# slyforce/MusicStyleTransfer

Hardware: AMD Instinct MI355X
Metric: piano-roll frames/s (VAE train step) (higher is better)
Workload: dtype bf16; 1 GPU; BASELINE configs[1]: single-track piano-roll VAE train step, T=256, pitch=128, latent=64, batch=64/GPU, bf16; encoder 256x2x8h, decoder 128x1x8h (scripts/train-vae.sh), dropout 0.2; Xavier-initialised weights; global_batch=64, seq_len=256, pitches=128, latent=64, parallelism=dp1, params=1885440

## Files before the change

include/mst_hip.h:

```cpp
#ifndef MST_HIP_H
#define MST_HIP_H

#include <stdint.h>

#ifdef __cplusplus
extern "C" {
#endif

typedef void* mst_stream_t;

enum mst_status {
  MST_OK = 0,
  MST_ERR_INVALID = -1,
  MST_ERR_LAUNCH = -2,
  MST_ERR_UNSUPPORTED = -3
};

enum mst_dtype { MST_BF16 = 0, MST_F16 = 1, MST_F32 = 2 };

enum mst_act { MST_ACT_NONE = 0, MST_ACT_RELU = 1 };

int mst_version(void);
const char* mst_last_error(void);

int mst_graph_begin(mst_stream_t stream);
int mst_graph_end(mst_stream_t stream, void** graph_exec_out);
int mst_graph_end_counted(mst_stream_t stream, void** graph_exec_out, int32_t* nodes_out, int32_t* kernel_nodes_out);
int mst_graph_launch(void* graph_exec, mst_stream_t stream);
int mst_graph_destroy(void* graph_exec);

int mst_event_create(void** ev_out);
int mst_event_record(void* ev, mst_stream_t stream);
int mst_event_sync(void* ev);
int mst_event_elapsed_ms(void* ev_start, void* ev_stop, float* ms_out);
int mst_event_destroy(void* ev);

typedef struct mst_gemm_args {
  int32_t dtype;
  int32_t c_f32;
  int64_t M, N, K;
  const void* A; int64_t lda;
  const void* B; int64_t ldb;
  void* C; int64_t ldc;
  const float* bias;
  const void* resid; int64_t ldr;
  int32_t act;
  const void* gate; int64_t ldg;
  float alpha;
  const float* rowadd; int64_t ldra; int64_t rowadd_period;
  const float* grpadd; int64_t ldga; const int32_t* grp_index;
  int64_t a_rows_per_group, a_group_stride, a_group_offset;
  int64_t c_rows_per_group, c_group_stride, c_group_offset;
  float dropout_p; uint64_t dropout_seed; uint32_t dropout_site;
  int32_t self_resid;
  const uint64_t* dropout_seed_ptr;
  int32_t a_u8;
  int32_t resid_phys;
} mst_gemm_args;

int mst_gemm_nt(const mst_gemm_args* args, mst_stream_t stream);
int mst_gemm_nt_form(const mst_gemm_args* args);

int mst_gemm_nt_pair(const mst_gemm_args* args0, const mst_gemm_args* args1, mst_stream_t stream);

typedef struct mst_bce_args {
  const uint8_t* labels;
  int64_t T;
  float label_smoothing;
  int32_t downweight;
  float* loss;
  void* probs; int64_t ldp;
  void* logits; int64_t ldl;
  float gscale;
} mst_bce_args;
int mst_gemm_sigmoid_bce(const mst_gemm_args* args, const mst_bce_args* bce, mst_stream_t stream);

typedef struct mst_ln_args {
  int32_t mode;
  const float* gamma;
  const float* beta;
  float eps;
  void* out; int64_t ld_out;
  float* mean; float* rstd;
  const void* x; int64_t ld_x;
  float* dgamma; float* dbeta;
  int32_t mask_mode;
  float* partials;
} mst_ln_args;

int mst_gemm_nt_ln(const mst_gemm_args* args, const mst_ln_args* ln, mst_stream_t stream);
int mst_gemm_sigmoid_bce_dgrad_ln(const mst_gemm_args* args, const mst_bce_args* bce, const mst_gemm_args* dgrad,
                                  const mst_ln_args* ln, mst_stream_t stream);
int64_t mst_gemm_nt_ln_parts(int64_t M);

int mst_ffn_ln_fwd(const mst_gemm_args* ff1, const mst_gemm_args* ff2, const mst_ln_args* ln, mst_stream_t stream);
int mst_ffn_ln_bwd(const mst_gemm_args* ff2_dgrad, const mst_gemm_args* ff1_dgrad, const mst_ln_args* ln, mst_stream_t stream);
typedef struct mst_ln_bwd_in {
  const void* dy; int64_t ld_dy;
  const void* x;  int64_t ld_x;
  const float* gamma; const float* mean; const float* rstd;
  void* dx; int64_t ld_dx;
  void* dx_masked; int64_t ld_dxm;
  float* dgamma; float* dbeta; float* partials;
  int32_t mask_mode;
  float dropout_p; uint64_t dropout_seed; const uint64_t* dropout_seed_ptr; uint32_t dropout_site;
} mst_ln_bwd_in;
int mst_ffn_ln_bwd_lead(const mst_ln_bwd_in* lead, const mst_gemm_args* ff2_dgrad, const mst_gemm_args* ff1_dgrad,
                        const mst_ln_args* ln, mst_stream_t stream);
int mst_proj_ffn_ln_fwd(const mst_gemm_args* proj, const mst_ln_args* ln1, const mst_gemm_args* ff1, const mst_gemm_args* ff2,
                        const mst_ln_args* ln2, mst_stream_t stream);

typedef struct mst_partial_sum {
  const float* src; int64_t n_parts; int64_t stride; int64_t len;
  float* dst; float scale;
} mst_partial_sum;
int mst_partial_sums(const mst_partial_sum* jobs, int n, mst_stream_t stream);

typedef struct mst_wgrad_args {
  int32_t dtype;
  int64_t M, N, K;
  const void* A; int64_t lda;
  const void* B; int64_t ldb;
  float* dW; int64_t ldw;
  float* db;
  float scale;
  int64_t a_rows_per_group, a_group_stride, a_group_offset;
  int64_t b_rows_per_group, b_group_stride, b_group_offset;
  int32_t a_u8;
} mst_wgrad_args;

typedef struct mst_outer_job {
  const float* L; const void* R; int32_t r_dtype; int64_t r_stride;
  int64_t B, J, I;
  float* out; float* obias;
} mst_outer_job;
int mst_outer_jobs(const mst_outer_job* jobs, int n, mst_stream_t stream);
int mst_gemm_wgrad_batch_flush(const mst_wgrad_args* list, int n, float* scratch, int64_t scratch_bytes,
                               const mst_partial_sum* sums, int n_sums, const mst_outer_job* outers, int n_outers,
                               mst_stream_t stream);
int mst_gemm_wgrad_plan(const mst_wgrad_args* list, int n, int64_t scratch_bytes, int64_t* plan);

int mst_embed_fwd(int dtype, int64_t B, int64_t T, int64_t D,
                  const int32_t* tokens, const float* table, int64_t ldt,
                  const int32_t* classes, const float* cls_table, int64_t ldc,
                  const float* pos, int64_t ldp, float alpha,
                  void* out, int64_t ld_out, int64_t S_out, int64_t s_off,
                  uint8_t* keymask, mst_stream_t stream);

int mst_embed_bwd(int dtype, int64_t B, int64_t T, int64_t D,
                  const int32_t* tokens, float* dtable, int64_t ldt,
                  const int32_t* classes, float* dcls, int64_t ldc, float alpha,
                  const void* dX, int64_t ld_dx, int64_t S_out, int64_t s_off,
                  mst_stream_t stream);

int mst_group_colsum(int dtype, int64_t B, int64_t T, int64_t D, const void* X, int64_t ldx,
                     int64_t S_out, int64_t s_off, const int32_t* idx, float* dst, int64_t ldd,
                     float alpha, mst_stream_t stream);

int mst_mask_from_lengths(int64_t B, int64_t S, const int32_t* lens, int32_t add,
                          uint8_t* keymask, mst_stream_t stream);

int mst_attn_keysoftmax_fwd(int dtype, int64_t B, int64_t S, int64_t H, int64_t dh,
                            const void* qkv, int64_t ld_qkv, int64_t k_off, int64_t q_off, int64_t v_off,
                            const uint8_t* keymask, float* lse,
                            void* out, int64_t ld_out,
                            int64_t q_limit ,
                            mst_stream_t stream);

int mst_attn_qkv_fwd(int dtype, int64_t B, int64_t S, int64_t H, int64_t dh, const void* x, int64_t ld_x, const void* w,
                     int64_t ld_w, const float* bias, void* qkv, int64_t ld_qkv, int64_t k_off, int64_t q_off, int64_t v_off,
                     const uint8_t* keymask, float* lse, void* out, int64_t ld_out, int64_t q_limit, mst_stream_t stream);
int mst_attn_keysoftmax_bwd(int dtype, int64_t B, int64_t S, int64_t H, int64_t dh,
                            const void* qkv, int64_t ld_qkv, int64_t k_off, int64_t q_off, int64_t v_off,
                            const uint8_t* keymask, const float* lse,
                            const void* dout, int64_t ld_dout,
                            void* dqkv, int64_t ld_dqkv, float* delta,
                            int64_t q_limit ,
                            mst_stream_t stream);

int mst_attn_causal_fwd(int dtype, int64_t B, int64_t S, int64_t H, int64_t dh,
                        const void* qkv, int64_t ld_qkv, int64_t k_off, int64_t q_off, int64_t v_off,
                        const uint8_t* keymask, float* lse, void* out, int64_t ld_out, mst_stream_t stream);
int mst_attn_causal_bwd(int dtype, int64_t B, int64_t S, int64_t H, int64_t dh,
                        const void* qkv, int64_t ld_qkv, int64_t k_off, int64_t q_off, int64_t v_off,
                        const uint8_t* keymask, const float* lse, const void* dout, int64_t ld_dout,
                        void* dqkv, int64_t ld_dqkv, float* delta, mst_stream_t stream);

int mst_layernorm_fwd(int dtype, int64_t M, int64_t D, const void* x, int64_t ldx,
                      const float* gamma, const float* beta, float eps,
                      void* y, int64_t ldy, float* mean, float* rstd,
                      int64_t row_id_stride ,
                      mst_stream_t stream);

int mst_layernorm_bwd(int dtype, int64_t M, int64_t D, const void* x, int64_t ldx,
                      const float* gamma, const float* mean, const float* rstd,
                      const void* dy, int64_t ldy, void* dx, int64_t ld_dx,
                      void* dx_masked, int64_t ld_dxm, float* dgamma, float* dbeta,
                      int mask_mode, float dropout_p, uint64_t dropout_seed, uint32_t dropout_site,
                      const uint64_t* dropout_seed_ptr,
                      int64_t row_id_stride ,
                      float* partials ,
                      mst_stream_t stream);
int64_t mst_layernorm_bwd_parts(int64_t M, int64_t D);

int mst_latent_fwd(int dtype, int64_t B, int64_t De, int64_t Z, int64_t Dd,
                   const void* enc_out, int64_t enc_sample_stride,
                   const float* Wl, const float* bl, const float* eps,
                   const float* Wh, const float* bh,
                   const int32_t* classes, const float* cls_d, int64_t ld_cls,
                   const float* pos_d, float alpha_d,
                   float* mu, float* sigma, float* z, float* kl,
                   void* dec_in, int64_t dec_sample_stride, mst_stream_t stream);
int mst_latent_fwd_proj(int dtype, int64_t B, int64_t De, int64_t Z, int64_t Dd,
                        const void* enc_out, int64_t enc_sample_stride,
                        const float* Wl, const float* bl, const float* eps,
                        const float* Wh, const float* bh,
                        const int32_t* classes, const float* cls_d, int64_t ld_cls,
                        const float* pos_d, float alpha_d,
                        float* mu, float* sigma, float* z, float* kl,
                        void* dec_in, int64_t dec_sample_stride,
                        const void* Wq, int64_t ld_wq, const float* bq, void* qkv0, int64_t qkv_sample_stride, int64_t nq,
                        mst_stream_t stream);
int mst_latent_rows(int dtype, int64_t N, int64_t M, int64_t Z, int64_t Dd,
                    const float* zsrc, const float* ssrc, const int32_t* a, const int32_t* b, const float* w, int mode,
                    float tau, uint64_t seed, const uint64_t* seed_ptr, uint32_t site, int64_t row0,
                    const float* Wh, const float* bh,
                    const int32_t* ca, const int32_t* cb, const float* cw, const float* cls_d, int64_t ld_cls, int64_t n_classes,
                    const float* pos_d, float alpha_d,
                    float* z_out, void* dec_in, int64_t dec_stride, mst_stream_t stream);

int mst_latent_bwd_vec(int dtype, int64_t B, int64_t De, int64_t Z, int64_t Dd, const float* Wl, const float* eps, const float* Wh,
                       const int32_t* classes, const float* mu, const float* sigma, const void* d_dec_in, int64_t dec_sample_stride,
                       float alpha_d, float kl_weight, float gscale, float enc_scale, float* dcls_d, int64_t ld_cls,
                       void* d_enc_out, int64_t denc_sample_stride, float* scratch, mst_stream_t stream);
int mst_latent_bwd_vec_proj(int dtype, int64_t B, int64_t De, int64_t Z, int64_t Dd, const float* Wl, const float* eps, const float* Wh,
                            const int32_t* classes, const float* mu, const float* sigma,
                            const void* dq0, int64_t dq_sample_stride, const void* Wt, int64_t ld_wt, int64_t nq,
                            const void* resid0, int64_t resid_sample_stride,
                            float alpha_d, float kl_weight, float gscale, float enc_scale, float* dcls_d, int64_t ld_cls,
                            void* d_enc_out, int64_t denc_sample_stride, float* scratch, mst_stream_t stream);

int mst_latent_bwd_vec_sched(int dtype, int64_t B, int64_t De, int64_t Z, int64_t Dd, const float* Wl, const float* eps, const float* Wh,
                             const int32_t* classes, const float* mu, const float* sigma, const void* d_dec_in, int64_t dec_sample_stride,
                             float alpha_d, const float* sched, const float* kl, float gscale, float enc_scale, float* dcls_d,
                             int64_t ld_cls, void* d_enc_out, int64_t denc_sample_stride, float* scratch, mst_stream_t stream);
int mst_latent_bwd_vec_proj_sched(int dtype, int64_t B, int64_t De, int64_t Z, int64_t Dd, const float* Wl, const float* eps,
                                  const float* Wh, const int32_t* classes, const float* mu, const float* sigma,
                                  const void* dq0, int64_t dq_sample_stride, const void* Wt, int64_t ld_wt, int64_t nq,
                                  const void* resid0, int64_t resid_sample_stride,
                                  float alpha_d, const float* sched, const float* kl, float gscale, float enc_scale, float* dcls_d,
                                  int64_t ld_cls, void* d_enc_out, int64_t denc_sample_stride, float* scratch, mst_stream_t stream);

int mst_reparam_kl_fwd(int64_t B, int64_t Z, const float* mu, const float* sigma, const float* eps,
                       float* z, float* kl, mst_stream_t stream);
int mst_reparam_kl_bwd(int64_t B, int64_t Z, const float* mu, const float* sigma, const float* eps,
                       const float* dz, float kl_weight, float* dmu, float* dsigma, mst_stream_t stream);

typedef struct mst_row_tail_args {
  int32_t dtype;
  int64_t B, D;
  const void* att; int64_t rs_att;
  const void* resid; int64_t rs_res;
  const void* Wp; int64_t ldwp; const float* bp;
// ... 146 lines not shown
```

musicstyletransfer_amd/csrc/gemm_nt.hip:

```cpp
#include <math.h>
#include <type_traits>
#include "common.hpp"
#include "gemm_tile.hpp"
#include "bce_math.hpp"
#include "step_begin.hpp"
#include "shadows.hpp"

namespace mst {

template <typename T, int BM, int BN, int WGM, int WGN, bool C_F32, int BK, bool ROWOPS, int PATH, bool DROP, bool AU8 = false>
__global__ __launch_bounds__(WGM * WGN * 64) void gemm_nt_kernel(mst_gemm_args a) {
  extern __shared__ __attribute__((aligned(16))) unsigned char smem[];
  f32x4 acc[(BN / WGN) / 16][(BM / WGM) / 16];
  int64_t m0, n0;
  float bias_pre[8];
  gemm_bias_preload<BM, BN>(a, bias_pre);
  gemm_mainloop<T, BM, BN, WGM, WGN, BK, ROWOPS, AU8, false, PATH == 1 || PATH == 4>(a, smem, acc, m0, n0);
  gemm_epilogue<T, BM, BN, WGM, WGN, C_F32, ROWOPS, PATH, DROP>(a, smem, acc, m0, n0, bias_pre);
}

template <typename T, int BM, int BN, int WGM, int WGN, int BK, int PATH>
__global__ __launch_bounds__(WGM * WGN * 64) void gemm_nt_pair_kernel(mst_gemm_args a0, mst_gemm_args a1, int tiles0, int tiles1, StepBegin sb,
                                                                       int n_begin) {
  extern __shared__ __attribute__((aligned(16))) unsigned char smem[];
// ... 77 lines not shown
      bet8[e] = (MODE == 1) ? l.beta[nc + e] : 0.f;
    }
  }
  float dg8[8], db8[8];
#pragma unroll
  for (int e = 0; e < 8; ++e) { dg8[e] = 0.f; db8[e] = 0.f; }

  u32x4 rv[ITERS], xv[ITERS];
  float mean_r[ITERS], rstd_r[ITERS];
  const bool tile_remap = a.c_rows_per_group <= 0 || a.c_rows_per_group % BM == 0;
  const int64_t pm0 = remap_row(m0, a.c_rows_per_group, a.c_group_stride, a.c_group_offset);
  auto phys_row = [&](int64_t m) { return tile_remap ? pm0 + (m - m0) : remap_row(m, a.c_rows_per_group, a.c_group_stride, a.c_group_offset); };
#pragma unroll
  for (int it = 0; it < ITERS; ++it) {
    const int64_t m = m0 + row0 + it * RSTEP;
    rv[it] = u32x4{0u, 0u, 0u, 0u}; xv[it] = rv[it]; mean_r[it] = 0.f; rstd_r[it] = 0.f;
    if (m < a.M) {
      const int64_t pm = phys_row(m);
      if (lds_resid) rv[it] = *reinterpret_cast<const u32x4*>(lds_resid + (row0 + it * RSTEP) * lds_resid_ld + nc);
      else if (resid) rv[it] = *reinterpret_cast<const u32x4*>(resid + m * a.ldr + nc);
      if (MODE == 2) {
        xv[it] = *reinterpret_cast<const u32x4*>(reinterpret_cast<const T*>(l.x) + pm * l.ld_x + nc);
        mean_r[it] = l.mean[pm];
        rstd_r[it] = l.rstd[pm];
      }
    }
  }
  FFN_STAMP(6);
#pragma unroll
  for (int it = 0; it < ITERS; ++it) {
    const int row = row0 + it * RSTEP;
    const int64_t m = m0 + row;
    if (m < a.M) {
      const int64_t pm = phys_row(m);
      const f32x4 v0 = *reinterpret_cast<const f32x4*>(sF + row * LDS_F + nc);
      const f32x4 v1 = *reinterpret_cast<const f32x4*>(sF + row * LDS_F + nc + 4);
      float t[8] = {v0[0], v0[1], v0[2], v0[3], v1[0], v1[1], v1[2], v1[3]};
#pragma unroll
      for (int e = 0; e < 8; ++e) t[e] = (t[e] + bias8[e]) * a.alpha;
      if (MODE == 1 && (has_drop || a.self_resid)) {
        float u0[4] = {t[0], t[1], t[2], t[3]}, u1[4] = {t[4], t[5], t[6], t[7]};
        if (has_drop) {
          const uint64_t w = (uint64_t)(pm * a.N + nc) >> 2;
          dropout_apply4(dkey, w, dthr, inv_keep, u0);
          dropout_apply4(dkey, w + 1, dthr, inv_keep, u1);
        }
#pragma unroll
        for (int e = 0; e < 4; ++e) {
          t[e] = a.self_resid ? t[e] + u0[e] : u0[e];
          t[4 + e] = a.self_resid ? t[4 + e] + u1[e] : u1[e];
        }
      }
      if (resid || lds_resid) {
        Pack8 p8; p8.u = rv[it];
#pragma unroll
        for (int e = 0; e < 8; ++e) t[e] += bits_to_f32<T>(p8.h[e]);
      }
      Pack8 hb;
#pragma unroll
      for (int e = 0; e < 8; ++e) { hb.h[e] = f32_to_bits<T>(t[e]); t[e] = bits_to_f32<T>(hb.h[e]); }
      if (MODE == 1) {
        *reinterpret_cast<u32x4*>(reinterpret_cast<T*>(a.C) + pm * a.ldc + nc) = hb.u;
        float s = 0.f;
#pragma unroll
        for (int e = 0; e < 8; ++e) s += t[e];
        const float mean = row_sum<CPR>(s) * inv_n;
        float ss = 0.f;
#pragma unroll
        for (int e = 0; e < 8; ++e) { t[e] -= mean; ss += t[e] * t[e]; }
        const float rstd = 1.f / sqrtf(row_sum<CPR>(ss) * inv_n + l.eps);
        Pack8 yb;
#pragma unroll
        for (int e = 0; e < 8; ++e) yb.h[e] = f32_to_bits<T>(t[e] * rstd * gam8[e] + bet8[e]);
        *reinterpret_cast<u32x4*>(reinterpret_cast<T*>(l.out) + pm * l.ld_out + nc) = yb.u;
        if (lds_out) *reinterpret_cast<u32x4*>(lds_out + row * lds_out_ld + nc) = yb.u;
        if (ch == 0) { l.mean[pm] = mean; l.rstd[pm] = rstd; }
      } else {
        const int64_t rid = pm;
        const float mean = mean_r[it], rstd = rstd_r[it];
        Pack8 xb; xb.u = xv[it];
        float xh[8], g[8], s1 = 0.f, s2 = 0.f;
#pragma unroll
        for (int e = 0; e < 8; ++e) {
          xh[e] = (bits_to_f32<T>(xb.h[e]) - mean) * rstd;
          g[e] = t[e] * gam8[e];
          s1 += g[e];
          s2 += g[e] * xh[e];
          dg8[e] += t[e] * xh[e];
          db8[e] += t[e];
        }
        s1 = row_sum<CPR>(s1) * inv_n;
        s2 = row_sum<CPR>(s2) * inv_n;
        uint32_t keep8 = 0xFFu;
        if (l.mask_mode != 0 && has_drop) {
          const uint64_t w = (uint64_t)(rid * BN + nc) >> 2;
          keep8 = dropout_keep4k(dkey, w, dthr) | (dropout_keep4k(dkey, w + 1, dthr) << 4);
        }
        Pack8 ob, mb;
#pragma unroll
        for (int e = 0; e < 8; ++e) {
          float o = rstd * (g[e] - s1 - xh[e] * s2);
          float om = 0.f;
          if (l.mask_mode != 0) {
            const float k = has_drop ? (((keep8 >> e) & 1u) ? inv_keep : 0.f) : 1.f;
            if (l.mask_mode == 1) om = o * k; else o = o * (1.f + k);
          }
          ob.h[e] = f32_to_bits<T>(o);
          mb.h[e] = f32_to_bits<T>(om);
        }
        *reinterpret_cast<u32x4*>(reinterpret_cast<T*>(a.C) + pm * a.ldc + nc) = ob.u;
        if (l.mask_mode == 1) *reinterpret_cast<u32x4*>(reinterpret_cast<T*>(l.out) + m * l.ld_out + nc) = mb.u;
        if (lds_out) *reinterpret_cast<u32x4*>(lds_out + row * lds_out_ld + nc) = l.mask_mode == 1 ? mb.u : ob.u;
      }
    } else if (lds_out) {
      *reinterpret_cast<u32x4*>(lds_out + row * lds_out_ld + nc) = u32x4{0u, 0u, 0u, 0u};
    }
  }
  FFN_STAMP(7);
  if (MODE == 2) {
    __syncthreads();
    float* red = sF;
#pragma unroll
    for (int e = 0; e < 8; ++e) {
      red[row0 * BN + nc + e] = dg8[e];
      red[(RSTEP + row0) * BN + nc + e] = db8[e];
    }
    __syncthreads();
    for (int c = tid; c < 2 * BN; c += NT) {
      const int which = c / BN, col = c % BN;
      float s = 0.f;
      for (int r = 0; r < RSTEP; ++r) s += red[(which * RSTEP + r) * BN + col];
      if (l.partials) l.partials[(int64_t)blockIdx.x * 2 * BN + c] = s;
      else atomicAdd((which ? l.dbeta : l.dgamma) + col, s);
    }
  }
}

template <typename T, int BM, int BN, int WGM, int WGN, int MODE>
__global__ __launch_bounds__(WGM * WGN * 64) void gemm_nt_ln_kernel(mst_gemm_args a, mst_ln_args l) {
  extern __shared__ __attribute__((aligned(16))) unsigned char smem[];
  f32x4 acc[(BN / WGN) / 16][(BM / WGM) / 16];
  int64_t m0, n0;
  constexpr size_t LOOP_B = (size_t)2 * (BM + BN) * 64 * 2, EPI_B = (size_t)BM * (BN + 4) * 4;
  float* sPar = reinterpret_cast<float*>(smem + (LOOP_B > EPI_B ? LOOP_B : EPI_B));
  for (int i = threadIdx.x; i < BN; i += WGM * WGN * 64) {
    sPar[i] = a.bias ? a.bias[i] : 0.f;
    sPar[BN + i] = l.gamma[i];
    sPar[2 * BN + i] = (MODE == 1) ? l.beta[i] : 0.f;
  }
  gemm_mainloop<T, BM, BN, WGM, WGN, 64>(a, smem, acc, m0, n0);
  gemm_epilogue_ln<T, BM, BN, WGM, WGN, MODE>(a, l, smem, acc, m0, nullptr, 0, nullptr, 0, sPar);
}

template <typename T, int BN, bool KEEP>
__device__ __forceinline__ void gemm_bce_tile(const mst_gemm_args& a, const mst_bce_args& q, unsigned char* smem, float* red, u32x4* keepA) {
  constexpr int BM = 64, WGM = 2, WGN = 4, NT = 512;
  constexpr int WTM = BM / WGM, WTN = BN / WGN, TM = WTM / 16, TN = WTN / 16;
  constexpr int LDS_F = BN + 4, CPR = BN / 8, RSTEP = NT / CPR, ITERS = BM / RSTEP;
  f32x4 acc[TN][TM];
  int64_t m0, n0;
  float bias8[8];
  gemm_bias_preload<BM, BN>(a, bias8);
  gemm_mainloop<T, BM, BN, WGM, WGN, 64>(a, smem, acc, m0, n0);
  const int64_t P = a.N;
  const int tid = threadIdx.x, lane = tid & 63, wave = tid >> 6;
  const int wm = wave / WGN, wn = wave % WGN, frow = lane & 15, fq = lane >> 4;
  float* sF = reinterpret_cast<float*>(smem);
#pragma unroll
  for (int i = 0; i < TM; ++i)
#pragma unroll
    for (int j = 0; j < TN; ++j)
      *reinterpret_cast<f32x4*>(sF + (wm * WTM + i * 16 + frow) * LDS_F + wn * WTN + j * 16 + fq * 4) = acc[j][i];
  const int64_t b = m0 / q.T;
  const int64_t per_sample = q.T * P;
  float w = 0.f;
  if (q.downweight) {
    const uint8_t* lab = q.labels + b * per_sample;
    int cnt = 0;
    for (int64_t i = (int64_t)tid * 8; i < per_sample; i += (int64_t)NT * 8)
      cnt += __popcll(*reinterpret_cast<const uint64_t*>(lab + i) & 0x0101010101010101ull);
    float c = wave_sum((float)cnt);
    if (lane == 0) red[wave] = c;
    __syncthreads();
    float np = 0.f;
#pragma unroll
    for (int i = 0; i < NT / 64; ++i) np += red[i];
    w = np / (((float)q.T * (float)P - np) + 1e-12f);
  }
  __syncthreads();
  const int ch = tid % CPR, nc = ch * 8, row0 = tid / CPR;
  const int64_t gc = n0 + nc;
  const float inv_n = 1.f / ((float)q.T * (float)P), ls = q.label_smoothing;
  float lsum = 0.f;
  const float s1 = (1.f - ls) + 0.5f * ls, s0 = 0.5f * ls;
  auto sweep = [&](auto dwc) {
    constexpr bool DW = decltype(dwc)::value;
#pragma unroll
    for (int it = 0; it < ITERS; ++it) {
      const int row = row0 + it * RSTEP;
      const int64_t m = m0 + row;
      const bool live = m < a.M;
      const f32x4 v0 = *reinterpret_cast<const f32x4*>(sF + row * LDS_F + nc);
      const f32x4 v1 = *reinterpret_cast<const f32x4*>(sF + row * LDS_F + nc + 4);
      const float t8[8] = {v0[0], v0[1], v0[2], v0[3], v1[0], v1[1], v1[2], v1[3]};
      const uint64_t lab8 = live ? *reinterpret_cast<const uint64_t*>(q.labels + m * P + gc) : 0ull;
      Pack8 pb, gb, xb;
      float x8[8];
      bool in_dom = true;
#pragma unroll
      for (int e = 0; e < 8; ++e) {
        xb.h[e] = f32_to_bits<T>((t8[e] + bias8[e]) * a.alpha);
        x8[e] = bits_to_f32<T>(xb.h[e]);
        in_dom = in_dom && bce_fast_domain(x8[e]);
      }
      const bool fast = __all(in_dom || !live);
#pragma unroll
      for (int e = 0; e < 8; ++e) {
        const float y = (float)((lab8 >> (8 * e)) & 0xFFull);
        float p, bce, dbce;
        bce_fast<DW>(x8[e], y, s1, s0, w, p, bce, dbce);
        if (!fast) {
          float p2, b2, d2;
          bce_exact<DW>(x8[e], y, ls, w, p2, b2, d2);
          if (!bce_fast_domain(x8[e])) { p = p2; bce = b2; dbce = d2; }
        }
        lsum += live ? bce : 0.f;
        pb.h[e] = f32_to_bits<T>(p);
        gb.h[e] = f32_to_bits<T>(dbce * inv_n * q.gscale);
      }
      if (!live) continue;
      if (a.C) *reinterpret_cast<u32x4*>(reinterpret_cast<T*>(a.C) + m * a.ldc + gc) = gb.u;
      if constexpr (KEEP) keepA[(ch >> 3) * (BM * 8) + row * 8 + ((ch & 7) ^ (row & 7))] = gb.u;
      if (q.probs) *reinterpret_cast<u32x4*>(reinterpret_cast<T*>(q.probs) + m * q.ldp + gc) = pb.u;
      if (q.logits) *reinterpret_cast<u32x4*>(reinterpret_cast<T*>(q.logits) + m * q.ldl + gc) = xb.u;
    }
  };
  if (q.downweight) sweep(std::true_type()); else sweep(std::false_type());
  lsum = wave_sum(lsum);
  if (lane == 0) red[wave] = lsum;
  __syncthreads();
  if (tid == 0) {
    float tot = 0.f;
#pragma unroll
    for (int i = 0; i < NT / 64; ++i) tot += red[i];
    atomicAdd(q.loss + b, tot * inv_n);
  }
}

template <typename T, int BN>
__global__ __launch_bounds__(512) void gemm_bce_kernel(mst_gemm_args a, mst_bce_args q) {
  extern __shared__ __attribute__((aligned(16))) unsigned char smem[];
  __shared__ float red[512 / 64];
  gemm_bce_tile<T, BN, false>(a, q, smem, red, nullptr);
}

template <typename T>
__global__ __launch_bounds__(512) void gemm_bce_dgrad_ln_kernel(mst_gemm_args a, mst_bce_args q, mst_gemm_args g2, mst_ln_args l) {
  constexpr int BM = 64, BN = 128, WGM = 2, WGN = 4;
  constexpr size_t OFF2 = 48 * 1024, END2 = OFF2 + (size_t)2 * (BM + BN) * 64 * 2;
  extern __shared__ __attribute__((aligned(16))) unsigned char smem[];
  __shared__ float red[512 / 64];
  float* sPar = reinterpret_cast<float*>(smem + END2);
  for (int i = threadIdx.x; i < BN; i += 512) {
    sPar[i] = g2.bias ? g2.bias[i] : 0.f;
    sPar[BN + i] = l.gamma[i];
    sPar[2 * BN + i] = 0.f;
  }
  gemm_bce_tile<T, BN, true>(a, q, smem, red, reinterpret_cast<u32x4*>(smem + OFF2));
  __syncthreads();
  f32x4 acc[(BN / WGN) / 16][(BM / WGM) / 16];
  int64_t m0, n0;
  gemm_mainloop<T, BM, BN, WGM, WGN, 64, true, false, true>(g2, smem + OFF2, acc, m0, n0);
  gemm_epilogue_ln<T, BM, BN, WGM, WGN, 2>(g2, l, smem, acc, m0, nullptr, 0, nullptr, 0, sPar);
}

template <typename T>
static int launch_gemm_bce_dgrad_ln(const mst_gemm_args& a, const mst_bce_args& q, const mst_gemm_args& g2, const mst_ln_args& l, hipStream_t s) {
  const size_t lds = (size_t)48 * 1024 + (size_t)2 * (64 + 128) * 64 * 2 + (size_t)3 * 128 * 4;
  static bool opted = false;
  if (!opted) {
    const hipError_t e = hipFuncSetAttribute(reinterpret_cast<const void*>(&gemm_bce_dgrad_ln_kernel<T>), hipFuncAttributeMaxDynamicSharedMemorySize, (int)lds);
    if (e != hipSuccess) { set_error("gemm_bce_dgrad_ln_kernel: LDS opt-in of %zu bytes: %s", lds, hipGetErrorString(e)); return MST_ERR_LAUNCH; }
    opted = true;
  }
  hipLaunchKernelGGL((gemm_bce_dgrad_ln_kernel<T>), dim3((unsigned)cdiv(a.M, 64)), dim3(512), lds, s, a, q, g2, l);
  MST_CHECK_LAUNCH("gemm_bce_dgrad_ln_kernel");
  return MST_OK;
}

template <typename T, int BN>
static int launch_gemm_bce(const mst_gemm_args& a, const mst_bce_args& q, hipStream_t s) {
  const size_t lds_loop = (size_t)2 * (64 + BN) * 64 * 2, lds_epi = (size_t)64 * (BN + 4) * 4;
  const size_t lds = lds_loop > lds_epi ? lds_loop : lds_epi;
  if (lds > 64 * 1024) {
    static bool opted = false;
    if (!opted) {
      const hipError_t e = hipFuncSetAttribute(reinterpret_cast<const void*>(&gemm_bce_kernel<T, BN>), hipFuncAttributeMaxDynamicSharedMemorySize, (int)lds);
      if (e != hipSuccess) { set_error("gemm_bce_kernel: LDS opt-in of %zu bytes: %s", lds, hipGetErrorString(e)); return MST_ERR_LAUNCH; }
      opted = true;
    }
  }
  hipLaunchKernelGGL((gemm_bce_kernel<T, BN>), dim3((unsigned)(cdiv(a.M, 64) * (a.N / BN))), dim3(512), lds, s, a, q);
  MST_CHECK_LAUNCH("gemm_bce_kernel");
  return MST_OK;
}

template <typename T, int BN, int WGM, int WGN, int MODE, bool LEAD, bool FULL, bool EXTRA = false>
__global__ __launch_bounds__(WGM * WGN * 64) void ffn_ln_kernel(mst_gemm_args g1, mst_gemm_args g2, mst_ln_args ln, mst_ln_bwd_in lead,
                                                                mst_gemm_args gx, mst_ln_args lnx) {
  constexpr bool HEAD = EXTRA;
  static_assert(!EXTRA || MODE == 1, "the extra GEMM is the forward form's head");
  constexpr int BM = 64, BK = 64, CHUNKS = BK / 8;
  constexpr int NT = WGM * WGN * 64;
  constexpr int WTM = BM / WGM, WTN = BN / WGN, TM = WTM / 16, TN = WTN / 16;
  constexpr int B_CH = BN * CHUNKS / NT;
  constexpr int LDA = BN + 8;
  constexpr int KST = BN / BK;
  static_assert(BN * CHUNKS % NT == 0 && (BM * BN / 8) % NT == 0, "tile/threads mismatch");
  typedef typename Act<T>::vec8 vec8;
  extern __shared__ __attribute__((aligned(16))) unsigned char smem[];
  u32x4* sB = reinterpret_cast<u32x4*>(smem);
  T* sH = reinterpret_cast<T*>(smem + (size_t)2 * BN * BK * 2);
  T* sX = sH + BM * LDA;
  float* sBias1 = reinterpret_cast<float*>(sX + BM * LDA);
  float* sPar = sBias1 + g1.N;
  const int tid = threadIdx.x, lane = tid & 63, wave = tid >> 6;
  const int wm = wave / WGN, wn = wave % WGN, frow = lane & 15, fq = lane >> 4;
  int64_t m0 = xcd_chunk(blockIdx.x, gridDim.x) * BM;
  if (g1.a_rows_per_group > 0) {
    const uint32_t grp = (uint32_t)m0 / (uint32_t)g1.a_rows_per_group;
    m0 += (int64_t)grp * (g1.a_group_stride - g1.a_rows_per_group) + g1.a_group_offset;
    g1.M = g2.M = gx.M = (g1.M / g1.a_rows_per_group) * g1.a_group_stride;
  }
  const int64_t F = g1.N;
  FFN_STAMP(0); FFN_RT(190);
  const int64_t Mg = FULL ? (int64_t)1 << 62 : g1.M;
  for (int i = tid * 4; i < (int)F; i += NT * 4)
    *reinterpret_cast<f32x4*>(sBias1 + i) = g1.bias ? *reinterpret_cast<const f32x4*>(g1.bias + i) : f32x4{0.f, 0.f, 0.f, 0.f};
  const uint64_t seed2 = g2.dropout_seed ^ ((g2.dropout_p > 0.f && g2.dropout_seed_ptr) ? g2.dropout_seed_ptr[0] : 0ull);
  const uint64_t seedx = EXTRA ? gx.dropout_seed ^ ((gx.dropout_p > 0.f && gx.dropout_seed_ptr) ? gx.dropout_seed_ptr[0] : 0ull) : 0ull;
  for (int i = tid; i < BN; i += NT) {
    sPar[i] = g2.bias ? g2.bias[i] : 0.f;
    sPar[BN + i] = ln.gamma[i];
    sPar[2 * BN + i] = (MODE == 1) ? ln.beta[i] : 0.f;
    if constexpr (HEAD) {
      sPar[3 * BN + i] = gx.bias ? gx.bias[i] : 0.f;
      sPar[4 * BN + i] = lnx.gamma[i];
      sPar[5 * BN + i] = lnx.beta[i];
    }
  }
  const int n_chunks = (int)(F / BN);
  const int rot = (int)((blockIdx.x / 8) % (unsigned)n_chunks);
  auto phys = [&](int c) { const int pc = c + rot; return pc >= n_chunks ? pc - n_chunks : pc; };
  const T* __restrict__ W1 = reinterpret_cast<const T*>(g1.B);
  const T* __restrict__ W2 = reinterpret_cast<const T*>(g2.B);
  const T* __restrict__ WX = reinterpret_cast<const T*>(gx.B);

  uint32_t off1[B_CH], off2[B_CH], offx[B_CH];
  int b_lds[B_CH];
#pragma unroll
  for (int i = 0; i < B_CH; ++i) {
    const int c = tid + i * NT;
    const int row = c / CHUNKS, ch = c % CHUNKS;
    off1[i] = (uint32_t)row * (uint32_t)g1.ldb + (uint32_t)ch * 8u;
    off2[i] = (uint32_t)row * (uint32_t)g2.ldb + (uint32_t)ch * 8u;
    offx[i] = EXTRA ? (uint32_t)row * (uint32_t)gx.ldb + (uint32_t)ch * 8u : 0u;
    b_lds[i] = row * CHUNKS + (ch ^ (row & 7));
  }
  constexpr int SPC = 2 * KST;
  constexpr int RING = BN >= 256 ? 4 : 2, AHEAD = RING - 1;
  static_assert(SPC % RING == 0, "ring slots must repeat per chunk");
  u32x4 ring[RING][B_CH];
  auto load_stage = [&](int c, int s, u32x4 (&rb)[B_CH]) {
    if (HEAD && c < 0) {
      const T* base = WX + s * BK;
#pragma unroll
      for (int i = 0; i < B_CH; ++i) rb[i] = *reinterpret_cast<const u32x4*>(base + offx[i]);
    } else if (s < KST) {
      const T* base = W1 + (int64_t)phys(c) * BN * g1.ldb + s * BK;
#pragma unroll
      for (int i = 0; i < B_CH; ++i) rb[i] = *reinterpret_cast<const u32x4*>(base + off1[i]);
    } else {
      const T* base = W2 + (int64_t)phys(c) * BN + (s - KST) * BK;
#pragma unroll
      for (int i = 0; i < B_CH; ++i) rb[i] = *reinterpret_cast<const u32x4*>(base + off2[i]);
    }
  };
  auto load_piece = [&](int c, int s, u32x4 (&rb)[B_CH], auto ic) {
    constexpr int i = decltype(ic)::value;
    const T* base;
    uint32_t off;
    if (HEAD && c < 0) { base = WX + s * BK; off = offx[i]; }
    else if (s < KST) { base = W1 + (int64_t)phys(c) * BN * g1.ldb + s * BK; off = off1[i]; }
    else { base = W2 + (int64_t)phys(c) * BN + (s - KST) * BK; off = off2[i]; }
    rb[i] = *reinterpret_cast<const u32x4*>(base + off);
  };
  auto store_stage = [&](int buf, const u32x4 (&rb)[B_CH]) {
#pragma unroll
    for (int i = 0; i < B_CH; ++i) sB[buf * BN * CHUNKS + b_lds[i]] = rb[i];
  };
  {
    auto pro = [&](auto jc) {
      constexpr int j = decltype(jc)::value;
      if constexpr (HEAD) {
        static_assert(!HEAD || AHEAD <= KST, "the head GEMM's stages cover the prologue");
        if (j < AHEAD) load_stage(-1, j, ring[j % RING]);
      } else {
        if (j < AHEAD && (j < SPC || n_chunks > 1)) load_stage(j / SPC, j % SPC, ring[j % RING]);
      }
    };
    pro(std::integral_constant<int, 0>()); pro(std::integral_constant<int, 1>()); pro(std::integral_constant<int, 2>());
    pro(std::integral_constant<int, 3>()); pro(std::integral_constant<int, 4>()); pro(std::integral_constant<int, 5>());
    pro(std::integral_constant<int, 6>());
    static_assert(AHEAD <= 7, "the prologue list covers seven stages");
  }
  if constexpr (LEAD) {
    constexpr int CPR = BN / 8, RSTEP = NT / CPR, ITERS = BM / RSTEP;
    const int ch = tid % CPR, nc = ch * 8, row0 = tid / CPR;
    const float inv_n = 1.f / (float)BN;
    const bool has_drop = lead.dropout_p > 0.f && lead.mask_mode == 1;
    const uint64_t dseed = lead.dropout_seed ^ ((has_drop && lead.dropout_seed_ptr) ? lead.dropout_seed_ptr[0] : 0ull);
    const uint32_t dkey = dropout_key(dseed, lead.dropout_site), dthr = dropout_thr(lead.dropout_p);
    const float inv_keep = dropout_inv_keep(lead.dropout_p);
    float gam8[8], dg8[8], db8[8];
#pragma unroll
    for (int e = 0; e < 8; ++e) { gam8[e] = lead.gamma[nc + e]; dg8[e] = 0.f; db8[e] = 0.f; }
    u32x4 dyv[ITERS], xv[ITERS];
    float mean_r[ITERS], rstd_r[ITERS];
#pragma unroll
    for (int it = 0; it < ITERS; ++it) {
      const int64_t m = m0 + row0 + it * RSTEP;
      dyv[it] = u32x4{0u, 0u, 0u, 0u}; xv[it] = dyv[it]; mean_r[it] = 0.f; rstd_r[it] = 0.f;
      if (m < Mg) {
        dyv[it] = *reinterpret_cast<const u32x4*>(reinterpret_cast<const T*>(lead.dy) + m * lead.ld_dy + nc);
        xv[it] = *reinterpret_cast<const u32x4*>(reinterpret_cast<const T*>(lead.x) + m * lead.ld_x + nc);
        mean_r[it] = lead.mean[m];
        rstd_r[it] = lead.rstd[m];
      }
    }
#pragma unroll
    for (int it = 0; it < ITERS; ++it) {
      const int row = row0 + it * RSTEP;
      const int64_t m = m0 + row;
      Pack8 db, xb;
      db.u = dyv[it]; xb.u = xv[it];
      float xh[8], g[8], s1 = 0.f, s2 = 0.f;
#pragma unroll
      for (int e = 0; e < 8; ++e) {
        const float d = bits_to_f32<T>(db.h[e]);
        xh[e] = (bits_to_f32<T>(xb.h[e]) - mean_r[it]) * rstd_r[it];
        g[e] = d * gam8[e];
        s1 += g[e];
        s2 += g[e] * xh[e];
        dg8[e] += d * xh[e];
        db8[e] += d;
      }
      s1 = row_sum<CPR>(s1) * inv_n;
      s2 = row_sum<CPR>(s2) * inv_n;
      uint32_t keep8 = 0xFFu;
      if (has_drop) {
        const uint64_t w = (uint64_t)(m * BN + nc) >> 2;
        keep8 = dropout_keep4k(dkey, w, dthr) | (dropout_keep4k(dkey, w + 1, dthr) << 4);
      }
      Pack8 ob, mb;
#pragma unroll
      for (int e = 0; e < 8; ++e) {
        const float o = rstd_r[it] * (g[e] - s1 - xh[e] * s2);
        const float k = has_drop ? (((keep8 >> e) & 1u) ? inv_keep : 0.f) : 1.f;
        ob.h[e] = f32_to_bits<T>(o);
        mb.h[e] = f32_to_bits<T>(o * k);
      }
      if (m < Mg) {
        *reinterpret_cast<u32x4*>(reinterpret_cast<T*>(lead.dx) + m * lead.ld_dx + nc) = ob.u;
        if (lead.mask_mode == 1) *reinterpret_cast<u32x4*>(reinterpret_cast<T*>(lead.dx_masked) + m * lead.ld_dxm + nc) = mb.u;
      }
      *reinterpret_cast<u32x4*>(sX + row * LDA + nc) = (m < Mg) ? (lead.mask_mode == 1 ? mb.u : ob.u) : u32x4{0u, 0u, 0u, 0u};
    }
    float* red = reinterpret_cast<float*>(smem);
    static_assert((size_t)2 * RSTEP * BN * 4 <= (size_t)2 * BN * BK * 2, "reduction scratch must fit the weight stages");
#pragma unroll
    for (int e = 0; e < 8; ++e) {
      red[row0 * BN + nc + e] = dg8[e];
      red[(RSTEP + row0) * BN + nc + e] = db8[e];
    }
    __syncthreads();
    for (int c = tid; c < 2 * BN; c += NT) {
      const int which = c / BN, col = c % BN;
      float sm = 0.f;
      for (int r = 0; r < RSTEP; ++r) sm += red[(which * RSTEP + r) * BN + col];
      if (lead.partials) lead.partials[(int64_t)blockIdx.x * 2 * BN + c] = sm;
      else atomicAdd((which ? lead.dbeta : lead.dgamma) + col, sm);
    }
    __syncthreads();
  } else
  {
    const T* X = reinterpret_cast<const T*>(HEAD ? gx.A : g1.A);
    const int64_t ldx = HEAD ? gx.lda : g1.lda;
    constexpr int CPR = BN / 8;
#pragma unroll
    for (int i = 0; i < BM * CPR / NT; ++i) {
      const int c = tid + i * NT, row = c / CPR, ch = c % CPR;
      u32x4 v = {0u, 0u, 0u, 0u};
      if (m0 + row < Mg) v = *reinterpret_cast<const u32x4*>(X + (m0 + row) * ldx + ch * 8);
      *reinterpret_cast<u32x4*>(sX + row * LDA + ch * 8) = v;
    }
  }
  auto mma_stage = [&](f32x4 (&acc)[TN][TM], const T* sA, int buf, const u32x4 (&rb)[B_CH], auto&& hook) {
    const u32x4* cB = sB + buf * BN * CHUNKS;
#pragma unroll
    for (int ks = 0; ks < BK / 32; ++ks) {
      vec8 xf[TM], wf[TN];
      const int kc = ks * 4 + fq;
#pragma unroll
      for (int i = 0; i < TM; ++i)
        xf[i] = __builtin_bit_cast(vec8, *reinterpret_cast<const u32x4*>(sA + (wm * WTM + i * 16 + frow) * LDA + kc * 8));
#pragma unroll
      for (int j = 0; j < TN; ++j) {
        const int row = wn * WTN + j * 16 + frow;
        wf[j] = __builtin_bit_cast(vec8, cB[row * CHUNKS + (kc ^ (row & 7))]);
      }
      auto row = [&](auto jc) {
        constexpr int j = decltype(jc)::value;
        if constexpr (j < TN) {
#pragma unroll
          for (int i = 0; i < TM; ++i) acc[j][i] = Act<T>::mfma16(wf[j], xf[i], acc[j][i]);
          if (ks == 0) hook(std::integral_constant<int, j>()); else hook(std::integral_constant<int, TN + j>());
        }
      };
      static_assert(TN <= 4, "row list");
      row(std::integral_constant<int, 0>()); row(std::integral_constant<int, 1>());
      row(std::integral_constant<int, 2>()); row(std::integral_constant<int, 3>());
    }
  };
  auto no_hook = [](auto) {};

  f32x4 acc1[TN][TM], acc2[TN][TM];
#pragma unroll
  for (int j = 0; j < TN; ++j)
#pragma unroll
    for (int i = 0; i < TM; ++i) acc2[j][i] = f32x4{0.f, 0.f, 0.f, 0.f};
  const float p1 = g1.dropout_p;
  const bool drop1 = MODE == 1 && p1 > 0.f;
  const uint64_t seed1 = g1.dropout_seed ^ ((drop1 && g1.dropout_seed_ptr) ? g1.dropout_seed_ptr[0] : 0ull);
  const uint32_t dkey1 = dropout_key(seed1, g1.dropout_site), dthr1 = dropout_thr(p1);
  const float inv_keep1 = dropout_inv_keep(p1);
  const bool idx32 = (uint64_t)g1.M * (uint64_t)F < (1ull << 32);
  const bool relu1 = MODE == 1 && g1.act == MST_ACT_RELU;
  const bool step_form1 = MODE == 1 && relu1 && drop1 && idx32 && g1.alpha == 1.f;
  uint32_t rowmul[TM];
#pragma unroll
  for (int i = 0; i < TM; ++i) rowmul[i] = (uint32_t)(m0 + wm * WTM + i * 16 + frow) * (uint32_t)(F >> 1) * DROPOUT_MUL;
  T* Aout = reinterpret_cast<T*>(g1.C);

  auto extra_gemm = [&](int cx) {
#pragma unroll
    for (int j = 0; j < TN; ++j)
#pragma unroll
      for (int i = 0; i < TM; ++i) acc1[j][i] = f32x4{0.f, 0.f, 0.f, 0.f};
    store_stage(0, ring[0]);
    __syncthreads();
    auto xstage = [&](auto sc) {
      constexpr int s = decltype(sc)::value;
      if constexpr (s < KST) {
        constexpr int t = s + AHEAD;
        if constexpr (t < KST) load_stage(cx, t, ring[t % RING]);
        else if constexpr (HEAD) load_stage(0, t - KST, ring[t % RING]);
        mma_stage(acc1, sX + s * BK, s & 1, ring[s % RING], no_hook);
        if constexpr (s + 1 < KST) store_stage((s + 1) & 1, ring[(s + 1) % RING]);
        __syncthreads();
      }
    };
    static_assert(!EXTRA || (KST <= 4 && KST % RING == 0), "the extra GEMM stage list / ring slots");
    xstage(std::integral_constant<int, 0>()); xstage(std::integral_constant<int, 1>());
    xstage(std::integral_constant<int, 2>()); xstage(std::integral_constant<int, 3>());
  };
  if constexpr (HEAD) {
    extra_gemm(-1);
    gemm_epilogue_ln<T, BM, BN, WGM, WGN, 1>(gx, lnx, smem, acc1, m0, nullptr, 0, sX, LDA, sPar + 3 * BN, &seedx);
    __syncthreads();
  }
  store_stage(0, ring[0]);
  __syncthreads();
  FFN_STAMP(1);
  for (int c = 0; c < n_chunks; ++c) {
    const int pc = phys(c);
#pragma unroll
    for (int j = 0; j < TN; ++j)
#pragma unroll
      for (int i = 0; i < TM; ++i) acc1[j][i] = f32x4{0.f, 0.f, 0.f, 0.f};
    constexpr int OUT_CH = BM * (BN / 8) / NT;
    u32x4 gv[OUT_CH];
    if constexpr (MODE == 2) {
      const T* G = reinterpret_cast<const T*>(g1.gate);
#pragma unroll
      for (int i = 0; i < OUT_CH; ++i) {
        const int cc = tid + i * NT, row = cc / (BN / 8), ch = cc % (BN / 8);
        gv[i] = u32x4{0u, 0u, 0u, 0u};
        if (m0 + row < Mg) gv[i] = *reinterpret_cast<const u32x4*>(G + (m0 + row) * g1.ldg + (int64_t)pc * BN + ch * 8);
      }
    }
    auto stage = [&](auto sc) {
      constexpr int s = decltype(sc)::value;
      if constexpr (s < SPC) {
        constexpr bool IL = BN >= 256 && B_CH <= 2 * TN;
        constexpr int t = s + AHEAD;
        const int tc = t < SPC ? c : (c + 1 < n_chunks ? c + 1 : c);
        const bool more = s + 1 < SPC || c + 1 < n_chunks;
        auto piece = [&](auto kc) {
          constexpr int k = decltype(kc)::value;
          if constexpr (IL && k < B_CH) {
            __builtin_amdgcn_sched_barrier(0);
            load_piece(tc, t % SPC, ring[t % RING], kc);
            if (more) sB[((s + 1) & 1) * BN * CHUNKS + b_lds[k]] = ring[(s + 1) % RING][k];
            __builtin_amdgcn_sched_barrier(0);
          }
        };
        if constexpr (!IL) load_stage(tc, t % SPC, ring[t % RING]);
        FFN_STAMP(8 + (c * SPC + s) * 4);
        if constexpr (s < KST) mma_stage(acc1, sX + s * BK, s & 1, ring[s % RING], piece);
        else mma_stage(acc2, sH + (s - KST) * BK, s & 1, ring[s % RING], piece);
        FFN_STAMP(8 + (c * SPC + s) * 4 + 1);
        if constexpr (s == KST - 1) {
          auto chunk_epilogue = [&](auto step_form) {
            constexpr bool STEP = decltype(step_form)::value;
            const uint32_t cmul = ((uint32_t)pc * (BN / 2) + (uint32_t)((wn * WTN + fq * 4) / 2)) * DROPOUT_MUL;
#pragma unroll
            for (int j = 0; j < TN; ++j) {
              const int n = wn * WTN + j * 16 + fq * 4;
              const int64_t col = (int64_t)pc * BN + n;
              const f32x4 b4 = *reinterpret_cast<const f32x4*>(sBias1 + col);
#pragma unroll
              for (int i = 0; i < TM; ++i) {
                const int row = wm * WTM + i * 16 + frow;
                float tv[4];
                if constexpr (STEP) {
#pragma unroll
                  for (int e = 0; e < 4; ++e) tv[e] = fmaxf(acc1[j][i][e] + b4[e], 0.f);
                  dropout_apply4_pre(dkey1, rowmul[i] + cmul + (uint32_t)(j * 8) * DROPOUT_MUL, dthr1, inv_keep1, tv);
                } else {
#pragma unroll
                  for (int e = 0; e < 4; ++e) {
                    tv[e] = (acc1[j][i][e] + b4[e]) * g1.alpha;
                    if (relu1) tv[e] = fmaxf(tv[e], 0.f);
                  }
                  if (drop1) dropout_apply4(dkey1, (uint64_t)((m0 + row) * F + col) >> 2, dthr1, inv_keep1, tv);
                }
                uint16_t hb[4];
#pragma unroll
                for (int e = 0; e < 4; ++e) hb[e] = f32_to_bits<T>(tv[e]);
                *reinterpret_cast<u32x2*>(sH + row * LDA + n) =
                    u32x2{(uint32_t)hb[0] | ((uint32_t)hb[1] << 16), (uint32_t)hb[2] | ((uint32_t)hb[3] << 16)};
              }
            }
          };
          if (step_form1) chunk_epilogue(std::true_type()); else chunk_epilogue(std::false_type());
        }
        if (!IL && more) store_stage((s + 1) & 1, ring[(s + 1) % RING]);
        FFN_STAMP(8 + (c * SPC + s) * 4 + 2);
        __syncthreads();
        FFN_STAMP(8 + (c * SPC + s) * 4 + 3);
        if constexpr (s == KST - 1) {
          constexpr int CPR = BN / 8;
#pragma unroll
          for (int i = 0; i < BM * CPR / NT; ++i) {
            const int cc = tid + i * NT, row = cc / CPR, ch = cc % CPR;
            u32x4 v = *reinterpret_cast<const u32x4*>(sH + row * LDA + ch * 8);
            if constexpr (MODE == 2) {
              Pack8 pv, pg;
              pv.u = v; pg.u = gv[i];
#pragma unroll
              for (int e = 0; e < 8; ++e)
                if (!(bits_to_f32<T>(pg.h[e]) > 0.f)) pv.h[e] = 0;
              v = pv.u;
              *reinterpret_cast<u32x4*>(sH + row * LDA + ch * 8) = v;
            }
            if (m0 + row < Mg) *reinterpret_cast<u32x4*>(Aout + (m0 + row) * g1.ldc + (int64_t)pc * BN + ch * 8) = v;
          }
          if constexpr (MODE == 2) __syncthreads();
        }
      }
    };
    static_assert(SPC <= 8, "the stage list below covers eight stages per chunk");
    stage(std::integral_constant<int, 0>()); stage(std::integral_constant<int, 1>());
    stage(std::integral_constant<int, 2>()); stage(std::integral_constant<int, 3>());
    stage(std::integral_constant<int, 4>()); stage(std::integral_constant<int, 5>());
    stage(std::integral_constant<int, 6>()); stage(std::integral_constant<int, 7>());
  }
  const bool resid_is_x = g2.resid == g1.A && g2.ldr == g1.lda;
  FFN_STAMP(2);
  gemm_epilogue_ln<T, BM, BN, WGM, WGN, MODE>(g2, ln, smem, acc2, m0, resid_is_x ? sX : nullptr, LDA, nullptr, 0, sPar, &seed2);
  FFN_STAMP(3); FFN_RT(191);
}

template <typename T, int BN>
static int launch_ffn_ln(const mst_gemm_args& g1, const mst_gemm_args& g2, const mst_ln_args& ln, const mst_ln_bwd_in* lead, hipStream_t s,
                         const mst_gemm_args* gx = nullptr, const mst_ln_args* lnx = nullptr) {
  constexpr int BM = 64;
  const int ex = gx ? 1 : 0;
  const size_t lds_loop = (size_t)2 * BN * 64 * 2 + (size_t)2 * BM * (BN + 8) * 2 + (size_t)g1.N * 4 + (size_t)6 * BN * 4;
  const size_t lds_epi = (size_t)BM * (BN + 4) * 4;
  const size_t lds = lds_loop > lds_epi ? lds_loop : lds_epi;
  const int full = g1.M % BM == 0 ? 1 : 0;
  const int mi = ex ? 6 + full : (lead ? 2 : (ln.mode == 2 ? 1 : 0)) * 2 + full;
  typedef void (*kern_t)(mst_gemm_args, mst_gemm_args, mst_ln_args, mst_ln_bwd_in, mst_gemm_args, mst_ln_args);
  const kern_t fns[8] = {&ffn_ln_kernel<T, BN, 2, 4, 1, false, false>, &ffn_ln_kernel<T, BN, 2, 4, 1, false, true>,
                         &ffn_ln_kernel<T, BN, 2, 4, 2, false, false>, &ffn_ln_kernel<T, BN, 2, 4, 2, false, true>,
                         &ffn_ln_kernel<T, BN, 2, 4, 2, true, false>, &ffn_ln_kernel<T, BN, 2, 4, 2, true, true>,
                         &ffn_ln_kernel<T, BN, 2, 4, 1, false, false, true>, &ffn_ln_kernel<T, BN, 2, 4, 1, false, true, true>};
  static size_t opted[8] = {64 * 1024, 64 * 1024, 64 * 1024, 64 * 1024, 64 * 1024, 64 * 1024, 64 * 1024, 64 * 1024};
  if (lds > opted[mi]) {
    const hipError_t e = hipFuncSetAttribute(reinterpret_cast<const void*>(fns[mi]), hipFuncAttributeMaxDynamicSharedMemorySize, (int)lds);
    if (e != hipSuccess) { set_error("ffn_ln_kernel: LDS opt-in of %zu bytes: %s", lds, hipGetErrorString(e)); return MST_ERR_LAUNCH; }
    opted[mi] = lds;
  }
  const mst_ln_bwd_in none = {};
  const mst_gemm_args no_gemm = {};
  const mst_ln_args no_ln = {};
  hipLaunchKernelGGL(fns[mi], dim3((unsigned)cdiv(g1.M, BM)), dim3(512), lds, s, g1, g2, ln, lead ? *lead : none,
                     gx ? *gx : no_gemm, lnx ? *lnx : no_ln);
  MST_CHECK_LAUNCH("ffn_ln_kernel");
  return MST_OK;
}

template <typename T, int BM, int BN, int WGM, int WGN>
static int launch_gemm_ln(const mst_gemm_args& a, const mst_ln_args& l, hipStream_t s) {
  const size_t lds_loop = (size_t)2 * (BM + BN) * 64 * 2, lds_epi = (size_t)BM * (BN + 4) * 4;
  const size_t lds = (lds_loop > lds_epi ? lds_loop : lds_epi) + (size_t)3 * BN * 4;
  dim3 grid((unsigned)cdiv(a.M, BM)), block(WGM * WGN * 64);
  const int mi = l.mode == 2 ? 1 : 0;
  const void* fn = mi ? reinterpret_cast<const void*>(&gemm_nt_ln_kernel<T, BM, BN, WGM, WGN, 2>)
                      : reinterpret_cast<const void*>(&gemm_nt_ln_kernel<T, BM, BN, WGM, WGN, 1>);
  if (lds > 64 * 1024) {
    static bool opted[2] = {false, false};
    if (!opted[mi]) {
      const hipError_t e = hipFuncSetAttribute(fn, hipFuncAttributeMaxDynamicSharedMemorySize, (int)lds);
      if (e != hipSuccess) { set_error("gemm_nt_ln_kernel: LDS opt-in of %zu bytes: %s", lds, hipGetErrorString(e)); return MST_ERR_LAUNCH; }
      opted[mi] = true;
    }
  }
  if (mi) hipLaunchKernelGGL((gemm_nt_ln_kernel<T, BM, BN, WGM, WGN, 2>), grid, block, lds, s, a, l);
  else hipLaunchKernelGGL((gemm_nt_ln_kernel<T, BM, BN, WGM, WGN, 1>), grid, block, lds, s, a, l);
  MST_CHECK_LAUNCH("gemm_nt_ln_kernel");
  return MST_OK;
}

static bool gemm_3cu_form(const mst_gemm_args& a) {
  constexpr int BM = 128, BN = 128, BK = 32;
  const bool rowops = a.rowadd || a.grpadd || a.a_rows_per_group > 0 || a.c_rows_per_group > 0;
  return !a.c_f32 && !a.a_u8 && !rowops && a.dropout_p == 0.f && !a.self_resid && a.M % BM == 0 && a.N % BN == 0 && a.K % BK == 0 &&
         a.ldc % 8 == 0 && (uint64_t)a.M * (uint64_t)a.N < (1ull << 32) &&
         (!a.resid || (a.ldr % 8 == 0 && (uintptr_t)a.resid % 16 == 0)) && (!a.gate || (a.ldg % 8 == 0 && (uintptr_t)a.gate % 16 == 0));
}
template <typename T>
static int launch_gemm_3cu(const mst_gemm_args& a, hipStream_t s) {
  constexpr int BM = 128, BN = 128, BK = 32;
  const size_t lds_loop = (size_t)2 * (BM + BN) * BK * 2, lds_epi = (size_t)(BM / 2) * (BN + 4) * 4;
  const size_t lds = lds_loop > lds_epi ? lds_loop : lds_epi;
  hipLaunchKernelGGL((gemm_nt_kernel<T, BM, BN, 2, 2, false, BK, false, 4, false>), dim3((unsigned)((a.M / BM) * (a.N / BN))), dim3(256), lds, s, a);
  MST_CHECK_LAUNCH("gemm_nt_kernel");
  return MST_OK;
}

template <int BM, int BN>
static bool gemm_fast_form(const mst_gemm_args& a) {
  const bool rowops = a.rowadd || a.grpadd || a.a_rows_per_group > 0 || a.c_rows_per_group > 0;
  const int64_t phys_rows = a.c_rows_per_group > 0 ? (a.M / a.c_rows_per_group + 1) * a.c_group_stride + a.c_group_offset : a.M;
  return !a.c_f32 && a.M % BM == 0 && a.N % BN == 0 && a.ldc % 8 == 0 &&
         (a.c_rows_per_group <= 0 || a.c_rows_per_group % BM == 0) &&
         (uint64_t)phys_rows * (uint64_t)a.N < (1ull << 32) &&
         (!a.resid || (a.ldr % 8 == 0 && (uintptr_t)a.resid % 16 == 0)) &&
         (!a.gate || (a.ldg % 8 == 0 && (uintptr_t)a.gate % 16 == 0)) &&
         (!rowops || (a.rowadd_period % BM == 0 && (!a.rowadd || (a.ldra % 4 == 0 && (uintptr_t)a.rowadd % 16 == 0)) &&
                      (!a.grpadd || (a.ldga % 4 == 0 && (uintptr_t)a.grpadd % 16 == 0))));
}

template <int BM, int BN, int BK>
static int gemm_variant(const mst_gemm_args& a) {
  const bool rowops = a.rowadd || a.grpadd || a.a_rows_per_group > 0 || a.c_rows_per_group > 0;
  const bool fast = gemm_fast_form<BM, BN>(a) && a.K % BK == 0;
  const bool drop = a.dropout_p > 0.f || a.self_resid;
  return a.a_u8 ? (fast ? 8 : 9) : (a.c_f32 ? 3 : (fast ? (drop ? 1 : 0) : 2)) + (rowops ? 4 : 0);
}

static int gemm_nt_form(const mst_gemm_args& a) {
  const int64_t big_tiles = cdiv(a.M, 128) * cdiv(a.N, 128);
  const int64_t last_round = big_tiles % 512;
  const bool stub_round = big_tiles > 512 && last_round > 0 && last_round < 128;
  const bool ragged128 = a.M % 128 != 0 && a.M % 64 == 0 && a.N % 128 == 0 && !a.c_f32;
  if (big_tiles > 512 && big_tiles <= 768 && a.N >= 128 && !ragged128 && gemm_3cu_form(a)) return 3 * 16;
  if (big_tiles >= 384 && a.N >= 128 && !stub_round && !ragged128) return 2 * 16 + gemm_variant<128, 128, 64>(a);
  if (a.M <= 64 && a.K >= 512 && a.K % 256 == 0) return 1 * 16 + gemm_variant<64, 64, 256>(a);
  return gemm_variant<64, 64, 64>(a);
}

template <typename T, int BM, int BN, int WGM, int WGN, int BK = 64>
static int launch_gemm(const mst_gemm_args& a, int variant, hipStream_t s) {
  const int64_t tiles = cdiv(a.M, BM) * cdiv(a.N, BN);
  const size_t lds_loop = (size_t)2 * (BM + BN) * BK * 2, lds_epi = (size_t)BM * (BN + 4) * 4;
  const size_t lds = lds_loop > lds_epi ? lds_loop : lds_epi;
  dim3 grid((unsigned)tiles), block(WGM * WGN * 64);
  typedef void (*kern_t)(mst_gemm_args);
  const kern_t fns[10] = {&gemm_nt_kernel<T, BM, BN, WGM, WGN, false, BK, false, 1, false>, &gemm_nt_kernel<T, BM, BN, WGM, WGN, false, BK, false, 1, true>,
                         &gemm_nt_kernel<T, BM, BN, WGM, WGN, false, BK, false, 2, true>, &gemm_nt_kernel<T, BM, BN, WGM, WGN, true, BK, false, 2, true>,
                         &gemm_nt_kernel<T, BM, BN, WGM, WGN, false, BK, true, 1, false>, &gemm_nt_kernel<T, BM, BN, WGM, WGN, false, BK, true, 1, true>,
                         &gemm_nt_kernel<T, BM, BN, WGM, WGN, false, BK, true, 2, true>, &gemm_nt_kernel<T, BM, BN, WGM, WGN, true, BK, true, 2, true>,
                         &gemm_nt_kernel<T, BM, BN, WGM, WGN, false, BK, true, 1, false, true>, &gemm_nt_kernel<T, BM, BN, WGM, WGN, false, BK, true, 2, false, true>};
  if (lds > 64 * 1024) {
    static bool opted[10] = {false, false, false, false, false, false, false, false, false, false};
    if (!opted[variant]) {
      const hipError_t e = hipFuncSetAttribute(reinterpret_cast<const void*>(fns[variant]), hipFuncAttributeMaxDynamicSharedMemorySize, (int)lds);
      if (e != hipSuccess) { set_error("gemm_nt_kernel: LDS opt-in of %zu bytes: %s", lds, hipGetErrorString(e)); return MST_ERR_LAUNCH; }
      opted[variant] = true;
    }
  }
  hipLaunchKernelGGL(fns[variant], grid, block, lds, s, a);
  MST_CHECK_LAUNCH("gemm_nt_kernel");
  return MST_OK;
}

}

using namespace mst;

static int check_gemm_common(const mst_gemm_args& a) {
  MST_CHECK_ARG(a.M > 0 && a.N > 0 && a.K > 0, "mst_gemm_nt: M,N,K must be positive (got %lld,%lld,%lld)",
                (long long)a.M, (long long)a.N, (long long)a.K);
  MST_CHECK_ARG(a.K % 8 == 0 && a.lda % 8 == 0 && a.ldb % 8 == 0,
                "mst_gemm_nt: K, lda, ldb must be multiples of 8 (got %lld,%lld,%lld)", (long long)a.K,
                (long long)a.lda, (long long)a.ldb);
  MST_CHECK_ARG(a.A && a.B && a.C, "mst_gemm_nt: null operand");
  MST_CHECK_ARG(a.dropout_p >= 0.f && a.dropout_p < 1.f, "mst_gemm_nt: dropout_p must be in [0,1)");
  MST_CHECK_ARG(((uintptr_t)a.A % 16 == 0) && ((uintptr_t)a.B % 16 == 0) && ((uintptr_t)a.C % 16 == 0),
                "mst_gemm_nt: operands must be 16-byte aligned");
  return MST_OK;
}

extern "C" int64_t mst_gemm_nt_ln_parts(int64_t M) { return M > 0 ? cdiv(M, 64) : 0; }

static int ffn_ln_impl(const char* who, const mst_gemm_args* first, const mst_gemm_args* second, const mst_ln_args* ln, int mode,
                       mst_stream_t stream, const mst_ln_bwd_in* lead = nullptr, const mst_gemm_args* extra = nullptr,
                       const mst_ln_args* extra_ln = nullptr) {
  MST_CHECK_ARG(first != nullptr && second != nullptr && ln != nullptr, "%s: null args", who);
  const mst_gemm_args& a = *first;
  const mst_gemm_args& b = *second;
  const mst_ln_args& l = *ln;
  int rc = check_gemm_common(a);
  if (rc) return rc;
  rc = check_gemm_common(b);
  if (rc) return rc;
  MST_CHECK_ARG(a.dtype == b.dtype && a.M == b.M, "%s: the two GEMMs must share dtype and M", who);
  MST_CHECK_ARG((b.N == 256 || b.N == 128) && a.K == b.N, "%s: the model width (first K = second N) must be 128 or 256 (got %lld, %lld)", who,
                (long long)a.K, (long long)b.N);
  MST_CHECK_ARG(a.N == b.K && a.N % b.N == 0, "%s: the hidden width (first N = second K) must be a multiple of the model width", who);
  MST_CHECK_ARG(b.A == a.C && b.lda == a.ldc, "%s: the second GEMM's A operand must be the first one's output (it is consumed on chip)", who);
  MST_CHECK_ARG(!a.c_f32 && !b.c_f32 && !b.gate && !a.rowadd && !b.rowadd && !a.grpadd && !b.grpadd && !a.resid && !a.self_resid &&
                b.act == MST_ACT_NONE && a.c_rows_per_group <= 0 && b.a_rows_per_group <= 0 && b.c_rows_per_group <= 0,
                "%s: fp32 outputs, row-indexed adds, row remaps, a gate or activation on the second GEMM and a residual on the first are not supported", who);
  MST_CHECK_ARG(a.a_rows_per_group <= 0 || (a.a_rows_per_group % 64 == 0 && a.M % a.a_rows_per_group == 0 && a.a_group_offset >= 0 &&
                                            a.a_group_stride >= a.a_rows_per_group + a.a_group_offset && a.M < (1ll << 31)),
                "%s: row groups must be whole 64-row tiles (rows per group %lld, stride %lld, offset %lld, M %lld)", who,
                (long long)a.a_rows_per_group, (long long)a.a_group_stride, (long long)a.a_group_offset, (long long)a.M);
  MST_CHECK_ARG(a.lda % 8 == 0 && a.ldc % 8 == 0 && a.ldc >= a.N && b.ldc % 8 == 0 && b.ldc >= b.N, "%s: leading dimensions must be multiples of 8", who);
  MST_CHECK_ARG((uint64_t)a.N * (uint64_t)a.ldb < (1ull << 32) && (uint64_t)b.N * (uint64_t)b.ldb < (1ull << 32), "%s: weight matrices too large", who);
  MST_CHECK_ARG(!b.resid || (b.ldr % 8 == 0 && b.ldr >= b.N && (uintptr_t)b.resid % 16 == 0), "%s: bad residual layout", who);
  MST_CHECK_ARG(!a.bias || (uintptr_t)a.bias % 16 == 0, "%s: the first GEMM's bias must be 16-byte aligned", who);
  MST_CHECK_ARG(a.dropout_p == 0.f || a.N % 4 == 0, "%s: dropout needs widths that are multiples of 4", who);
  MST_CHECK_ARG(l.mode == mode && l.gamma && l.mean && l.rstd, "%s: LayerNorm arguments of the wrong form", who);
  if (mode == 1) {
    MST_CHECK_ARG(!a.gate, "%s: a gate belongs to the backward form", who);
    MST_CHECK_ARG(l.beta && l.out && l.ld_out % 8 == 0 && l.ld_out >= b.N && (uintptr_t)l.out % 16 == 0,
                  "%s: the LayerNorm arguments are those of mst_gemm_nt_ln's forward form", who);
  } else {
    MST_CHECK_ARG(a.gate && a.ldg % 8 == 0 && a.ldg >= a.N && (uintptr_t)a.gate % 16 == 0, "%s: the first GEMM needs the forward activation as its gate", who);
    MST_CHECK_ARG(a.act == MST_ACT_NONE && a.dropout_p == 0.f && !b.self_resid, "%s: activation / dropout / self_resid belong to the forward form", who);
    MST_CHECK_ARG(l.x && l.ld_x % 8 == 0 && (uintptr_t)l.x % 16 == 0 && (l.partials || (l.dgamma && l.dbeta)) && (uintptr_t)l.partials % 16 == 0,
                  "%s: backward needs x and dgamma + dbeta (or partials)", who);
    MST_CHECK_ARG(l.mask_mode >= 0 && l.mask_mode <= 2 &&
                  (l.mask_mode != 1 || (l.out && l.ld_out % 8 == 0 && l.ld_out >= b.N && (uintptr_t)l.out % 16 == 0)),
                  "%s: mask_mode must be 0, 1 (with out) or 2", who);
  }
  if (lead) {
    const mst_ln_bwd_in& q = *lead;
    MST_CHECK_ARG(mode == 2, "%s: a leading LayerNorm belongs to the backward form", who);
    MST_CHECK_ARG(q.dy && q.x && q.gamma && q.mean && q.rstd && q.dx && (q.partials || (q.dgamma && q.dbeta)), "%s: leading LayerNorm: null pointer", who);
    MST_CHECK_ARG(q.ld_dy % 8 == 0 && q.ld_x % 8 == 0 && q.ld_dx % 8 == 0 && q.ld_dy >= b.N && q.ld_x >= b.N && q.ld_dx >= b.N &&
                  ((uintptr_t)q.dy | (uintptr_t)q.x | (uintptr_t)q.dx | (uintptr_t)q.partials) % 16 == 0, "%s: leading LayerNorm: bad layout", who);
    MST_CHECK_ARG(q.mask_mode == 0 || (q.mask_mode == 1 && q.dx_masked && q.ld_dxm % 8 == 0 && q.ld_dxm >= b.N && (uintptr_t)q.dx_masked % 16 == 0),
                  "%s: leading LayerNorm: mask_mode must be 0 or 1 (with dx_masked)", who);
    MST_CHECK_ARG(q.dropout_p >= 0.f && q.dropout_p < 1.f, "%s: leading LayerNorm: dropout_p must be in [0,1)", who);
    const void* tile = q.mask_mode == 1 ? q.dx_masked : q.dx;
    const int64_t tile_ld = q.mask_mode == 1 ? q.ld_dxm : q.ld_dx;
    MST_CHECK_ARG(a.A == tile && a.lda == tile_ld, "%s: the first GEMM's A operand must be the leading LayerNorm's (masked) output", who);
  }
  if (extra) {
    const mst_gemm_args& x = *extra;
    rc = check_gemm_common(x);
    if (rc) return rc;
    MST_CHECK_ARG(x.dtype == a.dtype && x.M == a.M && x.N == b.N && x.K == b.N, "%s: the extra GEMM is width x width on the same rows", who);
    MST_CHECK_ARG(!x.c_f32 && !x.gate && !x.rowadd && !x.grpadd && x.act == MST_ACT_NONE && x.a_rows_per_group <= 0 && x.c_rows_per_group <= 0 &&
                  x.ldc % 8 == 0 && x.ldc >= x.N && (uint64_t)x.N * (uint64_t)x.ldb < (1ull << 32),
                  "%s: the extra GEMM takes no gate, activation, row-indexed add or row remap", who);
    MST_CHECK_ARG(mode == 1 && extra_ln != nullptr, "%s: the projection (with its LayerNorm) rides in front of the forward form", who);
    const mst_ln_args& q = *extra_ln;
    MST_CHECK_ARG(q.mode == 1 && q.gamma && q.beta && q.mean && q.rstd && q.out == a.A && q.ld_out == a.lda,
                  "%s: the leading LayerNorm's output must be the first GEMM's A operand", who);
    MST_CHECK_ARG(!x.resid || (x.ldr % 8 == 0 && x.ldr >= x.N && (uintptr_t)x.resid % 16 == 0), "%s: bad residual layout", who);
  }
  hipStream_t s = (hipStream_t)stream;
  return dispatch_act(a.dtype, [&](auto tag) -> int {
    typedef decltype(tag) T;
    if (b.N == 256) return launch_ffn_ln<T, 256>(a, b, l, lead, s, extra, extra_ln);
    return launch_ffn_ln<T, 128>(a, b, l, lead, s, extra, extra_ln);
  });
}

extern "C" int mst_proj_ffn_ln_fwd(const mst_gemm_args* proj, const mst_ln_args* ln1, const mst_gemm_args* ff1, const mst_gemm_args* ff2,
                                   const mst_ln_args* ln2, mst_stream_t stream) {
  MST_CHECK_ARG(proj != nullptr && ln1 != nullptr, "mst_proj_ffn_ln_fwd: null args");
  return ffn_ln_impl("mst_proj_ffn_ln_fwd", ff1, ff2, ln2, 1, stream, nullptr, proj, ln1);
}

extern "C" int mst_ffn_ln_bwd_lead(const mst_ln_bwd_in* lead, const mst_gemm_args* ff2_dgrad, const mst_gemm_args* ff1_dgrad,
                                   const mst_ln_args* ln, mst_stream_t stream) {
  MST_CHECK_ARG(lead != nullptr, "mst_ffn_ln_bwd_lead: null args");
  return ffn_ln_impl("mst_ffn_ln_bwd_lead", ff2_dgrad, ff1_dgrad, ln, 2, stream, lead);
}

extern "C" int mst_ffn_ln_fwd(const mst_gemm_args* ff1, const mst_gemm_args* ff2, const mst_ln_args* ln, mst_stream_t stream) {
  return ffn_ln_impl("mst_ffn_ln_fwd", ff1, ff2, ln, 1, stream);
}
extern "C" int mst_ffn_ln_bwd(const mst_gemm_args* ff2_dgrad, const mst_gemm_args* ff1_dgrad, const mst_ln_args* ln, mst_stream_t stream) {
  return ffn_ln_impl("mst_ffn_ln_bwd", ff2_dgrad, ff1_dgrad, ln, 2, stream);
}

static int check_gemm_ln(const mst_gemm_args& a, const mst_ln_args& l) {
  int rc = check_gemm_common(a);
  if (rc) return rc;
  MST_CHECK_ARG(a.N == 256 || a.N == 128, "mst_gemm_nt_ln: the row width N must be 128 or 256 (got %lld): use mst_gemm_nt + "
                "mst_layernorm_* for other widths", (long long)a.N);
  MST_CHECK_ARG(l.mode == 1 || l.mode == 2, "mst_gemm_nt_ln: mode must be 1 (forward) or 2 (backward)");
  MST_CHECK_ARG(!a.c_f32 && !a.gate && !a.rowadd && !a.grpadd && a.act == MST_ACT_NONE,
                "mst_gemm_nt_ln: fp32 output, gate, rowadd, grpadd and activations are not supported in the fused form");
  MST_CHECK_ARG(a.ldc % 8 == 0 && a.ldc >= a.N, "mst_gemm_nt_ln: ldc must be a multiple of 8 and >= N");
  MST_CHECK_ARG(!a.resid || (a.ldr % 8 == 0 && a.ldr >= a.N && (uintptr_t)a.resid % 16 == 0), "mst_gemm_nt_ln: bad residual layout");
  MST_CHECK_ARG(l.gamma && l.mean && l.rstd, "mst_gemm_nt_ln: gamma / mean / rstd are required");
  if (l.mode == 1) {
    MST_CHECK_ARG(l.beta && l.out && l.ld_out % 8 == 0 && l.ld_out >= a.N && (uintptr_t)l.out % 16 == 0, "mst_gemm_nt_ln: forward needs beta and out");
  } else {
    MST_CHECK_ARG(l.x && l.ld_x % 8 == 0 && (uintptr_t)l.x % 16 == 0 && (l.partials || (l.dgamma && l.dbeta)),
                  "mst_gemm_nt_ln: backward needs x and dgamma + dbeta (or partials)");
    MST_CHECK_ARG((uintptr_t)l.partials % 16 == 0, "mst_gemm_nt_ln: partials must be 16-byte aligned");
    MST_CHECK_ARG(l.mask_mode >= 0 && l.mask_mode <= 2, "mst_gemm_nt_ln: mask_mode must be 0, 1 or 2");
    MST_CHECK_ARG(l.mask_mode != 1 || (l.out && l.ld_out % 8 == 0 && l.ld_out >= a.N && (uintptr_t)l.out % 16 == 0),
                  "mst_gemm_nt_ln: mask_mode 1 needs out");
    MST_CHECK_ARG(!a.self_resid, "mst_gemm_nt_ln: self_resid belongs to the forward form");
  }
  return MST_OK;
}

extern "C" int mst_gemm_nt_ln(const mst_gemm_args* args, const mst_ln_args* ln, mst_stream_t stream) {
  MST_CHECK_ARG(args != nullptr && ln != nullptr, "mst_gemm_nt_ln: null args");
  const mst_gemm_args& a = *args;
  const mst_ln_args& l = *ln;
  int rc = check_gemm_ln(a, l);
  if (rc) return rc;
  hipStream_t s = (hipStream_t)stream;
  return dispatch_act(a.dtype, [&](auto tag) -> int {
    typedef decltype(tag) T;
    if (a.N == 256) return launch_gemm_ln<T, 64, 256, 2, 4>(a, l, s);
    return launch_gemm_ln<T, 64, 128, 2, 4>(a, l, s);
  });
}

static int check_gemm_bce(const mst_gemm_args& a, const mst_bce_args& q) {
  MST_CHECK_ARG(a.M > 0 && a.K > 0 && a.K % 8 == 0 && a.lda % 8 == 0 && a.ldb % 8 == 0 && a.A && a.B,
                "mst_gemm_sigmoid_bce: bad GEMM operands");
  MST_CHECK_ARG(((uintptr_t)a.A % 16 == 0) && ((uintptr_t)a.B % 16 == 0), "mst_gemm_sigmoid_bce: operands must be 16-byte aligned");
  MST_CHECK_ARG(a.N == 128 || (a.N > 0 && a.N % 256 == 0), "mst_gemm_sigmoid_bce: the row of pitches must be 128 or a multiple of 256 wide (got %lld): use "
                "mst_gemm_nt + mst_sigmoid_bce for other widths", (long long)a.N);
  MST_CHECK_ARG(a.N <= 256 || !q.downweight, "mst_gemm_sigmoid_bce: the label down-weighting counts a sample's positives in every workgroup — rows wider than "
                "one tile (256) take mst_gemm_nt + mst_sigmoid_bce");
  MST_CHECK_ARG(q.T > 0 && q.T % 64 == 0 && a.M % q.T == 0, "mst_gemm_sigmoid_bce: T must be a multiple of 64 and divide M (a tile holds one sample's rows)");
  MST_CHECK_ARG(!a.c_f32 && !a.resid && !a.gate && !a.rowadd && !a.grpadd && a.act == MST_ACT_NONE && a.dropout_p == 0.f && !a.self_resid &&
                a.c_rows_per_group <= 0 && !a.a_u8, "mst_gemm_sigmoid_bce: only bias, alpha and an A row remap are supported");
  MST_CHECK_ARG(q.labels && q.loss && (uintptr_t)q.labels % 8 == 0, "mst_gemm_sigmoid_bce: labels / loss missing or labels not 8-byte aligned");
  MST_CHECK_ARG(!a.C || (a.ldc % 8 == 0 && a.ldc >= a.N && (uintptr_t)a.C % 16 == 0), "mst_gemm_sigmoid_bce: bad dlogits layout");
  MST_CHECK_ARG(!q.probs || (q.ldp % 8 == 0 && q.ldp >= a.N && (uintptr_t)q.probs % 16 == 0), "mst_gemm_sigmoid_bce: bad probs layout");
  MST_CHECK_ARG(!q.logits || (q.ldl % 8 == 0 && q.ldl >= a.N && (uintptr_t)q.logits % 16 == 0), "mst_gemm_sigmoid_bce: bad logits layout");
  return MST_OK;
}

extern "C" int mst_gemm_sigmoid_bce(const mst_gemm_args* args, const mst_bce_args* bce, mst_stream_t stream) {
  MST_CHECK_ARG(args != nullptr && bce != nullptr, "mst_gemm_sigmoid_bce: null args");
  const mst_gemm_args& a = *args;
  const mst_bce_args& q = *bce;
  int rc = check_gemm_bce(a, q);
  if (rc) return rc;
  hipStream_t s = (hipStream_t)stream;
  return dispatch_act(a.dtype, [&](auto tag) -> int {
    typedef decltype(tag) T;
    if (a.N % 256 == 0) return launch_gemm_bce<T, 256>(a, q, s);
    return launch_gemm_bce<T, 128>(a, q, s);
  });
}

extern "C" int mst_gemm_sigmoid_bce_dgrad_ln(const mst_gemm_args* args, const mst_bce_args* bce, const mst_gemm_args* dgrad,
                                             const mst_ln_args* ln, mst_stream_t stream) {
  MST_CHECK_ARG(args != nullptr && bce != nullptr && dgrad != nullptr && ln != nullptr, "mst_gemm_sigmoid_bce_dgrad_ln: null args");
  const mst_gemm_args &a = *args, &g2 = *dgrad;
  const mst_bce_args& q = *bce;
  const mst_ln_args& l = *ln;
  int rc = check_gemm_bce(a, q);
  if (rc == MST_OK) rc = check_gemm_ln(g2, l);
  if (rc) return rc;
  const bool one = a.N == 128 && g2.N == 128 && g2.K == 128 && g2.M == a.M && a.M % 64 == 0 && l.mode == 2 && a.C && g2.A == a.C &&
                   g2.lda == a.ldc && g2.dtype == a.dtype && g2.a_rows_per_group <= 0 && !g2.a_u8;
  if (!one) {
    rc = mst_gemm_sigmoid_bce(args, bce, stream);
    return rc != MST_OK ? rc : mst_gemm_nt_ln(dgrad, ln, stream);
  }
  hipStream_t s = (hipStream_t)stream;
  return dispatch_act(a.dtype, [&](auto tag) -> int {
    typedef decltype(tag) T;
    return launch_gemm_bce_dgrad_ln<T>(a, q, g2, l, s);
  });
}

static int check_gemm_nt(const mst_gemm_args* args) {
  MST_CHECK_ARG(args != nullptr, "mst_gemm_nt: null args");
  const mst_gemm_args& a = *args;
  MST_CHECK_ARG(a.M > 0 && a.N > 0 && a.K > 0, "mst_gemm_nt: M,N,K must be positive (got %lld,%lld,%lld)",
                (long long)a.M, (long long)a.N, (long long)a.K);
  MST_CHECK_ARG(a.K % 8 == 0 && a.lda % 8 == 0 && a.ldb % 8 == 0,
                "mst_gemm_nt: K, lda, ldb must be multiples of 8 (got %lld,%lld,%lld)", (long long)a.K,
                (long long)a.lda, (long long)a.ldb);
  MST_CHECK_ARG(a.ldc % 4 == 0 && a.ldc >= a.N, "mst_gemm_nt: ldc must be a multiple of 4 and >= N");
  MST_CHECK_ARG(a.A && a.B && a.C, "mst_gemm_nt: null operand");
  MST_CHECK_ARG(!a.resid || (a.ldr % 4 == 0 && a.ldr >= a.N), "mst_gemm_nt: ldr must be a multiple of 4 and >= N");
  MST_CHECK_ARG(!a.gate || (a.ldg % 4 == 0 && a.ldg >= a.N), "mst_gemm_nt: ldg must be a multiple of 4 and >= N");
  MST_CHECK_ARG((!a.rowadd && !a.grpadd) || a.rowadd_period > 0, "mst_gemm_nt: rowadd_period must be > 0");
  MST_CHECK_ARG(!a.grpadd || a.grp_index, "mst_gemm_nt: grpadd needs grp_index");
  MST_CHECK_ARG(a.dropout_p >= 0.f && a.dropout_p < 1.f, "mst_gemm_nt: dropout_p must be in [0,1)");
  MST_CHECK_ARG(a.dropout_p == 0.f || a.N % 4 == 0, "mst_gemm_nt: dropout needs N to be a multiple of 4");
  MST_CHECK_ARG(((uintptr_t)a.A % 16 == 0) && ((uintptr_t)a.B % 16 == 0) && ((uintptr_t)a.C % 16 == 0),
                "mst_gemm_nt: operands must be 16-byte aligned");
  MST_CHECK_ARG(!a.a_u8 || (!a.c_f32 && a.dropout_p == 0.f && !a.self_resid),
                "mst_gemm_nt: a uint8 A operand comes with a 16-bit C and without dropout / self_resid");
  if (a.dtype != MST_BF16 && a.dtype != MST_F16) return dispatch_act(a.dtype, [](auto) { return 0; });
  return MST_OK;
}

extern "C" int mst_gemm_nt_form(const mst_gemm_args* args) {
  const int rc = check_gemm_nt(args);
  return rc != MST_OK ? rc : gemm_nt_form(*args);
}

extern "C" int mst_gemm_nt(const mst_gemm_args* args, mst_stream_t stream) {
  const int rc = check_gemm_nt(args);
  if (rc != MST_OK) return rc;
  const mst_gemm_args& a = *args;
  const int form = gemm_nt_form(a), variant = form & 15;
  hipStream_t s = (hipStream_t)stream;
  return dispatch_act(a.dtype, [&](auto tag) -> int {
    typedef decltype(tag) T;
    switch (form >> 4) {
      case 3: return launch_gemm_3cu<T>(a, s);
      case 2: return launch_gemm<T, 128, 128, 2, 2>(a, variant, s);
      case 1: return launch_gemm<T, 64, 64, 2, 2, 256>(a, variant, s);
      default: return launch_gemm<T, 64, 64, 2, 2>(a, variant, s);
    }
  });
}

extern "C" int mst_gemm_nt_pair(const mst_gemm_args* args0, const mst_gemm_args* args1, mst_stream_t stream) {
  return mst_gemm_nt_pair_begin(args0, args1, nullptr, stream);
}

extern "C" int mst_gemm_nt_pair_begin(const mst_gemm_args* args0, const mst_gemm_args* args1, const mst_step_begin_args* begin,
                                      mst_stream_t stream) {
  MST_CHECK_ARG(args0 != nullptr && args1 != nullptr, "mst_gemm_nt_pair: null args");
  const mst_gemm_args &a0 = *args0, &a1 = *args1;
  auto plain = [](const mst_gemm_args& a) {
    return a.a_u8 && !a.c_f32 && a.M > 0 && a.N > 0 && a.K > 0 && a.K % 8 == 0 && a.lda % 8 == 0 && a.ldb % 8 == 0 && a.ldc >= a.N &&
           a.A && a.B && a.C && (uintptr_t)a.A % 16 == 0 && (uintptr_t)a.B % 16 == 0 && (uintptr_t)a.C % 16 == 0 && !a.resid && !a.gate &&
           a.act == 0 && a.dropout_p == 0.f && !a.self_resid && ((!a.rowadd && !a.grpadd) || a.rowadd_period > 0) &&
           (!a.grpadd || a.grp_index) && gemm_fast_form<64, 64>(a) && a.K % 64 == 0 && cdiv(a.M, 64) * cdiv(a.N, 64) < (1 << 20);
  };
  if (a0.dtype != a1.dtype || !plain(a0) || !plain(a1) || (begin && begin->sh_w && begin->sh_dtype != a0.dtype)) {
    int rc = begin ? mst_step_begin(begin, stream) : MST_OK;
    if (rc == MST_OK) rc = mst_gemm_nt(args0, stream);
    return rc != MST_OK ? rc : mst_gemm_nt(args1, stream);
  }
  StepBegin sb = {};
  int n_begin = 0;
  if (begin) {
    int64_t grid = 0;
    const int rc = pack_step_begin(*begin, sb, &grid);
    if (rc) return rc;
    n_begin = (int)((grid + 7) / 8 * 8);
  }
  hipStream_t s = (hipStream_t)stream;
  return dispatch_act(a0.dtype, [&](auto tag) -> int {
    typedef decltype(tag) T;
    const int64_t sh_tiles = sb.sh_w ? sb.sh_tiles : 0;
    if (a0.K >= 1024 && a1.K >= 1024 && gemm_fast_form<128, 128>(a0) && gemm_fast_form<128, 128>(a1)) {
      const int t0 = (int)((a0.M / 128) * (a0.N / 128)), t1 = (int)((a1.M / 128) * (a1.N / 128));
      const size_t lds_b = (size_t)2 * (128 + 128) * 64 * 2;
      static bool opted = false;
      if (!opted) {
        const hipError_t e = hipFuncSetAttribute(reinterpret_cast<const void*>(&gemm_nt_pair_kernel<T, 128, 128, 2, 2, 64, 4>),
                                                 hipFuncAttributeMaxDynamicSharedMemorySize, (int)lds_b);
        if (e != hipSuccess) { set_error("gemm_nt_pair_kernel: LDS opt-in of %zu bytes: %s", lds_b, hipGetErrorString(e)); return MST_ERR_LAUNCH; }
        opted = true;
      }
      hipLaunchKernelGGL((gemm_nt_pair_kernel<T, 128, 128, 2, 2, 64, 4>), dim3((unsigned)(n_begin + t0 + t1 + sh_tiles)), dim3(256), lds_b, s, a0, a1,
                         t0, t1, sb, n_begin);
      MST_CHECK_LAUNCH("gemm_nt_pair_kernel");
      return MST_OK;
    }
    const int tiles0 = (int)((a0.M / 64) * (a0.N / 64)), tiles1 = (int)((a1.M / 64) * (a1.N / 64));
    const size_t lds = (size_t)2 * (64 + 64) * 64 * 2;
    hipLaunchKernelGGL((gemm_nt_pair_kernel<T, 64, 64, 2, 2, 64, 1>), dim3((unsigned)(n_begin + tiles0 + tiles1 + sh_tiles)), dim3(256), lds, s, a0,
                       a1, tiles0, tiles1, sb, n_begin);
    MST_CHECK_LAUNCH("gemm_nt_pair_kernel");
    return MST_OK;
  });
}

#ifdef MST_FFN_STAMPS
extern "C" int mst_debug_ffn_stamps(uint64_t* host_out) {
  return hipMemcpyFromSymbol(host_out, HIP_SYMBOL(mst::g_ffn_stamps), sizeof(uint64_t) * (8 + 48 * 4)) == hipSuccess ? 0 : -1;
}
#endif
```

musicstyletransfer_amd/csrc/runtime.hip:

```cpp
#include <stdarg.h>
#include <string.h>
#include "common.hpp"

namespace mst {
static thread_local char g_err[512] = "";
void set_error(const char* fmt, ...) {
  va_list ap;
  va_start(ap, fmt);
  vsnprintf(g_err, sizeof(g_err), fmt, ap);
  va_end(ap);
}
}

using namespace mst;

extern "C" int mst_version(void) { return 105; }
extern "C" const char* mst_last_error(void) { return g_err; }

#define HIP_TRY(expr)                                             \
  do {                                                            \
    hipError_t e__ = (expr);                                      \
    if (e__ != hipSuccess) {                                      \
      set_error("%s: %s", #expr, hipGetErrorString(e__));         \
      return MST_ERR_LAUNCH;                                      \
    }                                                             \
  } while (0)

extern "C" int mst_graph_begin(mst_stream_t stream) {
  HIP_TRY(hipStreamBeginCapture((hipStream_t)stream, hipStreamCaptureModeThreadLocal));
  return MST_OK;
}
static hipError_t count_nodes(hipGraph_t g, int32_t* nodes_out, int32_t* kernel_nodes_out) {
  size_t n = 0;
  hipError_t e = hipGraphGetNodes(g, nullptr, &n);
  if (e != hipSuccess) return e;
  int32_t kernels = 0;
  if (n > 0 && kernel_nodes_out) {
    hipGraphNode_t* nodes = new hipGraphNode_t[n];
    e = hipGraphGetNodes(g, nodes, &n);
    for (size_t i = 0; e == hipSuccess && i < n; ++i) {
      hipGraphNodeType t;
      e = hipGraphNodeGetType(nodes[i], &t);
      kernels += (e == hipSuccess && t == hipGraphNodeTypeKernel);
    }
    delete[] nodes;
    if (e != hipSuccess) return e;
  }
  if (nodes_out) *nodes_out = (int32_t)n;
  if (kernel_nodes_out) *kernel_nodes_out = kernels;
  return hipSuccess;
}

extern "C" int mst_graph_end(mst_stream_t stream, void** graph_exec_out) {
  return mst_graph_end_counted(stream, graph_exec_out, nullptr, nullptr);
}
extern "C" int mst_graph_end_counted(mst_stream_t stream, void** graph_exec_out, int32_t* nodes_out, int32_t* kernel_nodes_out) {
  MST_CHECK_ARG(graph_exec_out != nullptr, "mst_graph_end: null output");
  hipGraph_t g = nullptr;
  HIP_TRY(hipStreamEndCapture((hipStream_t)stream, &g));
  hipError_t ec = (nodes_out || kernel_nodes_out) ? count_nodes(g, nodes_out, kernel_nodes_out) : hipSuccess;
  if (ec != hipSuccess) {
    (void)hipGraphDestroy(g);
    set_error("hipGraphGetNodes: %s", hipGetErrorString(ec));
    return MST_ERR_LAUNCH;
  }
  hipGraphExec_t ge = nullptr;
  hipError_t e = hipGraphInstantiate(&ge, g, nullptr, nullptr, 0);
  (void)hipGraphDestroy(g);
  if (e != hipSuccess) {
    set_error("hipGraphInstantiate: %s", hipGetErrorString(e));
    return MST_ERR_LAUNCH;
  }
  *graph_exec_out = (void*)ge;
  return MST_OK;
}
extern "C" int mst_graph_launch(void* graph_exec, mst_stream_t stream) {
  HIP_TRY(hipGraphLaunch((hipGraphExec_t)graph_exec, (hipStream_t)stream));
  return MST_OK;
}
extern "C" int mst_graph_destroy(void* graph_exec) {
  if (graph_exec) HIP_TRY(hipGraphExecDestroy((hipGraphExec_t)graph_exec));
  return MST_OK;
}

extern "C" int mst_event_create(void** ev_out) {
  MST_CHECK_ARG(ev_out != nullptr, "mst_event_create: null output");
  hipEvent_t ev;
  HIP_TRY(hipEventCreate(&ev));
  *ev_out = (void*)ev;
  return MST_OK;
}
extern "C" int mst_event_record(void* ev, mst_stream_t stream) {
  HIP_TRY(hipEventRecord((hipEvent_t)ev, (hipStream_t)stream));
  return MST_OK;
}
extern "C" int mst_event_sync(void* ev) {
  HIP_TRY(hipEventSynchronize((hipEvent_t)ev));
  return MST_OK;
}
extern "C" int mst_event_elapsed_ms(void* a, void* b, float* ms_out) {
  HIP_TRY(hipEventElapsedTime(ms_out, (hipEvent_t)a, (hipEvent_t)b));
  return MST_OK;
}
extern "C" int mst_event_destroy(void* ev) {
  if (ev) HIP_TRY(hipEventDestroy((hipEvent_t)ev));
  return MST_OK;
}

__global__ void selftest_kernel(int32_t* flags) {
  __shared__ __bf16 tile[32 * 32];
  const int l = threadIdx.x;
  auto Aval = [](int i, int k) { return (float)(((i * 3 + k * 5) % 7) - 3); };
  auto Bval = [](int k, int j) { return (float)(((k * 2 + j * 7) % 5) - 2); };

  {
    bf16x8 a, b;
    for (int j = 0; j < 8; ++j) {
      a[j] = (__bf16)Aval(l & 15, 8 * (l >> 4) + j);
      b[j] = (__bf16)Bval(8 * (l >> 4) + j, l & 15);
    }
    f32x4 d = {0, 0, 0, 0};
    d = __builtin_amdgcn_mfma_f32_16x16x32_bf16(a, b, d, 0, 0, 0);
    int ok = 1;
    for (int r = 0; r < 4; ++r) {
      int row = 4 * (l >> 4) + r, col = l & 15;
      float ref = 0;
      for (int k = 0; k < 32; ++k) ref += Aval(row, k) * Bval(k, col);
      ok &= (d[r] == ref);
    }
    ok = __all(ok);
    if (l == 0) flags[0] = ok;
  }
  f32x16 X;
  {
    bf16x8 a, b;
    for (int j = 0; j < 8; ++j) {
      a[j] = (__bf16)Aval(l & 31, 8 * (l >> 5) + j);
      b[j] = (__bf16)Bval(8 * (l >> 5) + j, l & 31);
    }
    f32x16 d;
    for (int r = 0; r < 16; ++r) d[r] = 0;
    d = __builtin_amdgcn_mfma_f32_32x32x16_bf16(a, b, d, 0, 0, 0);
    int ok = 1;
    for (int r = 0; r < 16; ++r) {
      int row = (r & 3) + 8 * (r >> 2) + 4 * (l >> 5), col = l & 31;
      float ref = 0;
      for (int k = 0; k < 16; ++k) ref += Aval(row, k) * Bval(k, col);
      ok &= (d[r] == ref);
    }
    ok = __all(ok);
    if (l == 0) flags[1] = ok;
    X = d;
  }
  auto Tval = [](int r, int c) { return (float)((r * 37 + c * 11) % 251); };
  for (int i = l; i < 32 * 32; i += 64) tile[i] = (__bf16)Tval(i / 32, i % 32);
  __syncthreads();
  {
    int g_i = l & 15, q = g_i >> 2, p = g_i & 3;
    int r0 = 8 + 4 * (l >> 5), c0 = 16 * ((l >> 4) & 1);
    const __bf16* addr = &tile[(r0 + q) * 32 + c0 + 4 * p];
    i16x4 v = __builtin_amdgcn_ds_read_tr16_b64_v4i16(
        (__attribute__((address_space(3))) i16x4*)(uintptr_t)(addr));
    int ok = 1;
    for (int e = 0; e < 4; ++e) {
      uint16_t bits = (uint16_t)v[e];
      float got = bits_to_f32<__bf16>(bits);
      ok &= (got == Tval(r0 + e, c0 + g_i));
    }
    ok = __all(ok);
// ... 38 lines not shown
```

musicstyletransfer_amd/engine.py:

```python
import math
import os
import warnings
from collections import OrderedDict, namedtuple

import numpy as np
import torch

from . import ops as o
from ._lib import CE_MAX_WORKGROUPS
from .ops import roundup


class VAEConfig:

    def __init__(self, kind, in_dim, out_dim, num_classes, latent_dim, e_model, e_layers, e_heads, d_model, d_layers,
                 d_heads, e_dropout=0.0, d_dropout=0.0, d_causal=False):
        assert kind in ("token", "pianoroll")
        assert e_model % e_heads == 0 and d_model % d_heads == 0
        self.kind = kind
        self.in_dim, self.out_dim = in_dim, out_dim
        self.num_classes, self.latent_dim = num_classes, latent_dim
        self.e_model, self.e_layers, self.e_heads = e_model, e_layers, e_heads
        self.d_model, self.d_layers, self.d_heads = d_model, d_layers, d_heads
        self.e_dropout, self.d_dropout = float(e_dropout), float(d_dropout)
# ... 194 lines not shown
                    raise RuntimeError(f"a one-launch position-0 tail failed on at least one rank (status words summed over the ranks: "
                                       f"{flags}, {skipped} skipped step(s)); the replicas are no longer identical — restart from the "
                                       "last checkpoint with MST_ROW_TAIL=0")
                cur = self.step_status[:2].tolist()
                self.handle_step_status(cur[0] or flags, cur[1] or skipped)
                handled = True
        if not self._poll_pending:
            self._poll_dev.copy_(self.step_status[:2])
            if reduce is not None:
                reduce(self._poll_dev)
            self._poll_host.copy_(self._poll_dev, non_blocking=True)
            self._poll_event.record()
            self._poll_pending = True
        return handled

    def read_metrics(self, reset=True):
        buf = self._metric_buf.cpu()
        acc = buf[:3].tolist()
        flags, skipped, nonfinite = buf[4:7].view(torch.int32).tolist()
        if nonfinite:
            self.nonfinite_steps += int(nonfinite)
            o.zero(self._metric_buf[6:7])
            warnings.warn(f"{int(nonfinite)} training step(s) skipped: a per-sample loss was not finite (an fp16 activation overflow or "
                          "sigma = 0 under log(sigma^2)); parameters, moments and the step count were left as they were", RuntimeWarning)
        if flags or skipped:
            self.handle_step_status(flags, skipped)
        out = {"kl_sum": acc[0], "total_sum": acc[1], "count": acc[2], "skipped_steps": skipped, "nonfinite_steps": int(nonfinite)}
        beta_t, _, f_lr, sched_t = buf[8:12].tolist()
        if sched_t > 0:
            out.update(kl_weight=beta_t, lr_scale=f_lr)
        if self.tok_parts is not None:
            t = self.tok_parts.cpu().double().sum(0).tolist()
            out.update(nll_sum=t[0], acc_hits=t[1], topk_hits=t[2], n_tokens=t[3])
        if reset:
            o.zero(self.metric_acc)
            if self.tok_parts is not None:
                o.zero(self.tok_parts)
        return out

    def wgrad_scratch(self, n_floats=16 * 1024 * 1024 + 256 * 256):
        for t in self._wgrad_scratch:
            if t.numel() >= n_floats:
                return t
        t = torch.empty(n_floats, dtype=torch.float32, device=self.device)
        self._wgrad_scratch.append(t)
        return t

    def _view(self, flat, name):
        shape = self.shapes[name]
        off = self.offsets[name]
        return flat[off: off + int(np.prod(shape))].view(*shape)

    def p(self, name):
        return self._view(self.w, name)

    def grad(self, name):
        return self._view(self.g, name)

    def h(self, name):
        return self._view(self.w16, name)

    def fused(self, flat, prefix, what):
        D = self.shapes[f"{prefix}.att.W_k.weight"][0]
        off = self.offsets[f"{prefix}.att.W_k.{what}"]
        return flat[off: off + 3 * D * D].view(3 * D, D) if what == "weight" else flat[off: off + 3 * D]

    def t(self, name):
        so, r, c = self.t_specs[name]
        off = self.t_off[name]
        return self.wt16[off: off + c * roundup(r, 8)].view(c, roundup(r, 8))

    def _layer_params(self, side, i):
        pre = f"{side}.layer{i}"

        def dense(name):
            w, b = f"{pre}.{name}.weight", f"{pre}.{name}.bias"
            return Dense(self.h(w), self.p(b), self.t(w), self.grad(w), self.grad(b))

        def norm(name):
            g, b = f"{pre}.{name}.gamma", f"{pre}.{name}.beta"
            return Norm(self.p(g), self.p(b), self.grad(g), self.grad(b), f"{pre}.{name}")

        kqv = Dense(self.fused(self.w16, pre, "weight"), self.fused(self.w, pre, "bias"), self.t(f"{pre}.att.W_kqv"),
                    self.fused(self.g, pre, "weight"), self.fused(self.g, pre, "bias"))
        dec = side == "decoder"
        return LayerParams(kqv, dense("att.W_proj"), dense("ff1"), dense("ff2"), norm("ln1"), norm("ln3" if dec else "ln2"),
                           self_resid=dec, mask_mode=2 if dec else 1)

    def layer(self, side, i):
        return self._layers[side, i]

    def load_numpy(self, params_np):
        host = np.zeros(self.n, np.float32)
        for name, shape in self.shapes.items():
            a = np.asarray(params_np[name], np.float32)
            assert tuple(a.shape) == tuple(shape), f"{name}: expected {shape}, got {a.shape}"
            host[self.offsets[name]: self.offsets[name] + a.size] = a.reshape(-1)
        self.w.copy_(torch.from_numpy(host))
        self.refresh_shadows()

    def to_numpy(self, which="w"):
        host = getattr(self, which).detach().cpu().numpy()
        return OrderedDict((n, host[self.offsets[n]: self.offsets[n] + int(np.prod(s))].reshape(s).copy())
                           for n, s in self.shapes.items())

    def shadowed_names(self):
        names = set()
        for key in self.t_specs:
            if key.endswith(".att.W_kqv"):
                p = key[: -len("W_kqv")]
                names.update({p + "W_k.weight", p + "W_q.weight", p + "W_v.weight"})
            else:
                names.add(key)
        return names

    def as_consumed_numpy(self):
        w = self.to_numpy("w")
        w16 = self.w16.detach().float().cpu().numpy()
        for n in self.shadowed_names():
            s = self.shapes[n]
            w[n] = w16[self.offsets[n]: self.offsets[n] + int(np.prod(s))].reshape(s).copy()
        return w

    def refresh_shadows(self):
        o.cast_to_act(self.w, self.w16)
        o.transpose_shadows(self.w, self.wt16, self.t_desc, self.t_prefix, len(self.t_specs), self.t_tiles)


class _Layer:
    pass


Dense = namedtuple("Dense", "w b t dw db")
Norm = namedtuple("Norm", "gamma beta dgamma dbeta site")
LayerParams = namedtuple("LayerParams", "kqv proj ff1 ff2 ln1 ln2 self_resid mask_mode")

Rows = namedtuple("Rows", "view c_remap ln")
ALL_ROWS = Rows(lambda buf: buf, (0, 0, 0), {})


def position0_rows(B, S):
    return Rows(lambda buf: buf.view(B, S, -1)[:, 0, :], (1, S, 0), dict(M=B, row_id_stride=S))


class Dropout(namedtuple("Dropout", "p seed_ptr site0")):

    def at(self, k):
        return dict(dropout_p=self.p, dropout_site=self.site0 + k, dropout_seed_ptr=self.seed_ptr) if self.p > 0 else {}


NO_DROPOUT = Dropout(0.0, None, 0)


def row_block_fwd(P, L, x_in, rows, drop, form, row_groups=None, tail=None):
    D, v = P.proj.w.shape[0], rows.view
    if form == "tail":
        o.row_tail_fwd(v(L.att), v(x_in), P.proj.w, P.proj.b, P.ln1.gamma, P.ln1.beta, P.ff1.w, P.ff1.b, P.ff2.w, P.ff2.b, P.ln2.gamma,
                       P.ln2.beta, v(L.h1), v(L.x1), v(L.a), v(L.h2), v(L.x2), L.mean1, L.rstd1, L.mean2, L.rstd2, dropout_p=drop.p,
                       dropout_seed_ptr=drop.seed_ptr, site0=drop.site0, **tail)
        return L.x2
    proj = dict(N=D, K=D, bias=P.proj.b, resid=v(x_in), **drop.at(0))
    ff1 = dict(K=D, bias=P.ff1.b, act=o.ACT_RELU, **drop.at(1))
    ff2 = dict(K=4 * D, bias=P.ff2.b, **drop.at(2))
    ff2.update(dict(self_resid=True) if P.self_resid else dict(resid=v(L.x1)))
    if form == "fused":
        head = dict(att=L.att, W=P.proj.w, h1=L.h1, gamma=P.ln1.gamma, beta=P.ln1.beta, mean=L.mean1, rstd=L.rstd1, **proj)
        o.ffn_ln_fwd(L.x1, P.ff1.w, L.a, P.ff2.w, L.h2, P.ln2.gamma, P.ln2.beta, L.x2, L.mean2, L.rstd2, ff1=ff1, ff2=ff2, proj=head,
                     row_groups=row_groups)
        return L.x2
    o.gemm_nt(v(L.att), P.proj.w, L.h1, c_remap=rows.c_remap, **proj)
    o.layernorm_fwd(v(L.h1), P.ln1.gamma, P.ln1.beta, v(L.x1), L.mean1, L.rstd1, D=D, **rows.ln)
    o.gemm_nt(v(L.x1), P.ff1.w, L.a, c_remap=rows.c_remap, **ff1)
    o.gemm_nt(v(L.a), P.ff2.w, L.h2, c_remap=rows.c_remap, **ff2)
    o.layernorm_fwd(v(L.h2), P.ln2.gamma, P.ln2.beta, v(L.x2), L.mean2, L.rstd2, D=D, **rows.ln)
    return L.x2


def _lead_mask(P, t, drop):
    if P.mask_mode == 2:
        return dict(mask_mode=2, **drop.at(2))
    return dict(mask_mode=1, dx_masked=t.dhm, **drop.at(2)) if drop.p > 0 else {}


def no_partials(norm, parts):
    return None


def row_block_bwd(P, L, t, dy, rows, drop, form, partials, dy_done=False, row_groups=None, tail=None):
    D, v = P.proj.w.shape[0], rows.view
    if form == "tail":
        o.row_tail_bwd(v(dy), v(L.h2), v(L.h1), v(L.a), L.mean1, L.rstd1, L.mean2, L.rstd2, P.ln1.gamma, P.ln2.gamma, P.ff2.t, P.ff1.t,
                       P.proj.t, t.dh, t.dhm, t.dx1, t.dh1m, t.dpre, v(t.dh1), v(t.datt), P.ln1.dgamma, P.ln1.dbeta, P.ln2.dgamma,
                       P.ln2.dbeta, dropout_p=drop.p, dropout_seed_ptr=drop.seed_ptr, site0=drop.site0, **tail)
        return t.dhm, t.dh1m
    M = L.h1.shape[0]
    lead = None
    if not dy_done and form == "fused" and P.mask_mode == 1:
        lead = dict(dy=dy, x=L.h2, gamma=P.ln2.gamma, mean=L.mean2, rstd=L.rstd2, dx=t.dh, dgamma=P.ln2.dgamma, dbeta=P.ln2.dbeta,
                    partials=partials(P.ln2, o.gemm_nt_ln_parts(M)), **_lead_mask(P, t, drop))
    elif not dy_done:
        mask = _lead_mask(P, t, drop)
        if P.mask_mode == 2:
            mask["dropout_site"] = drop.site0 + 2
        o.layernorm_bwd(v(L.h2), P.ln2.gamma, L.mean2, L.rstd2, v(dy), t.dh, P.ln2.dgamma, P.ln2.dbeta, D=D,
                        partials=partials(P.ln2, o.layernorm_bwd_parts(M, D)), **rows.ln, **mask)
    dff = t.dhm if (drop.p > 0 and not P.self_resid) else t.dh
    resid_ff = None if P.self_resid else t.dh
    inv_keep = 1.0 / (1.0 - drop.p) if drop.p > 0 else 1.0
    ln1 = dict(dx_masked=t.dh1m, mask_mode=1, **drop.at(0)) if drop.p > 0 else {}
    if form == "fused":
        n = M if row_groups is None else M // row_groups[1] * row_groups[0]
        o.ffn_ln_bwd(dff, P.ff2.t, t.dpre, L.a, P.ff1.t, t.dh1, L.h1, P.ln1.gamma, L.mean1, L.rstd1, P.ln1.dgamma, P.ln1.dbeta,
                     alpha=inv_keep, resid=resid_ff, partials=partials(P.ln1, o.gemm_nt_ln_parts(n)), lead=lead, row_groups=row_groups,
                     **ln1)
    else:
        o.gemm_nt(dff, P.ff2.t, t.dpre, N=4 * D, K=D, gate=v(L.a), alpha=inv_keep)
        if form == "ln_fused":
            o.gemm_nt_ln_bwd(t.dpre, P.ff1.t, t.dh1, L.h1, P.ln1.gamma, L.mean1, L.rstd1, P.ln1.dgamma, P.ln1.dbeta, N=D, K=4 * D,
                             resid=resid_ff, partials=partials(P.ln1, o.gemm_nt_ln_parts(M)), **ln1)
        else:
            o.gemm_nt(t.dpre, P.ff1.t, t.dx1, N=D, K=4 * D, resid=resid_ff)
            o.layernorm_bwd(v(L.h1), P.ln1.gamma, L.mean1, L.rstd1, t.dx1, v(t.dh1), P.ln1.dgamma, P.ln1.dbeta, D=D,
                            partials=partials(P.ln1, o.layernorm_bwd_parts(M, D)), **rows.ln, **ln1)
    dproj = t.dh1m if drop.p > 0 else v(t.dh1)
    o.gemm_nt(dproj, P.proj.t, t.datt, N=D, K=D, c_remap=rows.c_remap)
    return dff, dproj


def layer_wgrads(P, L, t, x_in, dff, dproj, rows):
    D, v = P.proj.w.shape[0], rows.view
    return [o.wgrad_problem(dff, v(L.a), P.ff2.dw, P.ff2.db, N=D, K=4 * D),
            o.wgrad_problem(t.dpre, v(L.x1), P.ff1.dw, P.ff1.db, N=4 * D, K=D),
            o.wgrad_problem(dproj, v(L.att), P.proj.dw, P.proj.db, N=D, K=D),
            o.wgrad_problem(t.dqkv, x_in, P.kqv.dw, P.kqv.db, N=3 * D, K=D)]


def row_tail_selfcheck(store, B=64, S=2):
    store.tail_checked = True
    cfg, dev, adt = store.cfg, store.device, store.act_dtype
    D, F = cfg.e_model, 4 * cfg.e_model
    if not (o.can_row_tail(B, D) and store.tail_fused and cfg.e_layers >= 1):
        return True
    f32 = dict(dtype=torch.float32, device=dev)
    P = store.layer("encoder", cfg.e_layers - 1)
    scratch = lambda n: n._replace(dgamma=torch.zeros(D, **f32), dbeta=torch.zeros(D, **f32))
    P = P._replace(ln1=scratch(P.ln1), ln2=scratch(P.ln2))

    def rnd(n, width, site):
        a = torch.zeros(n, width, **f32)
        o.randn(a, seed=0x7A11, site=site)
        t = torch.zeros(n, width, dtype=adt, device=dev)
        o.cast_to_act(a, t)
        return t

    z = lambda n, w: torch.zeros(n, w, dtype=adt, device=dev)
    att, xin = rnd(B * S, D, 1), rnd(B * S, D, 2)
    status = torch.zeros(2, dtype=torch.int32, device=dev)
    sync = torch.zeros(8, dtype=torch.int32, device=dev)
    rows = position0_rows(B, S)

    def fbufs():
        L = _Layer()
        L.att, L.h1, L.x1, L.a, L.h2, L.x2 = att, z(B * S, D), z(B * S, D), z(B * S, F), z(B * S, D), z(B * S, D)
        L.mean1, L.rstd1, L.mean2, L.rstd2 = (torch.zeros(B * S, **f32) for _ in range(4))
        return L

    u, f = fbufs(), fbufs()
    tail = dict(stat_stride=S, phys_stride=S, status=status[0:1])
    row_block_fwd(P, u, xin, rows, NO_DROPOUT, "launches")
    row_block_fwd(P, f, xin, rows, NO_DROPOUT, "tail", tail=dict(tail, sync=sync[0:3]))
    dy = rnd(B * S, D, 3)

    def bbufs():
        t = _Layer()
        t.dh, t.dhm, t.dx1, t.dh1m, t.dpre, t.dh1, t.datt = z(B, D), z(B, D), z(B, D), z(B, D), z(B, F), z(B * S, D), z(B * S, D)
        return t

    ub, fb = bbufs(), bbufs()
    row_block_bwd(P, u, ub, dy, rows, NO_DROPOUT, "launches", no_partials)
    row_block_bwd(P, u, fb, dy, rows, NO_DROPOUT, "tail", no_partials, tail=dict(tail, sync=sync[4:7]))
    torch.cuda.current_stream().synchronize()
    want_f, want_b = o.row_tail_barriers(D)
    sy, stv = sync.cpu().tolist(), status.cpu().tolist()
    why = []
    if stv[0]:
        why.append(f"status flags {stv[0]:#x}")
    if sy[0] != want_f or sy[4] != want_b:
        why.append(f"barrier counters {sy[0]} / {sy[4]} instead of {want_f} / {want_b}")
    ulp = 2.0 ** -7 if adt == torch.bfloat16 else 2.0 ** -10
    host = lambda t: t.float().cpu().numpy()
    for k in ("h1", "x1", "a", "h2", "x2"):
        a, b = host(rows.view(getattr(f, k))), host(rows.view(getattr(u, k)))
        if not np.all(np.abs(a - b) <= 4 * ulp * np.maximum(np.abs(b), 1.0)):
            why.append(f"forward {k}: max difference {np.abs(a - b).max():.3g}")
    for k in ("dh", "dpre", "dx1", "dh1", "datt"):
        a, b = host(getattr(fb, k)), host(getattr(ub, k))
        if not np.abs(a - b).max() <= 4 * ulp * max(float(np.abs(b).max()), 1e-6) + 1e-6:
            why.append(f"backward {k}: max difference {np.abs(a - b).max():.3g} (scale {np.abs(b).max():.3g})")
    if why:
        store.tail_fused = False
        warnings.warn("the one-launch position-0 tail failed its start-up check on this device (" + "; ".join(why) +
                      "): using the five-launch form", RuntimeWarning)
    return not why


Forms = namedtuple("Forms", "tails riders shadows fuse_bce bce_dgrad skip_row0 cls_fold ffn_e ffn_d ln_bwd_e ln_bwd_d sched")


def check_schedule(kl_warmup_steps=0, kl_cycle_steps=0, kl_free_bits=0.0, lr_warmup_steps=0):
    for name, val in (("kl_warmup_steps", kl_warmup_steps), ("kl_cycle_steps", kl_cycle_steps), ("lr_warmup_steps", lr_warmup_steps)):
        if int(val) != val or val < 0:
            raise ValueError(f"{name} must be a non-negative integer, not {val!r}")
    if not kl_free_bits >= 0:
        raise ValueError(f"kl_free_bits must be >= 0 nats per sample, not {kl_free_bits!r}")
    if kl_cycle_steps > 0 and kl_warmup_steps == 0:
        raise ValueError("kl_cycle_steps restarts the KL warm-up: it needs kl_warmup_steps > 0")
    if kl_cycle_steps > 0 and kl_warmup_steps > kl_cycle_steps:
        raise ValueError(f"kl_warmup_steps ({kl_warmup_steps}) must not exceed kl_cycle_steps ({kl_cycle_steps})")


def schedule_values(t, kl_weight=1.0, kl_warmup_steps=0, kl_cycle_steps=0, lr_warmup_steps=0):
    f_lr = min(1.0, t / lr_warmup_steps) if lr_warmup_steps > 0 else 1.0
    u = (t - 1) % kl_cycle_steps + 1 if kl_cycle_steps > 0 else t
    ramp = min(1.0, u / kl_warmup_steps) if kl_warmup_steps > 0 else 1.0
    return float(np.float32(float(np.float32(kl_weight)) * ramp)), f_lr


class StepPlan:

    def __init__(self, store, B, T, lr=3e-4, clip_gradient=1.0, kl_weight=1.0, label_smoothing=0.0,
                 negative_label_downscaling=False, global_batch=None, gscale=None, want_probs=False, seed=0,
                 internal_eps=False, optimizer_params=None, sample_offset=0, site_base=0,
                 kl_warmup_steps=0, kl_cycle_steps=0, kl_free_bits=0.0, lr_warmup_steps=0):
        cfg = store.cfg
        self.store, self.cfg, self.B, self.T = store, cfg, B, T
        self.dev, self.adt = store.device, store.act_dtype
        self.lr, self.clip, self.kl_weight = lr, clip_gradient, kl_weight
        check_schedule(kl_warmup_steps, kl_cycle_steps, kl_free_bits, lr_warmup_steps)
        self.schedule = dict(kl_warmup_steps=int(kl_warmup_steps), kl_cycle_steps=int(kl_cycle_steps), kl_free_bits=float(kl_free_bits),
                             lr_warmup_steps=int(lr_warmup_steps))
        self.scheduled = any(self.schedule.values())
        self.ls, self.nld = label_smoothing, negative_label_downscaling
        self.global_batch = global_batch or B
        self.sample_offset, self.site_base = int(sample_offset), int(site_base)
        if (self.sample_offset * cfg.latent_dim) % 2:
            raise ValueError("sample_offset * latent_dim must be even (eps is drawn in Box-Muller pairs)")
        self.gscale = gscale if gscale is not None else (1024.0 if self.adt == torch.float16 else 1.0)
        self.gscale_enc = 1.0
        self.want_probs, self.internal_eps = want_probs, internal_eps
        self.opt = dict(beta1=0.9, beta2=0.999, eps=1e-8, wd=0.0)
        if optimizer_params:
            for k_src, k_dst in (("beta1", "beta1"), ("beta2", "beta2"), ("epsilon", "eps"), ("wd", "wd")):
                if k_src in optimizer_params:
                    self.opt[k_dst] = float(optimizer_params[k_src])
        dev, adt = self.dev, self.adt
        De, Dd, Z = cfg.e_model, cfg.d_model, cfg.latent_dim
        Se, Sd = T, T + 1
        self.Me, self.Md = B * Se, B * Sd
        f32 = dict(dtype=torch.float32, device=dev)

        def act(rows, width):
            return torch.zeros(rows, roundup(width, 8), dtype=adt, device=dev)

        self.ride = (cfg.kind != "token" and cfg.d_layers >= 1 and cfg.e_layers >= 1 and Dd in (128, 256) and
                     o.can_ride(B * T, 3 * Dd, Dd, T) and o.can_ride(B * T, Dd, 3 * Dd, T))
        self.shadows_on_tail = True
        self.forms = self._resolve_forms()
        if cfg.kind == "token":
            seg = [("tokens", B * T * 4), ("labels", B * T * 4)]
        else:
            self.ld_roll = roundup(cfg.in_dim + (cfg.num_classes if self.forms.cls_fold else 0), 8)
            seg = [("roll", B * T * self.ld_roll), ("labels", B * T * cfg.out_dim)]
        seg += [("seq_lens", B * 4), ("classes", B * 4)]
        self.in_layout, off = {}, 0
        for name, nbytes in seg:
            self.in_layout[name] = (off, nbytes)
            off = roundup(off + nbytes, 16)
        self.own_inbuf = torch.zeros(off, dtype=torch.uint8, device=dev)
        self.bind_inputs(self.own_inbuf)
        self.eps = torch.zeros(B, Z, **f32)
        self.rng_state = store.rng_state(seed)
        self._outers = []

        self.pos_e = torch.from_numpy(positional_table(De, Se)).to(dev)
        self.pos_d = torch.from_numpy(positional_table(Dd, Sd)).to(dev)
        self.keymask_e = torch.zeros(B, Se, dtype=torch.uint8, device=dev)
        self.keymask_d = torch.zeros(B, Sd, dtype=torch.uint8, device=dev)

        def layers(n, M, D, H, S):
            out = []
            for _ in range(n):
                L = _Layer()
                L.qkv, L.att, L.h1, L.x1 = act(M, 3 * D), act(M, D), act(M, D), act(M, D)
                L.a, L.h2, L.x2 = act(M, 4 * D), act(M, D), act(M, D)
                L.lse = torch.zeros(2, B, H, S, **f32)
                L.mean1, L.rstd1 = torch.zeros(M, **f32), torch.zeros(M, **f32)
                L.mean2, L.rstd2 = torch.zeros(M, **f32), torch.zeros(M, **f32)
                out.append(L)
            return out

        self.x0_e = act(self.Me, De)
        self.enc = layers(cfg.e_layers, self.Me, De, cfg.e_heads, Se)
        self.x0_d = act(self.Md, Dd)
        self.dec = layers(cfg.d_layers, self.Md, Dd, cfg.d_heads, Sd)
        self.mu, self.sigma, self.z = torch.zeros(B, Z, **f32), torch.zeros(B, Z, **f32), torch.zeros(B, Z, **f32)
        self.kl, self.total = torch.zeros(B, **f32), torch.zeros(B, **f32)
        nb4 = (B + 3) // 4 * 4
        self._recon_buf = torch.zeros(nb4 + 8 + 24 + 64, **f32)
        self.recon = self._recon_buf[:B]
        self.sync_words = self._recon_buf[nb4: nb4 + 8].view(torch.int32)
        self.ride_queues = self._recon_buf[nb4 + 32:].view(torch.int32)
        self.metric_acc = store.metric_acc
        self.track_token_metrics = False
        self.logits = None if self.forms.fuse_bce else act(B * T, cfg.out_dim)
        self.dlogits = act(B * T, cfg.out_dim)
        if cfg.kind == "token":
            self.probs = torch.zeros(B * T, cfg.out_dim, **f32) if want_probs else None
        else:
            self.probs = act(B * T, cfg.out_dim) if want_probs else None
        self.npos = torch.zeros(B, dtype=torch.int32, device=dev)

        def bwd_bufs(M, D, H, S):
            t = _Layer()
            t.dx_a, t.dx_b = act(M, D), act(M, D)
            t.dh, t.dhm = act(M, D), act(M, D)
            t.dh1, t.dh1m = act(M, D), act(M, D)
            t.dpre, t.dx1 = act(M, 4 * D), act(M, D)
            t.datt, t.dqkv = act(M, D), act(M, 3 * D)
            t.delta = torch.zeros(B, H, S, **f32)
            return t

        self.be_l = [bwd_bufs(self.Me, De, cfg.e_heads, Se) for _ in range(cfg.e_layers)]
        self.bd_l = [bwd_bufs(self.Md, Dd, cfg.d_heads, Sd) for _ in range(cfg.d_layers)]
        self._wgrads = []
        self.wgrad_scratch = store.wgrad_scratch()
        self._ln_part, self._psums = {}, []
        for side, n_l, M, D in (("encoder", cfg.e_layers, self.Me, De), ("decoder", cfg.d_layers, self.Md, Dd)):
            rows = max(o.layernorm_bwd_parts(M, D), o.gemm_nt_ln_parts(M))
            for i in range(n_l):
                for ln in ("ln1", "ln2" if side == "encoder" else "ln3"):
                    self._ln_part[f"{side}.layer{i}.{ln}"] = torch.zeros(rows, 2 * D, **f32)
        self.lat_scratch = torch.zeros(B * (Dd + 2 * Z), **f32)
        self.d_dec_out = act(self.Md, Dd)
        self.d_enc_out = act(self.Me, De)
        c = _Layer()
        c.dh, c.dhm, c.dx1, c.dh1m = act(B, De), act(B, De), act(B, De), act(B, De)
        c.dpre = act(B, 4 * De)
        self.sp_dh1 = c.dh1 = act(self.Me, De)
        self.sp_datt = c.datt = act(self.Me, De)
        c.dqkv, c.delta = self.be_l[-1].dqkv, self.be_l[-1].delta
        self.top = c
        self.graph = None
        self.graph_late = None
        self.graph_opt = None
        self._tick_adam = False
        self._infer = False
        self._tail_used = dict(fwd=False, bwd=False)
        if o.can_row_tail(B, De) and store.tail_fused and not store.tail_checked:
            row_tail_selfcheck(store)

    @property
    def e_p(self):
        return 0.0 if self._infer else self.cfg.e_dropout

    @property
    def d_p(self):
        return 0.0 if self._infer else self.cfg.d_dropout

    def _resolve_forms(self):
        cfg, st, B, T = self.cfg, self.store, self.B, self.T
        De, Dd = cfg.e_model, cfg.d_model
        roll = cfg.kind == "pianoroll"
        tails = bool(o.can_row_tail(B, De) and st.tail_fused)
        riders = bool(self.ride and tails)
        shadows = "own" if not st.shadows_deferred else ("tail" if self.shadows_on_tail and riders else "begin")
        fuse_bce = roll and o.can_fuse_bce(cfg.out_dim, T, self.nld) and o.bce_fusion_pays(cfg.out_dim)
        ffn_d, ln_bwd_d = o.ffn_fusion_pays(Dd, 4 * Dd), o.ln_bwd_fusion_pays(Dd)
        return Forms(
            tails=tails, riders=riders, shadows=shadows, fuse_bce=fuse_bce,
            bce_dgrad=fuse_bce and ln_bwd_d,
            skip_row0=cfg.d_layers > 0 and T % 64 == 0 and ffn_d,
            cls_fold=(roll and cfg.in_dim % 8 == 0 and roundup(cfg.in_dim + cfg.num_classes, 256) == roundup(cfg.in_dim, 256) and
                      st.offsets["encoder.class2hid.weight"] == st.offsets["encoder.embedding.weight"] + cfg.in_dim * De),
            ffn_e=o.ffn_fusion_pays(De, 4 * De), ffn_d=ffn_d, ln_bwd_e=o.ln_bwd_fusion_pays(De), ln_bwd_d=ln_bwd_d,
            sched=self.scheduled)

    def _guard(self):
        fwd, bwd = o.row_tail_barriers(self.cfg.e_model)
        exp = []
        if self._tail_used["fwd"]:
            exp.append((self.sync_words[0:1], fwd))
        if self._tail_used["bwd"]:
            exp.append((self.sync_words[4:5], bwd))
        g = dict(status=self.store.step_status, expect=exp)
        if self.global_batch == self.B:
            g["finite"] = (self.recon, self.kl)
        return g

    def bind_inputs(self, buf):
        cfg, B, T = self.cfg, self.B, self.T
        need = max(a + n for a, n in self.in_layout.values())
        if not (buf.dtype == torch.uint8 and buf.is_contiguous() and buf.is_cuda and buf.data_ptr() % 16 == 0 and buf.numel() >= need):
            raise ValueError("bind_inputs: need a contiguous, 16-byte aligned device uint8 blob of pack_batch()'s size")
        self.inbuf = buf

        def inview(name, dtype, *shape):
            a, n = self.in_layout[name]
            return buf[a: a + n].view(dtype).view(*shape)

        if cfg.kind == "token":
            self.tokens = inview("tokens", torch.int32, B, T)
            self.labels = inview("labels", torch.int32, B, T)
        else:
            self.roll_cls = inview("roll", torch.uint8, B * T, self.ld_roll)
            self.roll = self.roll_cls[:, : roundup(cfg.in_dim, 8)]
            self.labels = inview("labels", torch.uint8, B * T, cfg.out_dim)
        self.seq_lens = inview("seq_lens", torch.int32, B)
        self.classes = inview("classes", torch.int32, B)

    def load_batch(self, x, seq_lens, classes, labels, eps=None):
        def dev(a, dtype):
            t = torch.as_tensor(np.asarray(a)) if not torch.is_tensor(a) else a
            return t.to(device=self.dev, dtype=dtype, non_blocking=True)

        cfg, B, T = self.cfg, self.B, self.T
        if cfg.kind == "token":
            self.tokens.copy_(dev(x, torch.int32).view(B, T))
            self.labels.copy_(dev(labels, torch.int32).view(B, T))
        else:
            self.roll[:, : cfg.in_dim].copy_(dev(x, torch.uint8).view(B * T, cfg.in_dim))
            self.labels.copy_(dev(labels, torch.uint8).view(B * T, cfg.out_dim))
        self.seq_lens.copy_(dev(seq_lens, torch.int32))
        self.classes.copy_(dev(classes, torch.int32))
        if self.forms.cls_fold:
            w = self.ld_roll - cfg.in_dim
            onehot = (self.classes.view(B, 1).to(torch.int64) == torch.arange(w, device=self.dev).view(1, w)).to(torch.uint8)
            self.roll_cls.view(B, T, -1)[:, :, cfg.in_dim:].copy_(onehot.view(B, 1, w).expand(B, T, w))
        if eps is not None:
            self.eps.copy_(dev(eps, torch.float32))

    def pack_into(self, blob, x, seq_lens, classes, labels):
        cfg, B, T = self.cfg, self.B, self.T
        assert blob.dtype == torch.uint8 and not blob.is_cuda and blob.numel() >= self.inbuf.numel()
        raw = blob.numpy()

        def seg(name, dtype, *shape):
            a, n = self.in_layout[name]
            return raw[a: a + n].view(dtype).reshape(*shape)

        def as_np(a):
            return a.cpu().numpy() if torch.is_tensor(a) else np.asarray(a)

        if cfg.kind == "token":
            np.copyto(seg("tokens", np.int32, B, T), as_np(x).reshape(B, T), casting="unsafe")
            np.copyto(seg("labels", np.int32, B, T), as_np(labels).reshape(B, T), casting="unsafe")
        else:
            ldp = self.ld_roll
            roll = seg("roll", np.uint8, B * T, ldp)
            np.copyto(roll[:, : cfg.in_dim], as_np(x).reshape(B * T, cfg.in_dim), casting="unsafe")
            if self.forms.cls_fold:
                w = ldp - cfg.in_dim
                roll.reshape(B, T, ldp)[:, :, cfg.in_dim:] = (as_np(classes).reshape(B, 1, 1).astype(np.int64) ==
                                                              np.arange(w).reshape(1, 1, w)).astype(np.uint8)
            elif ldp != cfg.in_dim:
                roll[:, cfg.in_dim:] = 0
            np.copyto(seg("labels", np.uint8, B * T, cfg.out_dim), as_np(labels).reshape(B * T, cfg.out_dim), casting="unsafe")
        np.copyto(seg("seq_lens", np.int32, B), as_np(seq_lens).reshape(B), casting="unsafe")
        np.copyto(seg("classes", np.int32, B), as_np(classes).reshape(B), casting="unsafe")
        return blob

    def pack_batch(self, x, seq_lens, classes, labels):
        return self.pack_into(torch.zeros(self.inbuf.numel(), dtype=torch.uint8), x, seq_lens, classes, labels)

    def load_packed(self, blob):
        self.inbuf.copy_(blob, non_blocking=True)

    def _drop(self, p, site):
        return dict(dropout_p=p, dropout_site=site, dropout_seed_ptr=self.rng_state) if p > 0 else {}

    def _dropout(self, p, site0):
        return Dropout(p, self.rng_state if p > 0 else None, site0)

    def _site_e(self, i):
        return self.site_base + 3 * i

    def _site_d(self, i):
        return self.site_base + 3 * (self.cfg.e_layers + i)

    def _late_shadows(self):
        st = self.store
        return dict(w=st.w, wt16=st.wt16, desc=st.t_desc_late, prefix=st.t_prefix_late, n_mat=st.t_n_late, tiles=st.t_tiles_late)

    def _top_encoder_layer_fwd(self, i, L, x_in):
        cfg, st, B, S, F = self.cfg, self.store, self.B, self.T, self.forms
        D, H = cfg.e_model, cfg.e_heads
        P = st.layer("encoder", i)
        o.attn_qkv_fwd(x_in, P.kqv.w, P.kqv.b, L.qkv, self.keymask_e, L.lse, L.att, B, S, H, D // H, 0, D, 2 * D, q_limit=1)
        self._tail_used["fwd"] = F.tails
        tail = None
        if F.tails:
            tail = dict(sync=self.sync_words[0:3], stat_stride=S, phys_stride=S, status=st.step_status[0:1], queue=self.ride_queues[0:1])
            if F.riders:
                Pd, Dd, Sd = st.layer("decoder", 0), cfg.d_model, S + 1
                tail["rider"] = dict(A=self.x0_d, B=Pd.kqv.w, C_out=self.dec[0].qkv, M=B * S, N=3 * Dd, K=Dd, bias=Pd.kqv.b,
                                     a_remap=(S, Sd, 1), c_remap=(S, Sd, 1))
                if F.shadows == "tail":
                    tail["shadows"] = self._late_shadows()
        return row_block_fwd(P, L, x_in, position0_rows(B, S), self._dropout(self.e_p, self._site_e(i)),
                             "tail" if F.tails else "launches", tail=tail)

    def _layer_fwd(self, side, i, L, x_in, keymask, D, H, S, p, site0):
        F = self.forms
        dh = D // H
        if side == "encoder" and i == self.cfg.e_layers - 1:
            return self._top_encoder_layer_fwd(i, L, x_in)
        P = self.store.layer(side, i)
        causal = side == "decoder" and self.cfg.d_causal
        if side == "decoder" and i == 0 and F.riders:
            (o.attn_causal_fwd if causal else o.attn_fwd)(L.qkv, keymask, L.lse, L.att, self.B, S, H, dh, 0, D, 2 * D)
        elif causal:
            o.gemm_nt(x_in, P.kqv.w, L.qkv, N=3 * D, K=D, bias=P.kqv.b)
            o.attn_causal_fwd(L.qkv, keymask, L.lse, L.att, self.B, S, H, dh, 0, D, 2 * D)
        else:
            o.attn_qkv_fwd(x_in, P.kqv.w, P.kqv.b, L.qkv, keymask, L.lse, L.att, self.B, S, H, dh, 0, D, 2 * D)
        fused = F.ffn_e if side == "encoder" else F.ffn_d
        return row_block_fwd(P, L, x_in, ALL_ROWS, self._dropout(p, site0), "fused" if fused else "launches",
                             row_groups=self._row0_groups(side, i))

    def _row0_groups(self, side, i):
        if side == "decoder" and i == self.cfg.d_layers - 1 and self.forms.skip_row0:
            return (self.T, self.T + 1, 1)
        return None

    def forward(self, inference=False, upto=None):
        if upto not in (None, "latent") or (upto and not inference):
            raise ValueError("forward(upto=...) takes 'latent', in inference mode only")
        cfg, st, B, T = self.cfg, self.store, self.B, self.T
        self._infer = bool(inference)
        F = self.forms = self._resolve_forms()
        self._tail_used = dict(fwd=False, bwd=False)
        De, Dd = cfg.e_model, cfg.d_model
        Se, Sd = T, T + 1
        sq_e, sq_d = math.sqrt(float(De)), math.sqrt(float(Dd))
        self._wgrads, self._psums, self._outers = [], [], []
        need_rng = self.e_p > 0 or self.d_p > 0 or self.internal_eps
        rng = st.rng_state_inference() if self._infer else self.rng_state
        tick = self._tick_adam and not self._infer
        begin = dict(rng_state=rng if need_rng else None,
                     adam_state=st.step_state if tick else None, lr=self.lr, beta1=self.opt["beta1"],
                     beta2=self.opt["beta2"], eps_out=self.eps if self.internal_eps else None,
                     eps_index0=self.sample_offset * cfg.latent_dim, lens=self.seq_lens,
                     mask_e=self.keymask_e if cfg.kind != "token" else None, add_e=0, mask_d=self.keymask_d, add_d=1,
                     zero_a=self._recon_buf, zero_b=st.g if tick else None)
        if F.shadows == "begin":
            begin["shadows"] = self._late_shadows()
        if F.sched and tick:
            begin["schedule"] = dict(block=st.sched, kl_weight=self.kl_weight, **self.schedule)
        ride = cfg.kind != "token"
        if not ride:
            o.step_begin(**begin)
        if cfg.kind == "token":
            o.embed_fwd(self.tokens, st.p("encoder.embedding.weight"), self.pos_e, self.x0_e.view(B, Se, -1), 0, sq_e,
                        classes=self.classes, cls_table=st.p("encoder.class2hid.weight"), keymask=self.keymask_e)
        else:
            o.gemm_nt_pair(dict(A=self.roll, B=st.t("encoder.embedding.weight"), C_out=self.x0_e, N=De, alpha=sq_e,
                                grpadd=st.p("encoder.class2hid.weight"), grp_index=self.classes, rowadd=self.pos_e, rowadd_period=T),
                           dict(A=self.roll, B=st.t("decoder.embedding.weight"), C_out=self.x0_d, M=B * T, N=Dd, alpha=sq_d,
                                rowadd=self.pos_d[1:], rowadd_period=T, c_remap=(T, Sd, 1)),
                           begin=begin if ride else None)
        x = self.x0_e
        for i, L in enumerate(self.enc):
            x = self._layer_fwd("encoder", i, L, x, self.keymask_e, De, cfg.e_heads, Se, self.e_p, self._site_e(i))
        self.enc_out = x
        lat = (x.view(B, Se, -1), st.p("encoder.latent_proj.weight"), st.p("encoder.latent_proj.bias"), self.eps,
               st.p("decoder.latent2hid.weight"), st.p("decoder.latent2hid.bias"), self.classes,
               st.p("decoder.class2hid.weight"), self.pos_d, sq_d, self.mu, self.sigma, self.z, self.kl,
               self.x0_d.view(B, Sd, -1))
        proj0 = None
        if F.riders:
            Pd = st.layer("decoder", 0)
            proj0 = (Pd.kqv.w, Pd.kqv.b, self.dec[0].qkv.view(B, Sd, -1))
        o.latent_fwd(*lat, proj=proj0)
        if upto == "latent":
            return
        if cfg.kind == "token":
            o.embed_fwd(self.tokens, st.p("decoder.embedding.weight"), self.pos_d, self.x0_d.view(B, Sd, -1), 1, sq_d)
        x = self.x0_d
        site_d = self._site_d(0)
        for i, L in enumerate(self.dec):
            x = self._layer_fwd("decoder", i, L, x, self.keymask_d, Dd, cfg.d_heads, Sd, self.d_p, site_d + 3 * i)
        self.dec_out = x
        if not F.fuse_bce:
            o.gemm_nt(x, st.h("decoder.output_layer.weight"), self.logits, M=B * T, K=Dd, bias=st.p("decoder.output_layer.bias"),
                      a_remap=(T, Sd, 1))

    def losses(self, with_grad=True, combine=True):
        cfg, B, T, F = self.cfg, self.B, self.T, self.forms
        dl = self.dlogits if with_grad else None
        if cfg.kind == "token":
            o.softmax_ce(self.logits, self.labels, self.recon, B, T, cfg.out_dim, probs=self.probs, dlogits=dl,
                         gscale=self.gscale, pre_zeroed=True,
                         tok_parts=self.store.tok_parts if self.track_token_metrics else None)
        elif F.fuse_bce:
            dgrad = None
            if with_grad and F.bce_dgrad:
                last, Dd, Sd = cfg.d_layers - 1, cfg.d_model, T + 1
                dgrad = dict(A=self.dlogits, B=self.store.t("decoder.output_layer.weight"), dX_out=self.bd_l[last].dh, M=B * T, N=Dd,
                             K=self.dlogits.shape[1], c_remap=(T, Sd, 1),
                             **self._out_ln_bwd("decoder", last, self.dec[last], cfg.d_dropout, self._site_d(0) + 3 * last,
                                                self.bd_l[last], B * T))
            o.gemm_sigmoid_bce(self.dec_out, self.store.h("decoder.output_layer.weight"), self.labels, self.recon, T, dgrad=dgrad,
                               dlogits=dl, probs=self.probs, label_smoothing=self.ls, downweight=self.nld, gscale=self.gscale, M=B * T,
                               K=cfg.d_model, bias=self.store.p("decoder.output_layer.bias"), a_remap=(T, T + 1, 1))
        else:
            o.sigmoid_bce(self.logits, self.labels, self.recon, B, T, cfg.out_dim, label_smoothing=self.ls,
                          downweight=self.nld, npos=self.npos, probs=self.probs, dlogits=dl, gscale=self.gscale,
                          pre_zeroed=True)
        if combine:
            o.loss_combine(self.recon, self.kl, self.kl_weight, self.total, self.metric_acc, guard=self._guard())

    LN_PARTIALS_MIN = 32

    def _ln_partials(self, norm, parts):
        if parts < self.LN_PARTIALS_MIN:
            return None
        buf, dg, db = self._ln_part[norm.site], norm.dgamma, norm.dbeta
        D = dg.numel()
        if db.data_ptr() == dg.data_ptr() + 4 * D:
            self._psums.append(o.partial_sum_job(buf, parts, dg, length=2 * D))
        else:
            self._psums += [o.partial_sum_job(buf, parts, dg, length=D), o.partial_sum_job(buf, parts, db, col_off=D, length=D)]
        return buf

    def _flush_grads(self):
        o.gemm_wgrad_batch(self._wgrads, scratch=self.wgrad_scratch, sums=self._psums, outers=self._outers)
        self.last_wgrad_launch = (self._wgrads, self._psums)
        self._wgrads, self._psums, self._outers = [], [], []

    def _out_ln_bwd(self, side, i, L, p, site0, t, M):
        P = self.store.layer(side, i)
        return dict(x=L.h2, gamma=P.ln2.gamma, mean=L.mean2, rstd=L.rstd2, dgamma=P.ln2.dgamma, dbeta=P.ln2.dbeta,
                    partials=self._ln_partials(P.ln2, o.gemm_nt_ln_parts(M)), **_lead_mask(P, t, self._dropout(p, site0)))

    def _layer_bwd(self, side, i, L, x_in, dy, dx_in, keymask, D, H, S, p, site0, t, dy_done=False, next_ln=None, ride=False):
        F, P = self.forms, self.store.layer(side, i)
        ffn, ln = (F.ffn_e, F.ln_bwd_e) if side == "encoder" else (F.ffn_d, F.ln_bwd_d)
        dff, dproj = row_block_bwd(P, L, t, dy, ALL_ROWS, self._dropout(p, site0), "fused" if ffn else ("ln_fused" if ln else "launches"),
                                   self._ln_partials, dy_done=dy_done, row_groups=self._row0_groups(side, i))
        if side == "decoder" and self.cfg.d_causal:
            o.attn_causal_bwd(L.qkv, keymask, L.lse, t.datt, t.dqkv, t.delta, self.B, S, H, D // H, 0, D, 2 * D)
        else:
            o.attn_bwd(L.qkv, keymask, L.lse, t.datt, t.dqkv, t.delta, self.B, S, H, D // H, 0, D, 2 * D)
        handed = None
        if next_ln is not None:
            kw, t_below = next_ln
            o.gemm_nt_ln_bwd(t.dqkv, P.kqv.t, t_below.dh, N=D, K=3 * D, resid=t.dh1, **kw)
        elif ride:
            T_ = self.T
            handed = (dict(A=t.dqkv, B=P.kqv.t, C_out=dx_in, M=self.B * T_, N=D, K=3 * D, resid=t.dh1, resid_phys=True,
                           a_remap=(T_, T_ + 1, 1), c_remap=(T_, T_ + 1, 1)),
                      (t.dqkv.view(self.B, S, -1), P.kqv.t, t.dh1.view(self.B, S, -1)))
        else:
            o.gemm_nt(t.dqkv, P.kqv.t, dx_in, N=D, K=3 * D, resid=t.dh1)
        self._wgrads += layer_wgrads(P, L, t, x_in, dff, dproj, ALL_ROWS)
        return handed

    def _top_encoder_layer_bwd(self, i, L, x_in, dx_in, next_ln=None, rider=None):
        cfg, st, B, S, F = self.cfg, self.store, self.B, self.T, self.forms
        D, H = cfg.e_model, cfg.e_heads
        P, c, rows = st.layer("encoder", i), self.top, position0_rows(B, S)
        self._tail_used["bwd"] = F.tails
        tail = None
        if F.tails:
            tail = dict(sync=self.sync_words[4:7], stat_stride=S, phys_stride=S, status=st.step_status[0:1], rider=rider,
                        queue=self.ride_queues[32:33])
        dff, dproj = row_block_bwd(P, L, c, self.d_enc_out, rows, self._dropout(cfg.e_dropout, self._site_e(i)),
                                   "tail" if F.tails else "launches", no_partials, tail=tail)
        o.attn_bwd(L.qkv, self.keymask_e, L.lse, c.datt, c.dqkv, c.delta, B, S, H, D // H, 0, D, 2 * D, q_limit=1)
        if next_ln is not None:
            kw, t_below = next_ln
            o.gemm_nt_ln_bwd(c.dqkv, P.kqv.t, t_below.dh, N=D, K=3 * D, resid=c.dh1, **kw)
        else:
            o.gemm_nt(c.dqkv, P.kqv.t, dx_in, N=D, K=3 * D, resid=c.dh1)
        self._wgrads += layer_wgrads(P, L, c, x_in, dff, dproj, rows)

    def backward(self):
        self.backward_early(flush=False)
        self.backward_late()

    def grad_cut(self):
        cfg, st = self.cfg, self.store
        if cfg.e_layers < 2:
            return 0
        return st.offsets[f"encoder.layer{cfg.e_layers - 1}.att.W_k.weight"]

    def _below(self, side, i, fuse):
        if not (fuse and i > 0):
            return None
        if side == "encoder":
            layers, bufs, p, site0, M = self.enc, self.be_l, self.cfg.e_dropout, self._site_e(i - 1), self.Me
        else:
            layers, bufs, p, site0, M = self.dec, self.bd_l, self.cfg.d_dropout, self._site_d(i - 1), self.Md
        return self._out_ln_bwd(side, i - 1, layers[i - 1], p, site0, bufs[i - 1], M), bufs[i - 1]

    def backward_early(self, flush):
        cfg, st, B, T, F = self.cfg, self.store, self.B, self.T, self.forms
        De, Dd = cfg.e_model, cfg.d_model
        Se, Sd = T, T + 1
        sq_d = math.sqrt(float(Dd))
        ldv = self.dlogits.shape[1]
        site_d = self._site_d(0)
        last = cfg.d_layers - 1
        if F.bce_dgrad:
            pass
        elif F.ln_bwd_d:
            o.gemm_nt_ln_bwd(self.dlogits, st.t("decoder.output_layer.weight"), self.bd_l[last].dh, M=B * T, N=Dd, K=ldv,
                             c_remap=(T, Sd, 1),
                             **self._out_ln_bwd("decoder", last, self.dec[last], cfg.d_dropout, site_d + 3 * last, self.bd_l[last], B * T))
        else:
            o.gemm_nt(self.dlogits, st.t("decoder.output_layer.weight"), self.d_dec_out, M=B * T, N=Dd, K=ldv, c_remap=(T, Sd, 1))
        self._wgrads.append(o.wgrad_problem(self.dlogits, self.dec_out, st.grad("decoder.output_layer.weight"),
                                            st.grad("decoder.output_layer.bias"), M=B * T, N=cfg.out_dim, K=Dd, b_remap=(T, Sd, 1)))
        dy, pingpong, handed = self.d_dec_out, (self.bd_l[0].dx_a, self.bd_l[0].dx_b), None
        for n, i in enumerate(reversed(range(cfg.d_layers))):
            x_in = self.dec[i - 1].x2 if i > 0 else self.x0_d
            handed = self._layer_bwd("decoder", i, self.dec[i], x_in, dy, pingpong[n % 2], self.keymask_d, Dd, cfg.d_heads, Sd,
                                     cfg.d_dropout, site_d + 3 * i, self.bd_l[i], dy_done=F.ln_bwd_d,
                                     next_ln=self._below("decoder", i, F.ln_bwd_d), ride=F.riders and i == 0)
            dy = pingpong[n % 2]
        d_x0_d = dy
        rider, dx0 = handed or (None, None)
        if cfg.kind == "token":
            o.embed_bwd(self.tokens, st.grad("decoder.embedding.weight"), d_x0_d.view(B, Sd, -1), 1, sq_d)
        else:
            self._wgrads.append(o.wgrad_problem(self.roll, d_x0_d, st.grad("decoder.embedding.weight"), M=B * T, N=cfg.out_dim,
                                                K=Dd, scale=sq_d, b_remap=(T, Sd, 1)))
        d_enc = self.d_enc_out
        o.latent_bwd_vec(st.p("encoder.latent_proj.weight"), self.eps, st.p("decoder.latent2hid.weight"), self.classes, self.mu,
                         self.sigma, d_x0_d.view(B, Sd, -1), sq_d, self.kl_weight, self.gscale_enc,
                         st.grad("decoder.class2hid.weight"), d_enc.view(B, Se, -1), self.lat_scratch,
                         enc_scale=self.gscale_enc / self.gscale, proj=dx0, sched=(st.sched, self.kl) if F.sched else None)
        self._outers += o.latent_outer_jobs(self.lat_scratch, self.enc_out.view(B, Se, -1), self.z,
                                            st.grad("encoder.latent_proj.weight"), st.grad("encoder.latent_proj.bias"),
                                            st.grad("decoder.latent2hid.weight"), st.grad("decoder.latent2hid.bias"))
        top = cfg.e_layers - 1
        x_in = self.enc[top - 1].x2 if top > 0 else self.x0_e
        self._top_encoder_layer_bwd(top, self.enc[top], x_in, self.be_l[0].dx_a, next_ln=self._below("encoder", top, F.ln_bwd_e),
                                    rider=rider)
        if flush and cfg.e_layers >= 2:
            self._flush_grads()

    def backward_late(self):
        cfg, st, B, T, F = self.cfg, self.store, self.B, self.T, self.forms
        De, Se = cfg.e_model, T
        sq_e = math.sqrt(float(De))
        dy, pingpong = self.be_l[0].dx_a, (self.be_l[0].dx_b, self.be_l[0].dx_a)
        for n, i in enumerate(reversed(range(cfg.e_layers - 1))):
            x_in = self.enc[i - 1].x2 if i > 0 else self.x0_e
            self._layer_bwd("encoder", i, self.enc[i], x_in, dy, pingpong[n % 2], self.keymask_e, De, cfg.e_heads, Se, cfg.e_dropout,
                            self._site_e(i), self.be_l[i], dy_done=F.ln_bwd_e, next_ln=self._below("encoder", i, F.ln_bwd_e))
            dy = pingpong[n % 2]
        d_x0_e = dy
        if cfg.kind == "token":
            o.embed_bwd(self.tokens, st.grad("encoder.embedding.weight"), d_x0_e.view(B, Se, -1), 0, sq_e,
                        classes=self.classes, dcls=st.grad("encoder.class2hid.weight"))
        else:
            self._wgrads.append(o.wgrad_problem(self.roll_cls, d_x0_e, st.grad("encoder.embedding.weight"), M=B * T,
                                                N=cfg.in_dim + (cfg.num_classes if F.cls_fold else 0), K=De, scale=sq_e))
            if not F.cls_fold:
                o.group_colsum(d_x0_e.view(B, Se, -1), T, De, 0, self.classes, st.grad("encoder.class2hid.weight"), sq_e)
        self._flush_grads()

    def optimizer(self):
        st = self.store
        deferred = self.forms.shadows != "own"
        sched = st.sched if self.forms.sched else None
        clip = self.clip if self.clip is not None else -1.0
        guard = self._guard()
        mt = dict(recon=self.recon, kl=self.kl, kl_weight=self.kl_weight, total=self.total, metric=self.metric_acc, **guard)
        emb = (lambda base: dict(base=base, specs=st.emb_specs, wt16=st.wt16)) if deferred else (lambda base: None)
        if self.gscale == self.gscale_enc:
            o.adam_flat(st.w, st.g, st.m, st.v, st.w16, st.step_state, lr=self.lr,
                        rescale=1.0 / (self.global_batch * self.gscale), clip=clip, advance_step=False, metrics=mt, emb=emb(0),
                        sched=sched, **self.opt)
        else:
            cut = st.offsets["decoder.latent2hid.weight"]
            rng = [(0, cut, self.gscale_enc, False), (cut, st.n, self.gscale, False)]
            for a, b, gs, adv in rng:
                o.adam_flat(st.w[a:b], st.g[a:b], st.m[a:b], st.v[a:b], st.w16[a:b], st.step_state, lr=self.lr,
                            rescale=1.0 / (self.global_batch * gs), clip=clip, advance_step=adv,
                            metrics=mt if a == 0 else (guard or None), emb=emb(a), sched=sched if a == 0 else None, **self.opt)
        if not deferred:
            o.transpose_shadows(st.w, st.wt16, st.t_desc, st.t_prefix, len(st.t_specs), st.t_tiles)

    def fwd_bwd_kernels(self, is_train=True):
        self._tick_adam = is_train
        self.forward()
        self.losses(with_grad=is_train, combine=not is_train)
        if is_train:
            self.backward()

    def step_kernels(self, is_train=True, reduce_fn=None):
        self.fwd_bwd_kernels(is_train)
        if is_train:
            if reduce_fn is not None:
                reduce_fn(self.store.g)
            self.optimizer()

    def capture(self, is_train=True, split_optimizer=False, overlap=False):
        self.is_train, self.split = is_train, split_optimizer
        self.graph_late = None
        if is_train and split_optimizer and overlap and self.grad_cut() > 0:
            def early():
                self._tick_adam = True
                self.forward()
                self.losses(with_grad=True, combine=False)
                self.backward_early(flush=True)
            self.graph = o.Graph().capture(early)
            self.graph_late = o.Graph().capture(self.backward_late)
            self.graph_opt = o.Graph().capture(self.optimizer)
        elif split_optimizer or not is_train:
            self.graph = o.Graph().capture(lambda: self.fwd_bwd_kernels(is_train))
            self.graph_opt = o.Graph().capture(self.optimizer) if is_train else None
        else:
            self.graph = o.Graph().capture(lambda: self.step_kernels(True))
            self.graph_opt = None
        return self

    def graph_nodes(self):
        gs = [g for g in (self.graph, self.graph_late, self.graph_opt) if g is not None]
        return sum(g.nodes for g in gs), sum(g.kernel_nodes for g in gs)

    def run(self, reduce_fn=None, reducer=None, stamps=None):
        if self.graph is None:
            raise RuntimeError("call capture() first")
        self.graph.launch()
        if self.graph_late is not None:
            g, cut = self.store.g, self.grad_cut()
            pending = [reducer.start(g[cut:])] if reducer is not None else []
            self.graph_late.launch()
            if stamps is not None:
                stamps[0].record()
            if reducer is not None:
                pending.append(reducer.start(g[:cut]))
                reducer.finish(pending)
            elif reduce_fn is not None:
                reduce_fn(g)
            if stamps is not None:
                stamps[1].record()
            self.graph_opt.launch()
            return
        if self.graph_opt is not None:
            if stamps is not None:
                stamps[0].record()
            if reducer is not None:
                reducer.finish([reducer.start(self.store.g)])
            elif reduce_fn is not None:
                reduce_fn(self.store.g)
            if stamps is not None:
                stamps[1].record()
            self.graph_opt.launch()

    def metrics(self, reset=True):
        m = self.store.read_metrics(reset)
        n = max(m["count"], 1.0)
        return {"kl_loss": m["kl_sum"] / n, "total_loss": m["total_sum"] / n, "count": m["count"], "nonfinite_steps": m["nonfinite_steps"],
                "kl_weight": m.get("kl_weight", self.kl_weight) if self.scheduled else self.kl_weight,
                "lr_scale": m.get("lr_scale", 1.0) if self.scheduled else 1.0}
```

musicstyletransfer_amd/ops.py:

```python
import ctypes as C
import math

import torch

from . import _lib
from ._lib import LnArgs, LnBwdIn, PartialSum, OuterJob, StepBeginArgs, StepMetrics, ACT_NONE, ACT_RELU, MST_BF16, MST_F16, GemmArgs, WgradArgs, call

_DT = {torch.bfloat16: MST_BF16, torch.float16: MST_F16}


def dt(x):
    try:
        return _DT[x if isinstance(x, torch.dtype) else x.dtype]
    except KeyError:
        raise TypeError(f"activation dtype must be bfloat16 or float16, got {x}") from None


def ptr(t):
    if t is None:
        return None
    assert t.is_cuda, "mst ops need device tensors (there is no CPU fallback)"
    if t.device.index != torch.cuda.current_device():
        raise RuntimeError(f"tensor on cuda:{t.device.index} but the current device is cuda:{torch.cuda.current_device()}: "
                           "call torch.cuda.set_device() for this rank's GPU first")
# ... 31 lines not shown
    g.act = act
    g.gate, g.ldg = ptr(gate), (ld(gate) if gate is not None else 0)
    g.alpha = alpha
    g.rowadd, g.ldra = ptr(rowadd), (ld(rowadd) if rowadd is not None else 0)
    g.rowadd_period = rowadd_period
    g.grpadd, g.ldga = ptr(grpadd), (ld(grpadd) if grpadd is not None else 0)
    g.grp_index = ptr(grp_index)
    g.a_rows_per_group, g.a_group_stride, g.a_group_offset = a_remap
    g.c_rows_per_group, g.c_group_stride, g.c_group_offset = c_remap
    g.dropout_p, g.dropout_seed, g.dropout_site = dropout_p, dropout_seed, dropout_site
    g.self_resid = 1 if self_resid else 0
    g.resid_phys = 1 if resid_phys else 0
    g.dropout_seed_ptr = ptr(dropout_seed_ptr)
    return g


def gemm_nt(A, B, C_out, **kw):
    call("mst_gemm_nt", C.byref(_gemm_args(A, B, C_out, **kw)), stream())


def gemm_nt_form(A, B, C_out, **kw):
    rc = _lib.load().mst_gemm_nt_form(C.byref(_gemm_args(A, B, C_out, **kw)))
    if rc < 0:
        _lib.check(rc, "mst_gemm_nt_form")
    return rc


def gemm_nt_pair(first, second, begin=None):
    if begin is None:
        call("mst_gemm_nt_pair", C.byref(_gemm_args(**first)), C.byref(_gemm_args(**second)), stream())
    else:
        call("mst_gemm_nt_pair_begin", C.byref(_gemm_args(**first)), C.byref(_gemm_args(**second)), C.byref(_step_begin_args(**begin)),
             stream())


def can_ride(M, N, K, T=0):
    return M % 128 == 0 and N % 128 == 0 and K % 64 == 0 and (T == 0 or T % 128 == 0)


def can_row_tail(B, D):
    return D in (128, 256) and 0 < B <= 64


def row_tail_barriers(D):
    return 3 * (D // 16), 2 * (D // 16)


def row_tail_fwd(att, resid, Wp, bp, g1, be1, W1, b1, W2, b2, g2, be2, h1, x1, a, h2, x2, mean1, rstd1, mean2, rstd2, sync, stat_stride,
                 phys_stride, eps=1e-5, dropout_p=0.0, dropout_seed_ptr=None, site0=0, status=None, rider=None, queue=None, shadows=None):
    assert sync.numel() >= 3 and (rider is None or queue is not None) and (shadows is None or rider is not None)
    q = _lib.RowTailArgs()
    q.dtype, q.B, q.D = dt(att), att.shape[0], Wp.shape[0]
    q.att, q.rs_att, q.resid, q.rs_res = ptr(att), att.stride(0), ptr(resid), resid.stride(0)
    q.Wp, q.ldwp, q.bp, q.g1, q.be1 = ptr(Wp), ld(Wp), ptr(bp), ptr(g1), ptr(be1)
    q.W1, q.ldw1, q.b1, q.W2, q.ldw2, q.b2, q.g2, q.be2 = ptr(W1), ld(W1), ptr(b1), ptr(W2), ld(W2), ptr(b2), ptr(g2), ptr(be2)
    assert h1.stride(0) == x1.stride(0) == h2.stride(0) == x2.stride(0)
    q.h1, q.x1, q.h2, q.x2, q.rs_d, q.a, q.rs_a = ptr(h1), ptr(x1), ptr(h2), ptr(x2), h1.stride(0), ptr(a), a.stride(0)
    q.mean1, q.rstd1, q.mean2, q.rstd2, q.stat_stride = ptr(mean1), ptr(rstd1), ptr(mean2), ptr(rstd2), stat_stride
    q.eps, q.dropout_p, q.dropout_seed, q.dropout_seed_ptr, q.site0 = eps, dropout_p, 0, ptr(dropout_seed_ptr), site0
    q.phys_stride, q.sync, q.status = phys_stride, ptr(sync), ptr(status)
    if shadows is not None:
        call("mst_row_tail_fwd_ride_shadows", C.byref(q), C.byref(_gemm_args(**rider)), ptr(queue), dt(shadows["wt16"]), ptr(shadows["w"]),
             ptr(shadows["wt16"]), ptr(shadows["desc"]), ptr(shadows["prefix"]), shadows["n_mat"], shadows["tiles"], stream())
    elif rider is not None:
        call("mst_row_tail_fwd_ride", C.byref(q), C.byref(_gemm_args(**rider)), ptr(queue), stream())
    else:
        call("mst_row_tail_fwd", C.byref(q), stream())


def row_tail_bwd(dy, h2, h1, a, mean1, rstd1, mean2, rstd2, g1, g2, W2t, W1t, Wpt, dh, dhm, dx1, dh1m, dpre, dh1, datt, dg1, db1, dg2, db2,
                 sync, stat_stride, phys_stride, dropout_p=0.0, dropout_seed_ptr=None, site0=0, status=None, rider=None, queue=None):
    assert sync.numel() >= 3 and (rider is None or queue is not None)
    q = _lib.RowTailBwdArgs()
    q.dtype, q.B, q.D = dt(dy), dy.shape[0], Wpt.shape[0]
    q.dy, q.rs_dy = ptr(dy), dy.stride(0)
    assert h2.stride(0) == h1.stride(0)
    q.h2, q.h1, q.rs_d, q.a, q.rs_a = ptr(h2), ptr(h1), h2.stride(0), ptr(a), a.stride(0)
    q.mean1, q.rstd1, q.mean2, q.rstd2, q.stat_stride = ptr(mean1), ptr(rstd1), ptr(mean2), ptr(rstd2), stat_stride
    q.g1, q.g2 = ptr(g1), ptr(g2)
    q.W2t, q.ldw2t, q.W1t, q.ldw1t, q.Wpt, q.ldwpt = ptr(W2t), ld(W2t), ptr(W1t), ld(W1t), ptr(Wpt), ld(Wpt)
    assert dh.stride(0) == dhm.stride(0) == dx1.stride(0) == dh1m.stride(0)
    q.dh, q.dhm, q.dx1, q.dh1m, q.rs_c = ptr(dh), ptr(dhm), ptr(dx1), ptr(dh1m), dh.stride(0)
    q.dpre, q.rs_dpre, q.dh1, q.rs_dh1, q.datt, q.rs_datt = ptr(dpre), dpre.stride(0), ptr(dh1), dh1.stride(0), ptr(datt), datt.stride(0)
    q.dg1, q.db1, q.dg2, q.db2 = ptr(dg1), ptr(db1), ptr(dg2), ptr(db2)
    q.dropout_p, q.dropout_seed, q.dropout_seed_ptr, q.site0 = dropout_p, 0, ptr(dropout_seed_ptr), site0
    q.phys_stride, q.sync, q.status = phys_stride, ptr(sync), ptr(status)
    if rider is not None:
        call("mst_row_tail_bwd_ride", C.byref(q), C.byref(_gemm_args(**rider)), ptr(queue), stream())
    else:
        call("mst_row_tail_bwd", C.byref(q), stream())


def can_fuse_bce(P, T, downweight=False):
    return (P == 128 or (P % 256 == 0 and (P == 256 or not downweight))) and T % 64 == 0


def bce_fusion_pays(P):
    return P <= 256


def _gemm_bce_args(A, B, labels, loss, T, dlogits=None, probs=None, logits=None, label_smoothing=0.0, downweight=False, gscale=1.0, **kw):
    g = _gemm_args(A, B, dlogits if dlogits is not None else A, N=B.shape[0], **kw)
    if dlogits is None:
        g.C, g.ldc = None, 0
    q = _lib.BceArgs()
    q.labels, q.T, q.label_smoothing, q.downweight, q.loss = ptr(labels), T, label_smoothing, 1 if downweight else 0, ptr(loss)
    q.probs, q.ldp = ptr(probs), (ld(probs) if probs is not None else 0)
    q.logits, q.ldl = ptr(logits), (ld(logits) if logits is not None else 0)
    q.gscale = gscale
    return g, q


def gemm_sigmoid_bce(A, B, labels, loss, T, dgrad=None, **kw):
    g, q = _gemm_bce_args(A, B, labels, loss, T, **kw)
    if dgrad is None:
        call("mst_gemm_sigmoid_bce", C.byref(g), C.byref(q), stream())
    else:
        g2, l = _gemm_ln_bwd_args(**dgrad)
        call("mst_gemm_sigmoid_bce_dgrad_ln", C.byref(g), C.byref(q), C.byref(g2), C.byref(l), stream())


def can_fuse_ln(D):
    return D in (128, 256)


def ln_bwd_fusion_pays(D):
    return D == 128


def gemm_nt_ln_fwd(A, B, H_out, gamma, beta, Y_out, mean, rstd, eps=1e-5, **kw):
    g = _gemm_args(A, B, H_out, **kw)
    l = LnArgs()
    l.mode, l.gamma, l.beta, l.eps = 1, ptr(gamma), ptr(beta), eps
    l.out, l.ld_out = ptr(Y_out), ld(Y_out)
    l.mean, l.rstd = ptr(mean), ptr(rstd)
    call("mst_gemm_nt_ln", C.byref(g), C.byref(l), stream())


def can_fuse_ffn(D, F):
    return D in (128, 256) and F % D == 0


def ffn_fusion_pays(D, F):
    return can_fuse_ffn(D, F)


def _row_groups(n_rows, row_groups):
    rpg, stride, off = row_groups
    assert n_rows % stride == 0 and rpg % 64 == 0 and off + rpg <= stride
    return (n_rows // stride) * rpg, (rpg, stride, off)


def ffn_ln_fwd(x, W1, a_out, W2, h_out, gamma, beta, y_out, mean, rstd, eps=1e-5, ff1=None, ff2=None, proj=None, row_groups=None):
    ff1, ff2 = dict(ff1 or {}), dict(ff2 or {})
    if row_groups is not None:
        M, remap = _row_groups(x.shape[0], row_groups)
        ff1.update(M=M, a_remap=remap)
        ff2.update(M=M)
        if proj is not None:
            proj = dict(proj, M=M)
    g1 = _gemm_args(x, W1, a_out, **ff1)
    g2 = _gemm_args(a_out, W2, h_out, **ff2)
    l = LnArgs()
    l.mode, l.gamma, l.beta, l.eps = 1, ptr(gamma), ptr(beta), eps
    l.out, l.ld_out = ptr(y_out), ld(y_out)
    l.mean, l.rstd = ptr(mean), ptr(rstd)
    if proj is None:
        call("mst_ffn_ln_fwd", C.byref(g1), C.byref(g2), C.byref(l), stream())
        return
    kw = {k: v for k, v in proj.items() if k not in ("att", "W", "h1", "gamma", "beta", "mean", "rstd")}
    g0 = _gemm_args(proj["att"], proj["W"], proj["h1"], **kw)
    l0 = LnArgs()
    l0.mode, l0.gamma, l0.beta, l0.eps = 1, ptr(proj["gamma"]), ptr(proj["beta"]), eps
    l0.out, l0.ld_out = ptr(x), ld(x)
    l0.mean, l0.rstd = ptr(proj["mean"]), ptr(proj["rstd"])
    call("mst_proj_ffn_ln_fwd", C.byref(g0), C.byref(l0), C.byref(g1), C.byref(g2), C.byref(l), stream())


def ffn_ln_bwd(dff, W2t, dpre_out, gate, W1t, dx_out, x, gamma, mean, rstd, dgamma, dbeta, alpha=1.0, dx_masked=None, mask_mode=0,
               partials=None, lead=None, row_groups=None, **kw):
    rg = {}
    if row_groups is not None:
        M, remap = _row_groups(dff.shape[0], row_groups)
        rg, kw = dict(M=M, a_remap=remap), dict(kw, M=M)
    g1 = _gemm_args(dff, W2t, dpre_out, gate=gate, alpha=alpha, **rg)
    g2 = _gemm_args(dpre_out, W1t, dx_out, **kw)
    l = LnArgs()
    l.mode, l.gamma = 2, ptr(gamma)
    l.mean, l.rstd = ptr(mean), ptr(rstd)
    l.x, l.ld_x = ptr(x), ld(x)
    l.dgamma, l.dbeta = ptr(dgamma), ptr(dbeta)
    l.out, l.ld_out = ptr(dx_masked), (ld(dx_masked) if dx_masked is not None else 0)
    l.mask_mode = mask_mode
    l.partials = ptr(partials)
    if partials is not None:
        assert partials.shape[0] >= gemm_nt_ln_parts(g1.M) and partials.shape[1] == 2 * g2.N and partials.is_contiguous()
    if lead is None:
        call("mst_ffn_ln_bwd", C.byref(g1), C.byref(g2), C.byref(l), stream())
        return
    q = LnBwdIn()
    q.dy, q.ld_dy = ptr(lead["dy"]), ld(lead["dy"])
    q.x, q.ld_x = ptr(lead["x"]), ld(lead["x"])
    q.gamma, q.mean, q.rstd = ptr(lead["gamma"]), ptr(lead["mean"]), ptr(lead["rstd"])
    q.dx, q.ld_dx = ptr(lead["dx"]), ld(lead["dx"])
    dxm = lead.get("dx_masked")
    q.dx_masked, q.ld_dxm = ptr(dxm), (ld(dxm) if dxm is not None else 0)
    q.dgamma, q.dbeta, q.partials = ptr(lead.get("dgamma")), ptr(lead.get("dbeta")), ptr(lead.get("partials"))
    q.mask_mode = 1 if dxm is not None else 0
    q.dropout_p, q.dropout_seed = lead.get("dropout_p", 0.0), lead.get("dropout_seed", 0)
    q.dropout_seed_ptr, q.dropout_site = ptr(lead.get("dropout_seed_ptr")), lead.get("dropout_site", 0)
    if lead.get("partials") is not None:
        assert lead["partials"].shape[0] >= gemm_nt_ln_parts(g1.M) and lead["partials"].shape[1] == 2 * g2.N
    call("mst_ffn_ln_bwd_lead", C.byref(q), C.byref(g1), C.byref(g2), C.byref(l), stream())


def gemm_nt_ln_bwd(A, B, dX_out, x, gamma, mean, rstd, dgamma, dbeta, dx_masked=None, mask_mode=0, partials=None, **kw):
    g, l = _gemm_ln_bwd_args(A, B, dX_out, x, gamma, mean, rstd, dgamma, dbeta, dx_masked, mask_mode, partials, **kw)
    call("mst_gemm_nt_ln", C.byref(g), C.byref(l), stream())


def _gemm_ln_bwd_args(A, B, dX_out, x, gamma, mean, rstd, dgamma, dbeta, dx_masked=None, mask_mode=0, partials=None, **kw):
    g = _gemm_args(A, B, dX_out, **kw)
    l = LnArgs()
    l.mode, l.gamma = 2, ptr(gamma)
    l.mean, l.rstd = ptr(mean), ptr(rstd)
    l.x, l.ld_x = ptr(x), ld(x)
    l.dgamma, l.dbeta = ptr(dgamma), ptr(dbeta)
    l.out, l.ld_out = ptr(dx_masked), (ld(dx_masked) if dx_masked is not None else 0)
    l.mask_mode = mask_mode
    l.partials = ptr(partials)
    if partials is not None:
        assert partials.shape[0] >= gemm_nt_ln_parts(g.M) and partials.shape[1] == 2 * g.N and partials.is_contiguous()
    return g, l


def gemm_nt_ln_parts(M):
    return int(_lib.load().mst_gemm_nt_ln_parts(M))


def layernorm_bwd_parts(M, D):
    return int(_lib.load().mst_layernorm_bwd_parts(M, D))


PARTIAL_SUM_MAX_JOBS = 20


def partial_sum_job(src, n_parts, dst, scale=1.0, col_off=0, length=None):
    j = PartialSum()
    length = dst.numel() if length is None else length
    assert src.dtype == dst.dtype and src.element_size() == 4 and src.shape[0] >= n_parts
    j.src = src.data_ptr() + 4 * col_off
    j.n_parts, j.stride, j.len = n_parts, src.stride(0), length
    j.dst, j.scale = ptr(dst), scale
    return j


def partial_sums(jobs):
    for i in range(0, len(jobs), PARTIAL_SUM_MAX_JOBS):
        chunk = jobs[i:i + PARTIAL_SUM_MAX_JOBS]
        call("mst_partial_sums", (PartialSum * len(chunk))(*chunk), len(chunk), stream())


def wgrad_problem(A, B, dW, db=None, M=None, N=None, K=None, scale=1.0, a_remap=(0, 0, 0), b_remap=(0, 0, 0)):
    w = WgradArgs()
    w.a_u8 = 1 if A.dtype == torch.uint8 else 0
    w.dtype = dt(B if w.a_u8 else A)
    w.M = A.shape[0] if M is None else M
    w.N = dW.shape[0] if N is None else N
    w.K = dW.shape[1] if K is None else K
    w.A, w.lda = ptr(A), ld(A)
    w.B, w.ldb = ptr(B), ld(B)
    w.dW, w.ldw = ptr(dW), ld(dW)
    w.db = ptr(db)
    w.scale = scale
    w.a_rows_per_group, w.a_group_stride, w.a_group_offset = a_remap
    w.b_rows_per_group, w.b_group_stride, w.b_group_offset = b_remap
    return w


WGRAD_MAX_PROBLEMS = 16
OUTER_MAX_JOBS = 2


def outer_job(L, R, out, obias=None):
    q = OuterJob()
    assert L.dtype == torch.float32 and L.is_contiguous() and out.dtype == torch.float32 and out.is_contiguous() and R.stride(1) == 1
    q.L, q.R, q.r_stride = ptr(L), ptr(R), R.stride(0)
    q.r_dtype = 2 if R.dtype == torch.float32 else dt(R)
    q.B, q.J, q.I = L.shape[0], L.shape[1], R.shape[1]
    assert out.numel() == q.J * q.I and R.shape[0] == q.B and (obias is None or obias.numel() == q.J)
    q.out, q.obias = ptr(out), ptr(obias)
    return q


def outer_jobs(jobs):
    for i in range(0, len(jobs), OUTER_MAX_JOBS):
        chunk = jobs[i:i + OUTER_MAX_JOBS]
        call("mst_outer_jobs", (OuterJob * len(chunk))(*chunk), len(chunk), stream())


def gemm_wgrad_batch(problems, scratch=None, sums=None, outers=None):
    sums, outers = list(sums or []), list(outers or [])
    for i in range(0, len(problems), WGRAD_MAX_PROBLEMS):
        chunk = problems[i:i + WGRAD_MAX_PROBLEMS]
        take, tko = [], []
        if i + WGRAD_MAX_PROBLEMS >= len(problems):
            take, sums = sums[:PARTIAL_SUM_MAX_JOBS], sums[PARTIAL_SUM_MAX_JOBS:]
            tko, outers = outers[:OUTER_MAX_JOBS], outers[OUTER_MAX_JOBS:]
        call("mst_gemm_wgrad_batch_flush", (WgradArgs * len(chunk))(*chunk), len(chunk), ptr(scratch),
             (scratch.numel() * scratch.element_size() if scratch is not None else 0),
             (PartialSum * len(take))(*take) if take else None, len(take),
             (OuterJob * len(tko))(*tko) if tko else None, len(tko), stream())
    if sums:
        partial_sums(sums)
    if outers:
        outer_jobs(outers)


def gemm_wgrad_plan(problems, scratch_bytes=0):
    plan = (C.c_int64 * (4 + WGRAD_MAX_PROBLEMS))()
    call("mst_gemm_wgrad_plan", (WgradArgs * len(problems))(*problems), len(problems), scratch_bytes, plan)
    return dict(form=plan[0], narrow=plan[1], items=plan[2], two_pass=plan[3], splits=list(plan[4:4 + len(problems)]))


def gemm_wgrad(A, B, dW, db=None, **kw):
    gemm_wgrad_batch([wgrad_problem(A, B, dW, db, **kw)])


def attn_fwd(qkv, keymask, lse, out, B, S, H, dh, k_off, q_off, v_off, q_limit=0):
    call("mst_attn_keysoftmax_fwd", dt(qkv), B, S, H, dh, ptr(qkv), ld(qkv), k_off, q_off, v_off, ptr(keymask),
         ptr(lse), ptr(out), ld(out), q_limit, stream())


def attn_qkv_fwd(x, W, bias, qkv, keymask, lse, out, B, S, H, dh, k_off, q_off, v_off, q_limit=0):
    call("mst_attn_qkv_fwd", dt(qkv), B, S, H, dh, ptr(x), ld(x), ptr(W), ld(W), ptr(bias), ptr(qkv), ld(qkv), k_off, q_off, v_off,
         ptr(keymask), ptr(lse), ptr(out), ld(out), q_limit, stream())


def attn_bwd(qkv, keymask, lse, dout, dqkv, delta, B, S, H, dh, k_off, q_off, v_off, q_limit=0):
    call("mst_attn_keysoftmax_bwd", dt(qkv), B, S, H, dh, ptr(qkv), ld(qkv), k_off, q_off, v_off, ptr(keymask),
         ptr(lse), ptr(dout), ld(dout), ptr(dqkv), ld(dqkv), ptr(delta), q_limit, stream())


def attn_causal_fwd(qkv, keymask, lse, out, B, S, H, dh, k_off, q_off, v_off):
    call("mst_attn_causal_fwd", dt(qkv), B, S, H, dh, ptr(qkv), ld(qkv), k_off, q_off, v_off, ptr(keymask), ptr(lse), ptr(out),
         ld(out), stream())


def attn_causal_bwd(qkv, keymask, lse, dout, dqkv, delta, B, S, H, dh, k_off, q_off, v_off):
# ... 352 lines not shown
```

Measured before the change: 26.10 million frames/s.

## Fuse last decoder layer forward, output BCE loss and its backward into one kernel

Adds a dec_tail kernel that runs, per 64-row tile, the last decoder layer's projection+FFN+LayerNorm forward, the output GEMM with sigmoid BCE, the output dgrad with LN backward, and the FFN backward. Intermediate activations stay in LDS, so the boundaries between these stages no longer go through global memory or separate launches. It only applies when D=128, F=512, 128 pitches and the tile count fits the CU count. In exchange it runs one large-LDS block per tile with limited parallelism and a long serial chain inside each block.

```diff
diff --git a/include/mst_hip.h b/include/mst_hip.h
--- a/include/mst_hip.h
+++ b/include/mst_hip.h
@@ -109,6 +109,10 @@
                         const mst_ln_args* ln, mst_stream_t stream);
 int mst_proj_ffn_ln_fwd(const mst_gemm_args* proj, const mst_ln_args* ln1, const mst_gemm_args* ff1, const mst_gemm_args* ff2,
                         const mst_ln_args* ln2, mst_stream_t stream);
+int mst_dec_tail_step(const mst_gemm_args* proj, const mst_ln_args* ln1, const mst_gemm_args* ff1, const mst_gemm_args* ff2,
+                      const mst_ln_args* ln3, const mst_gemm_args* out, const mst_bce_args* bce, const mst_gemm_args* out_dgrad,
+                      const mst_ln_args* ln3_bwd, const mst_gemm_args* ff2_dgrad, const mst_gemm_args* ff1_dgrad,
+                      const mst_ln_args* ln1_bwd, mst_stream_t stream);
 
 typedef struct mst_partial_sum {
   const float* src; int64_t n_parts; int64_t stride; int64_t len;
diff --git a/musicstyletransfer_amd/csrc/gemm_nt.hip b/musicstyletransfer_amd/csrc/gemm_nt.hip
--- a/musicstyletransfer_amd/csrc/gemm_nt.hip
+++ b/musicstyletransfer_amd/csrc/gemm_nt.hip
@@ -253,16 +253,12 @@
   gemm_epilogue_ln<T, BM, BN, WGM, WGN, MODE>(a, l, smem, acc, m0, nullptr, 0, nullptr, 0, sPar);
 }
 
-template <typename T, int BN, bool KEEP>
-__device__ __forceinline__ void gemm_bce_tile(const mst_gemm_args& a, const mst_bce_args& q, unsigned char* smem, float* red, u32x4* keepA) {
+template <typename T, int BN, int KEEP>
+__device__ __forceinline__ void bce_tile_finish(const mst_gemm_args& a, const mst_bce_args& q, unsigned char* smem, float* red, u32x4* keepA,
+                                                f32x4 (&acc)[(BN / 4) / 16][(64 / 2) / 16], int64_t m0, int64_t n0, const float (&bias8)[8]) {
   constexpr int BM = 64, WGM = 2, WGN = 4, NT = 512;
   constexpr int WTM = BM / WGM, WTN = BN / WGN, TM = WTM / 16, TN = WTN / 16;
   constexpr int LDS_F = BN + 4, CPR = BN / 8, RSTEP = NT / CPR, ITERS = BM / RSTEP;
-  f32x4 acc[TN][TM];
-  int64_t m0, n0;
-  float bias8[8];
-  gemm_bias_preload<BM, BN>(a, bias8);
-  gemm_mainloop<T, BM, BN, WGM, WGN, 64>(a, smem, acc, m0, n0);
   const int64_t P = a.N;
   const int tid = threadIdx.x, lane = tid & 63, wave = tid >> 6;
   const int wm = wave / WGN, wn = wave % WGN, frow = lane & 15, fq = lane >> 4;
@@ -331,7 +327,8 @@
       }
       if (!live) continue;
       if (a.C) *reinterpret_cast<u32x4*>(reinterpret_cast<T*>(a.C) + m * a.ldc + gc) = gb.u;
-      if constexpr (KEEP) keepA[(ch >> 3) * (BM * 8) + row * 8 + ((ch & 7) ^ (row & 7))] = gb.u;
+      if constexpr (KEEP == 1) keepA[(ch >> 3) * (BM * 8) + row * 8 + ((ch & 7) ^ (row & 7))] = gb.u;
+      if constexpr (KEEP == 2) *reinterpret_cast<u32x4*>(reinterpret_cast<T*>(keepA) + row * (BN + 8) + nc) = gb.u;
       if (q.probs) *reinterpret_cast<u32x4*>(reinterpret_cast<T*>(q.probs) + m * q.ldp + gc) = pb.u;
       if (q.logits) *reinterpret_cast<u32x4*>(reinterpret_cast<T*>(q.logits) + m * q.ldl + gc) = xb.u;
     }
@@ -346,6 +343,17 @@
     for (int i = 0; i < NT / 64; ++i) tot += red[i];
     atomicAdd(q.loss + b, tot * inv_n);
   }
+}
+
+template <typename T, int BN, bool KEEP>
+__device__ __forceinline__ void gemm_bce_tile(const mst_gemm_args& a, const mst_bce_args& q, unsigned char* smem, float* red, u32x4* keepA) {
+  constexpr int BM = 64, WGM = 2, WGN = 4;
+  f32x4 acc[(BN / WGN) / 16][(BM / WGM) / 16];
+  int64_t m0, n0;
+  float bias8[8];
+  gemm_bias_preload<BM, BN>(a, bias8);
+  gemm_mainloop<T, BM, BN, WGM, WGN, 64>(a, smem, acc, m0, n0);
+  bce_tile_finish<T, BN, KEEP ? 1 : 0>(a, q, smem, red, keepA, acc, m0, n0, bias8);
 }
 
 template <typename T, int BN>
@@ -406,10 +414,13 @@
   return MST_OK;
 }
 
-template <typename T, int BN, int WGM, int WGN, int MODE, bool LEAD, bool FULL, bool EXTRA = false>
-__global__ __launch_bounds__(WGM * WGN * 64) void ffn_ln_kernel(mst_gemm_args g1, mst_gemm_args g2, mst_ln_args ln, mst_ln_bwd_in lead,
-                                                                mst_gemm_args gx, mst_ln_args lnx) {
+template <typename T, int BN, int WGM, int WGN, int MODE, bool LEAD, bool FULL, bool EXTRA, bool X_IN_LDS = false, bool KEEP_OUT = false,
+          bool PAR_READY = false, typename Hook>
+__device__ __forceinline__ void ffn_ln_body(unsigned char* smem, mst_gemm_args g1, mst_gemm_args g2, const mst_ln_args ln,
+                                            const mst_ln_bwd_in lead, mst_gemm_args gx, const mst_ln_args lnx, float* par,
+                                            Hook&& before_epilogue) {
   constexpr bool HEAD = EXTRA;
+  static_assert(!(X_IN_LDS && (LEAD || EXTRA)), "a tile left in LDS is the block's own input");
   static_assert(!EXTRA || MODE == 1, "the extra GEMM is the forward form's head");
   constexpr int BM = 64, BK = 64, CHUNKS = BK / 8;
   constexpr int NT = WGM * WGN * 64;
@@ -419,11 +430,10 @@
   constexpr int KST = BN / BK;
   static_assert(BN * CHUNKS % NT == 0 && (BM * BN / 8) % NT == 0, "tile/threads mismatch");
   typedef typename Act<T>::vec8 vec8;
-  extern __shared__ __attribute__((aligned(16))) unsigned char smem[];
   u32x4* sB = reinterpret_cast<u32x4*>(smem);
   T* sH = reinterpret_cast<T*>(smem + (size_t)2 * BN * BK * 2);
   T* sX = sH + BM * LDA;
-  float* sBias1 = reinterpret_cast<float*>(sX + BM * LDA);
+  float* sBias1 = PAR_READY ? par : reinterpret_cast<float*>(sX + BM * LDA);
   float* sPar = sBias1 + g1.N;
   const int tid = threadIdx.x, lane = tid & 63, wave = tid >> 6;
   const int wm = wave / WGN, wn = wave % WGN, frow = lane & 15, fq = lane >> 4;
@@ -436,10 +446,12 @@
   const int64_t F = g1.N;
   FFN_STAMP(0); FFN_RT(190);
   const int64_t Mg = FULL ? (int64_t)1 << 62 : g1.M;
+  if constexpr (!PAR_READY)
   for (int i = tid * 4; i < (int)F; i += NT * 4)
     *reinterpret_cast<f32x4*>(sBias1 + i) = g1.bias ? *reinterpret_cast<const f32x4*>(g1.bias + i) : f32x4{0.f, 0.f, 0.f, 0.f};
   const uint64_t seed2 = g2.dropout_seed ^ ((g2.dropout_p > 0.f && g2.dropout_seed_ptr) ? g2.dropout_seed_ptr[0] : 0ull);
   const uint64_t seedx = EXTRA ? gx.dropout_seed ^ ((gx.dropout_p > 0.f && gx.dropout_seed_ptr) ? gx.dropout_seed_ptr[0] : 0ull) : 0ull;
+  if constexpr (!PAR_READY)
   for (int i = tid; i < BN; i += NT) {
     sPar[i] = g2.bias ? g2.bias[i] : 0.f;
     sPar[BN + i] = ln.gamma[i];
@@ -593,7 +605,7 @@
       else atomicAdd((which ? lead.dbeta : lead.dgamma) + col, sm);
     }
     __syncthreads();
-  } else
+  } else if constexpr (!X_IN_LDS)
   {
     const T* X = reinterpret_cast<const T*>(HEAD ? gx.A : g1.A);
     const int64_t ldx = HEAD ? gx.lda : g1.lda;
@@ -789,8 +801,17 @@
   }
   const bool resid_is_x = g2.resid == g1.A && g2.ldr == g1.lda;
   FFN_STAMP(2);
-  gemm_epilogue_ln<T, BM, BN, WGM, WGN, MODE>(g2, ln, smem, acc2, m0, resid_is_x ? sX : nullptr, LDA, nullptr, 0, sPar, &seed2);
+  before_epilogue();
+  gemm_epilogue_ln<T, BM, BN, WGM, WGN, MODE>(g2, ln, smem, acc2, m0, resid_is_x ? sX : nullptr, LDA, KEEP_OUT ? sX : nullptr, KEEP_OUT ? LDA : 0,
+                                              sPar, &seed2);
   FFN_STAMP(3); FFN_RT(191);
+}
+
+template <typename T, int BN, int WGM, int WGN, int MODE, bool LEAD, bool FULL, bool EXTRA = false>
+__global__ __launch_bounds__(WGM * WGN * 64) void ffn_ln_kernel(mst_gemm_args g1, mst_gemm_args g2, mst_ln_args ln, mst_ln_bwd_in lead,
+                                                                mst_gemm_args gx, mst_ln_args lnx) {
+  extern __shared__ __attribute__((aligned(16))) unsigned char smem[];
+  ffn_ln_body<T, BN, WGM, WGN, MODE, LEAD, FULL, EXTRA>(smem, g1, g2, ln, lead, gx, lnx, nullptr, [] {});
 }
 
 template <typename T, int BN>
@@ -823,6 +844,128 @@
   return MST_OK;
 }
 
+template <typename T>
+__device__ __forceinline__ void tile128_load_w(const mst_gemm_args& g, u32x4 (&rw)[2][2]) {
+  const T* __restrict__ W = reinterpret_cast<const T*>(g.B);
+#pragma unroll
+  for (int s = 0; s < 2; ++s)
+#pragma unroll
+    for (int i = 0; i < 2; ++i) {
+      const int c = threadIdx.x + i * 512, row = c / 8, ch = c % 8;
+      rw[s][i] = *reinterpret_cast<const u32x4*>(W + (int64_t)row * g.ldb + s * 64 + ch * 8);
+    }
+}
+template <typename T>
+__device__ __forceinline__ void tile128_gemm(unsigned char* smem, const T* sA, const u32x4 (&rw)[2][2], f32x4 (&acc)[2][2]) {
+  constexpr int BN = 128, LDA = BN + 8, CHUNKS = 8, WTM = 32, WTN = 32, TM = 2, TN = 2, WGN = 4;
+  typedef typename Act<T>::vec8 vec8;
+  u32x4* sB = reinterpret_cast<u32x4*>(smem);
+  const int tid = threadIdx.x, lane = tid & 63, wave = tid >> 6;
+  const int wm = wave / WGN, wn = wave % WGN, frow = lane & 15, fq = lane >> 4;
+#pragma unroll
+  for (int s = 0; s < 2; ++s)
+#pragma unroll
+    for (int i = 0; i < 2; ++i) {
+      const int c = tid + i * 512, row = c / CHUNKS, ch = c % CHUNKS;
+      sB[s * BN * CHUNKS + row * CHUNKS + (ch ^ (row & 7))] = rw[s][i];
+    }
+#pragma unroll
+  for (int j = 0; j < TN; ++j)
+#pragma unroll
+    for (int i = 0; i < TM; ++i) acc[j][i] = f32x4{0.f, 0.f, 0.f, 0.f};
+  __syncthreads();
+#pragma unroll
+  for (int s = 0; s < 2; ++s) {
+    const u32x4* cB = sB + s * BN * CHUNKS;
+#pragma unroll
+    for (int ks = 0; ks < 2; ++ks) {
+      vec8 xf[TM], wf[TN];
+      const int kc = ks * 4 + fq;
+#pragma unroll
+      for (int i = 0; i < TM; ++i)
+        xf[i] = __builtin_bit_cast(vec8, *reinterpret_cast<const u32x4*>(sA + (wm * WTM + i * 16 + frow) * LDA + s * 64 + kc * 8));
+#pragma unroll
+      for (int j = 0; j < TN; ++j) {
+        const int row = wn * WTN + j * 16 + frow;
+        wf[j] = __builtin_bit_cast(vec8, cB[row * CHUNKS + (kc ^ (row & 7))]);
+      }
+#pragma unroll
+      for (int j = 0; j < TN; ++j)
+#pragma unroll
+        for (int i = 0; i < TM; ++i) acc[j][i] = Act<T>::mfma16(wf[j], xf[i], acc[j][i]);
+    }
+  }
+  __syncthreads();
+}
+
+constexpr size_t DEC_TAIL_F = 512;
+constexpr size_t DEC_TAIL_BODY_LDS = (size_t)2 * 128 * 64 * 2 + (size_t)2 * 64 * (128 + 8) * 2 + DEC_TAIL_F * 4 + (size_t)6 * 128 * 4;
+constexpr size_t DEC_TAIL_LDS = DEC_TAIL_BODY_LDS + ((size_t)128 + 3 * 128 + DEC_TAIL_F + 3 * 128) * 4;
+static_assert(DEC_TAIL_LDS <= (size_t)48 * 1024 + (size_t)2 * (64 + 128) * 64 * 2 + (size_t)3 * 128 * 4, "no more LDS than the loss launch takes");
+
+template <typename T>
+__global__ __launch_bounds__(512) void dec_tail_kernel(mst_gemm_args proj, mst_ln_args ln1, mst_gemm_args ff1, mst_gemm_args ff2, mst_ln_args ln3,
+                                                       mst_gemm_args out, mst_bce_args bce, mst_gemm_args odg, mst_ln_args ln3b,
+                                                       mst_gemm_args f2d, mst_gemm_args f1d, mst_ln_args ln1b) {
+  constexpr int BM = 64, BN = 128, WGM = 2, WGN = 4, LDA = BN + 8, F = (int)DEC_TAIL_F;
+  extern __shared__ __attribute__((aligned(16))) unsigned char smem[];
+  __shared__ float red[512 / 64];
+  T* sX = reinterpret_cast<T*>(smem + (size_t)2 * BN * 64 * 2 + (size_t)BM * LDA * 2);
+  float* sBiasO = reinterpret_cast<float*>(smem + DEC_TAIL_BODY_LDS);
+  float* sPar3 = sBiasO + BN;
+  float* sPar4 = sPar3 + 3 * BN;
+  const int tid = threadIdx.x;
+  for (int i = tid; i < BN; i += 512) {
+    sBiasO[i] = out.bias ? out.bias[i] : 0.f;
+    sPar3[i] = odg.bias ? odg.bias[i] : 0.f;
+    sPar3[BN + i] = ln3b.gamma[i];
+    sPar3[2 * BN + i] = 0.f;
+    sPar4[F + i] = f1d.bias ? f1d.bias[i] : 0.f;
+    sPar4[F + BN + i] = ln1b.gamma[i];
+    sPar4[F + 2 * BN + i] = 0.f;
+  }
+  for (int i = tid; i < F; i += 512) sPar4[i] = f2d.bias ? f2d.bias[i] : 0.f;
+  const int64_t m0 = xcd_chunk(blockIdx.x, gridDim.x) * BM;
+  const mst_ln_bwd_in no_lead = {};
+  u32x4 rw[2][2];
+  f32x4 acc[2][2];
+  ffn_ln_body<T, BN, WGM, WGN, 1, false, true, true, false, true, false>(smem, ff1, ff2, ln3, no_lead, proj, ln1, nullptr,
+                                                                         [&] { tile128_load_w<T>(out, rw); });
+  __syncthreads();
+  tile128_gemm<T>(smem, sX, rw, acc);
+  tile128_load_w<T>(odg, rw);
+  {
+    float bias8[8];
+#pragma unroll
+    for (int e = 0; e < 8; ++e) bias8[e] = sBiasO[(tid % (BN / 8)) * 8 + e];
+    bce_tile_finish<T, BN, 2>(out, bce, smem, red, reinterpret_cast<u32x4*>(sX), acc, m0, 0, bias8);
+  }
+  __syncthreads();
+  tile128_gemm<T>(smem, sX, rw, acc);
+  gemm_epilogue_ln<T, BM, BN, WGM, WGN, 2>(odg, ln3b, smem, acc, m0, nullptr, 0, sX, LDA, sPar3);
+  __syncthreads();
+  mst_gemm_args no_gemm = {};
+  const mst_ln_args no_ln = {};
+  ffn_ln_body<T, BN, WGM, WGN, 2, false, true, false, true, false, true>(smem, f2d, f1d, ln1b, no_lead, no_gemm, no_ln, sPar4, [] {});
+}
+
+template <typename T>
+static int launch_dec_tail(const mst_gemm_args& proj, const mst_ln_args& ln1, const mst_gemm_args& ff1, const mst_gemm_args& ff2,
+                           const mst_ln_args& ln3, const mst_gemm_args& out, const mst_bce_args& bce, const mst_gemm_args& odg,
+                           const mst_ln_args& ln3b, const mst_gemm_args& f2d, const mst_gemm_args& f1d, const mst_ln_args& ln1b, hipStream_t s) {
+  static bool opted = false;
+  if (!opted) {
+    const hipError_t e = hipFuncSetAttribute(reinterpret_cast<const void*>(&dec_tail_kernel<T>), hipFuncAttributeMaxDynamicSharedMemorySize,
+                                             (int)DEC_TAIL_LDS);
+    if (e != hipSuccess) { set_error("dec_tail_kernel: LDS opt-in of %zu bytes: %s", DEC_TAIL_LDS, hipGetErrorString(e)); return MST_ERR_LAUNCH; }
+    opted = true;
+  }
+  hipLaunchKernelGGL((dec_tail_kernel<T>), dim3((unsigned)(out.M / 64)), dim3(512), DEC_TAIL_LDS, s, proj, ln1, ff1, ff2, ln3, out, bce, odg,
+                     ln3b, f2d, f1d, ln1b);
+  MST_CHECK_LAUNCH("dec_tail_kernel");
+  return MST_OK;
+}
+
 template <typename T, int BM, int BN, int WGM, int WGN>
 static int launch_gemm_ln(const mst_gemm_args& a, const mst_ln_args& l, hipStream_t s) {
   const size_t lds_loop = (size_t)2 * (BM + BN) * 64 * 2, lds_epi = (size_t)BM * (BN + 4) * 4;
@@ -938,9 +1081,8 @@
 
 extern "C" int64_t mst_gemm_nt_ln_parts(int64_t M) { return M > 0 ? cdiv(M, 64) : 0; }
 
-static int ffn_ln_impl(const char* who, const mst_gemm_args* first, const mst_gemm_args* second, const mst_ln_args* ln, int mode,
-                       mst_stream_t stream, const mst_ln_bwd_in* lead = nullptr, const mst_gemm_args* extra = nullptr,
-                       const mst_ln_args* extra_ln = nullptr) {
+static int check_ffn_ln(const char* who, const mst_gemm_args* first, const mst_gemm_args* second, const mst_ln_args* ln, int mode,
+                        const mst_ln_bwd_in* lead = nullptr, const mst_gemm_args* extra = nullptr, const mst_ln_args* extra_ln = nullptr) {
   MST_CHECK_ARG(first != nullptr && second != nullptr && ln != nullptr, "%s: null args", who);
   const mst_gemm_args& a = *first;
   const mst_gemm_args& b = *second;
@@ -1007,6 +1149,16 @@
                   "%s: the leading LayerNorm's output must be the first GEMM's A operand", who);
     MST_CHECK_ARG(!x.resid || (x.ldr % 8 == 0 && x.ldr >= x.N && (uintptr_t)x.resid % 16 == 0), "%s: bad residual layout", who);
   }
+  return MST_OK;
+}
+
+static int ffn_ln_impl(const char* who, const mst_gemm_args* first, const mst_gemm_args* second, const mst_ln_args* ln, int mode,
+                       mst_stream_t stream, const mst_ln_bwd_in* lead = nullptr, const mst_gemm_args* extra = nullptr,
+                       const mst_ln_args* extra_ln = nullptr) {
+  const int rc = check_ffn_ln(who, first, second, ln, mode, lead, extra, extra_ln);
+  if (rc) return rc;
+  const mst_gemm_args &a = *first, &b = *second;
+  const mst_ln_args& l = *ln;
   hipStream_t s = (hipStream_t)stream;
   return dispatch_act(a.dtype, [&](auto tag) -> int {
     typedef decltype(tag) T;
@@ -1124,6 +1276,45 @@
   return dispatch_act(a.dtype, [&](auto tag) -> int {
     typedef decltype(tag) T;
     return launch_gemm_bce_dgrad_ln<T>(a, q, g2, l, s);
+  });
+}
+
+extern "C" int mst_dec_tail_step(const mst_gemm_args* proj, const mst_ln_args* ln1, const mst_gemm_args* ff1, const mst_gemm_args* ff2,
+                                 const mst_ln_args* ln3, const mst_gemm_args* out, const mst_bce_args* bce, const mst_gemm_args* out_dgrad,
+                                 const mst_ln_args* ln3_bwd, const mst_gemm_args* ff2_dgrad, const mst_gemm_args* ff1_dgrad,
+                                 const mst_ln_args* ln1_bwd, mst_stream_t stream) {
+  const char* who = "mst_dec_tail_step";
+  MST_CHECK_ARG(proj && ln1 && ff1 && ff2 && ln3 && out && bce && out_dgrad && ln3_bwd && ff2_dgrad && ff1_dgrad && ln1_bwd, "%s: null args", who);
+  const mst_gemm_args &o = *out, &g = *out_dgrad, &d2 = *ff2_dgrad;
+  const int64_t T = bce->T;
+  MST_CHECK_ARG(ff2->N == 128 && ff1->K == 128 && proj->N == 128 && g.N == 128 && ff1_dgrad->N == 128,
+                "%s: the model width must be 128 (got %lld)", who, (long long)ff2->N);
+  MST_CHECK_ARG(ff1->N == 512 && d2.N == 512, "%s: the hidden width must be 512 (got %lld)", who, (long long)ff1->N);
+  MST_CHECK_ARG(o.N == 128 && o.K == 128 && g.K == 128, "%s: the output layer must have 128 pitches (got %lld)", who, (long long)o.N);
+  MST_CHECK_ARG(T > 0 && T % 64 == 0, "%s: T must be a multiple of 64 (got %lld)", who, (long long)T);
+  MST_CHECK_ARG(o.M > 0 && o.M % 64 == 0 && o.M % T == 0 && ff1->M == o.M && ff2->M == o.M && proj->M == o.M && g.M == o.M && d2.M == o.M &&
+                ff1_dgrad->M == o.M, "%s: every part works on the same whole 64-row tiles (M %lld)", who, (long long)o.M);
+  auto groups = [&](int64_t rpg, int64_t stride, int64_t off) { return rpg == T && stride == T + 1 && off == 1; };
+  MST_CHECK_ARG(groups(ff1->a_rows_per_group, ff1->a_group_stride, ff1->a_group_offset) &&
+                groups(o.a_rows_per_group, o.a_group_stride, o.a_group_offset) &&
+                groups(g.c_rows_per_group, g.c_group_stride, g.c_group_offset) &&
+                groups(d2.a_rows_per_group, d2.a_group_stride, d2.a_group_offset) && g.a_rows_per_group <= 0,
+                "%s: row groups must be (T, T + 1, 1) on all three parts", who);
+  MST_CHECK_ARG(ln3_bwd->mode == 2 && ln3_bwd->mask_mode == 2, "%s: the LayerNorm-3 backward takes mask mode 2 (got %d)", who, (int)ln3_bwd->mask_mode);
+  MST_CHECK_ARG(o.A == ln3->out && o.lda == ln3->ld_out, "%s: the output layer's A operand must be LayerNorm-3's output", who);
+  MST_CHECK_ARG(o.C && g.A == o.C && g.lda == o.ldc, "%s: the output dgrad's A operand must be the logit gradient", who);
+  MST_CHECK_ARG(d2.A == g.C && d2.lda == g.ldc, "%s: the A operand of the FF2 dgrad must be the output dgrad's dX_out", who);
+  MST_CHECK_ARG(proj->dtype == o.dtype && g.dtype == o.dtype && d2.dtype == o.dtype && ff1->dtype == o.dtype && !g.a_u8,
+                "%s: every part must share one activation dtype", who);
+  int rc = check_ffn_ln(who, ff1, ff2, ln3, 1, nullptr, proj, ln1);
+  if (rc == MST_OK) rc = check_gemm_bce(o, *bce);
+  if (rc == MST_OK) rc = check_gemm_ln(g, *ln3_bwd);
+  if (rc == MST_OK) rc = check_ffn_ln(who, ff2_dgrad, ff1_dgrad, ln1_bwd, 2);
+  if (rc) return rc;
+  hipStream_t s = (hipStream_t)stream;
+  return dispatch_act(o.dtype, [&](auto tag) -> int {
+    typedef decltype(tag) T_;
+    return launch_dec_tail<T_>(*proj, *ln1, *ff1, *ff2, *ln3, o, *bce, g, *ln3_bwd, d2, *ff1_dgrad, *ln1_bwd, s);
   });
 }
 
diff --git a/musicstyletransfer_amd/csrc/runtime.hip b/musicstyletransfer_amd/csrc/runtime.hip
--- a/musicstyletransfer_amd/csrc/runtime.hip
+++ b/musicstyletransfer_amd/csrc/runtime.hip
@@ -14,7 +14,7 @@
 
 using namespace mst;
 
-extern "C" int mst_version(void) { return 105; }
+extern "C" int mst_version(void) { return 106; }
 extern "C" const char* mst_last_error(void) { return g_err; }
 
 #define HIP_TRY(expr)                                             \
diff --git a/musicstyletransfer_amd/engine.py b/musicstyletransfer_amd/engine.py
--- a/musicstyletransfer_amd/engine.py
+++ b/musicstyletransfer_amd/engine.py
@@ -370,7 +370,7 @@
 NO_DROPOUT = Dropout(0.0, None, 0)
 
 
-def row_block_fwd(P, L, x_in, rows, drop, form, row_groups=None, tail=None):
+def row_block_fwd(P, L, x_in, rows, drop, form, row_groups=None, tail=None, launch=True):
     D, v = P.proj.w.shape[0], rows.view
     if form == "tail":
         o.row_tail_fwd(v(L.att), v(x_in), P.proj.w, P.proj.b, P.ln1.gamma, P.ln1.beta, P.ff1.w, P.ff1.b, P.ff2.w, P.ff2.b, P.ln2.gamma,
@@ -383,8 +383,11 @@
     ff2.update(dict(self_resid=True) if P.self_resid else dict(resid=v(L.x1)))
     if form == "fused":
         head = dict(att=L.att, W=P.proj.w, h1=L.h1, gamma=P.ln1.gamma, beta=P.ln1.beta, mean=L.mean1, rstd=L.rstd1, **proj)
-        o.ffn_ln_fwd(L.x1, P.ff1.w, L.a, P.ff2.w, L.h2, P.ln2.gamma, P.ln2.beta, L.x2, L.mean2, L.rstd2, ff1=ff1, ff2=ff2, proj=head,
-                     row_groups=row_groups)
+        kw = dict(x=L.x1, W1=P.ff1.w, a_out=L.a, W2=P.ff2.w, h_out=L.h2, gamma=P.ln2.gamma, beta=P.ln2.beta, y_out=L.x2, mean=L.mean2,
+                  rstd=L.rstd2, ff1=ff1, ff2=ff2, proj=head, row_groups=row_groups)
+        if not launch:
+            return kw
+        o.ffn_ln_fwd(**kw)
         return L.x2
     o.gemm_nt(v(L.att), P.proj.w, L.h1, c_remap=rows.c_remap, **proj)
     o.layernorm_fwd(v(L.h1), P.ln1.gamma, P.ln1.beta, v(L.x1), L.mean1, L.rstd1, D=D, **rows.ln)
@@ -404,7 +407,20 @@
     return None
 
 
-def row_block_bwd(P, L, t, dy, rows, drop, form, partials, dy_done=False, row_groups=None, tail=None):
+def ffn_bwd_parts(L, row_groups=None):
+    M = L.h1.shape[0]
+    return o.gemm_nt_ln_parts(M if row_groups is None else M // row_groups[1] * row_groups[0])
+
+
+def ffn_bwd_kw(P, L, t, drop, partials_buf, row_groups=None):
+    dff = t.dhm if (drop.p > 0 and not P.self_resid) else t.dh
+    ln1 = dict(dx_masked=t.dh1m, mask_mode=1, **drop.at(0)) if drop.p > 0 else {}
+    return dict(dff=dff, W2t=P.ff2.t, dpre_out=t.dpre, gate=L.a, W1t=P.ff1.t, dx_out=t.dh1, x=L.h1, gamma=P.ln1.gamma, mean=L.mean1,
+                rstd=L.rstd1, dgamma=P.ln1.dgamma, dbeta=P.ln1.dbeta, alpha=1.0 / (1.0 - drop.p) if drop.p > 0 else 1.0,
+                resid=None if P.self_resid else t.dh, partials=partials_buf, row_groups=row_groups, **ln1)
+
+
+def row_block_bwd(P, L, t, dy, rows, drop, form, partials, dy_done=False, row_groups=None, tail=None, launch=True):
     D, v = P.proj.w.shape[0], rows.view
     if form == "tail":
         o.row_tail_bwd(v(dy), v(L.h2), v(L.h1), v(L.a), L.mean1, L.rstd1, L.mean2, L.rstd2, P.ln1.gamma, P.ln2.gamma, P.ff2.t, P.ff1.t,
@@ -427,10 +443,11 @@
     inv_keep = 1.0 / (1.0 - drop.p) if drop.p > 0 else 1.0
     ln1 = dict(dx_masked=t.dh1m, mask_mode=1, **drop.at(0)) if drop.p > 0 else {}
     if form == "fused":
-        n = M if row_groups is None else M // row_groups[1] * row_groups[0]
-        o.ffn_ln_bwd(dff, P.ff2.t, t.dpre, L.a, P.ff1.t, t.dh1, L.h1, P.ln1.gamma, L.mean1, L.rstd1, P.ln1.dgamma, P.ln1.dbeta,
-                     alpha=inv_keep, resid=resid_ff, partials=partials(P.ln1, o.gemm_nt_ln_parts(n)), lead=lead, row_groups=row_groups,
-                     **ln1)
+        buf = partials(P.ln1, ffn_bwd_parts(L, row_groups))
+        if launch:
+            o.ffn_ln_bwd(lead=lead, **ffn_bwd_kw(P, L, t, drop, buf, row_groups))
+        elif lead is not None:
+            raise ValueError("row_block_bwd(launch=False) needs dy_done: the block that ran elsewhere has no leading LayerNorm backward")
     else:
         o.gemm_nt(dff, P.ff2.t, t.dpre, N=4 * D, K=D, gate=v(L.a), alpha=inv_keep)
         if form == "ln_fused":
@@ -522,7 +539,7 @@
     return not why
 
 
-Forms = namedtuple("Forms", "tails riders shadows fuse_bce bce_dgrad skip_row0 cls_fold ffn_e ffn_d ln_bwd_e ln_bwd_d sched")
+Forms = namedtuple("Forms", "tails riders shadows fuse_bce bce_dgrad skip_row0 cls_fold ffn_e ffn_d ln_bwd_e ln_bwd_d sched dec_tail")
 
 
 def check_schedule(kl_warmup_steps=0, kl_cycle_steps=0, kl_free_bits=0.0, lr_warmup_steps=0):
@@ -583,6 +600,8 @@
         self.ride = (cfg.kind != "token" and cfg.d_layers >= 1 and cfg.e_layers >= 1 and Dd in (128, 256) and
                      o.can_ride(B * T, 3 * Dd, Dd, T) and o.can_ride(B * T, Dd, 3 * Dd, T))
         self.shadows_on_tail = True
+        self.dec_tail = True
+        self.n_cu = torch.cuda.get_device_properties(self.dev).multi_processor_count if self.dev.type == "cuda" else 0
         self.forms = self._resolve_forms()
         if cfg.kind == "token":
             seg = [("tokens", B * T * 4), ("labels", B * T * 4)]
@@ -685,7 +704,7 @@
     def d_p(self):
         return 0.0 if self._infer else self.cfg.d_dropout
 
-    def _resolve_forms(self):
+    def _resolve_forms(self, with_grad=False):
         cfg, st, B, T = self.cfg, self.store, self.B, self.T
         De, Dd = cfg.e_model, cfg.d_model
         roll = cfg.kind == "pianoroll"
@@ -694,10 +713,14 @@
         shadows = "own" if not st.shadows_deferred else ("tail" if self.shadows_on_tail and riders else "begin")
         fuse_bce = roll and o.can_fuse_bce(cfg.out_dim, T, self.nld) and o.bce_fusion_pays(cfg.out_dim)
         ffn_d, ln_bwd_d = o.ffn_fusion_pays(Dd, 4 * Dd), o.ln_bwd_fusion_pays(Dd)
+        bce_dgrad = fuse_bce and ln_bwd_d
+        skip_row0 = cfg.d_layers > 0 and T % 64 == 0 and ffn_d
         return Forms(
             tails=tails, riders=riders, shadows=shadows, fuse_bce=fuse_bce,
-            bce_dgrad=fuse_bce and ln_bwd_d,
-            skip_row0=cfg.d_layers > 0 and T % 64 == 0 and ffn_d,
+            bce_dgrad=bce_dgrad,
+            skip_row0=skip_row0,
+            dec_tail=bool(with_grad and not self._infer and self.dec_tail and bce_dgrad and ffn_d and skip_row0 and
+                          o.dec_tail_pays(Dd, 4 * Dd, cfg.out_dim, T, B * T // 64, self.n_cu)),
             cls_fold=(roll and cfg.in_dim % 8 == 0 and roundup(cfg.in_dim + cfg.num_classes, 256) == roundup(cfg.in_dim, 256) and
                       st.offsets["encoder.class2hid.weight"] == st.offsets["encoder.embedding.weight"] + cfg.in_dim * De),
             ffn_e=o.ffn_fusion_pays(De, 4 * De), ffn_d=ffn_d, ln_bwd_e=o.ln_bwd_fusion_pays(De), ln_bwd_d=ln_bwd_d,
@@ -842,6 +865,8 @@
         else:
             o.attn_qkv_fwd(x_in, P.kqv.w, P.kqv.b, L.qkv, keymask, L.lse, L.att, self.B, S, H, dh, 0, D, 2 * D)
         fused = F.ffn_e if side == "encoder" else F.ffn_d
+        if F.dec_tail and side == "decoder" and i == self.cfg.d_layers - 1:
+            return L.x2
         return row_block_fwd(P, L, x_in, ALL_ROWS, self._dropout(p, site0), "fused" if fused else "launches",
                              row_groups=self._row0_groups(side, i))
 
@@ -850,12 +875,14 @@
             return (self.T, self.T + 1, 1)
         return None
 
-    def forward(self, inference=False, upto=None):
+    def forward(self, inference=False, upto=None, with_grad=False):
+        if with_grad and (inference or upto):
+            raise ValueError("forward(with_grad=True) is the forward pass of a training step")
         if upto not in (None, "latent") or (upto and not inference):
             raise ValueError("forward(upto=...) takes 'latent', in inference mode only")
         cfg, st, B, T = self.cfg, self.store, self.B, self.T
         self._infer = bool(inference)
-        F = self.forms = self._resolve_forms()
+        F = self.forms = self._resolve_forms(with_grad)
         self._tail_used = dict(fwd=False, bwd=False)
         De, Dd = cfg.e_model, cfg.d_model
         Se, Sd = T, T + 1
@@ -921,15 +948,25 @@
                          tok_parts=self.store.tok_parts if self.track_token_metrics else None)
         elif F.fuse_bce:
             dgrad = None
+            if F.dec_tail and not with_grad:
+                raise RuntimeError("forward(with_grad=True) left the last decoder layer to losses(with_grad=True)")
             if with_grad and F.bce_dgrad:
                 last, Dd, Sd = cfg.d_layers - 1, cfg.d_model, T + 1
                 dgrad = dict(A=self.dlogits, B=self.store.t("decoder.output_layer.weight"), dX_out=self.bd_l[last].dh, M=B * T, N=Dd,
                              K=self.dlogits.shape[1], c_remap=(T, Sd, 1),
                              **self._out_ln_bwd("decoder", last, self.dec[last], cfg.d_dropout, self._site_d(0) + 3 * last,
                                                 self.bd_l[last], B * T))
-            o.gemm_sigmoid_bce(self.dec_out, self.store.h("decoder.output_layer.weight"), self.labels, self.recon, T, dgrad=dgrad,
-                               dlogits=dl, probs=self.probs, label_smoothing=self.ls, downweight=self.nld, gscale=self.gscale, M=B * T,
-                               K=cfg.d_model, bias=self.store.p("decoder.output_layer.bias"), a_remap=(T, T + 1, 1))
+            loss = dict(A=self.dec_out, B=self.store.h("decoder.output_layer.weight"), labels=self.labels, loss=self.recon, T=T,
+                        dlogits=dl, probs=self.probs, label_smoothing=self.ls, downweight=self.nld, gscale=self.gscale, M=B * T,
+                        K=cfg.d_model, bias=self.store.p("decoder.output_layer.bias"), a_remap=(T, T + 1, 1))
+            if F.dec_tail:
+                L, t, P = self.dec[last], self.bd_l[last], self.store.layer("decoder", last)
+                drop, groups = self._dropout(self.d_p, self._site_d(0) + 3 * last), self._row0_groups("decoder", last)
+                x_in = self.dec[last - 1].x2 if last > 0 else self.x0_d
+                o.dec_tail_step(row_block_fwd(P, L, x_in, ALL_ROWS, drop, "fused", row_groups=groups, launch=False), loss, dgrad,
+                                ffn_bwd_kw(P, L, t, drop, self._ln_partials_buf(P.ln1, ffn_bwd_parts(L, groups)), groups))
+            else:
+                o.gemm_sigmoid_bce(dgrad=dgrad, **loss)
         else:
             o.sigmoid_bce(self.logits, self.labels, self.recon, B, T, cfg.out_dim, label_smoothing=self.ls,
                           downweight=self.nld, npos=self.npos, probs=self.probs, dlogits=dl, gscale=self.gscale,
@@ -939,10 +976,13 @@
 
     LN_PARTIALS_MIN = 32
 
+    def _ln_partials_buf(self, norm, parts):
+        return self._ln_part[norm.site] if parts >= self.LN_PARTIALS_MIN else None
+
     def _ln_partials(self, norm, parts):
-        if parts < self.LN_PARTIALS_MIN:
+        buf, dg, db = self._ln_partials_buf(norm, parts), norm.dgamma, norm.dbeta
+        if buf is None:
             return None
-        buf, dg, db = self._ln_part[norm.site], norm.dgamma, norm.dbeta
         D = dg.numel()
         if db.data_ptr() == dg.data_ptr() + 4 * D:
             self._psums.append(o.partial_sum_job(buf, parts, dg, length=2 * D))
@@ -963,8 +1003,9 @@
     def _layer_bwd(self, side, i, L, x_in, dy, dx_in, keymask, D, H, S, p, site0, t, dy_done=False, next_ln=None, ride=False):
         F, P = self.forms, self.store.layer(side, i)
         ffn, ln = (F.ffn_e, F.ln_bwd_e) if side == "encoder" else (F.ffn_d, F.ln_bwd_d)
+        in_loss = F.dec_tail and side == "decoder" and i == self.cfg.d_layers - 1
         dff, dproj = row_block_bwd(P, L, t, dy, ALL_ROWS, self._dropout(p, site0), "fused" if ffn else ("ln_fused" if ln else "launches"),
-                                   self._ln_partials, dy_done=dy_done, row_groups=self._row0_groups(side, i))
+                                   self._ln_partials, dy_done=dy_done, row_groups=self._row0_groups(side, i), launch=not in_loss)
         if side == "decoder" and self.cfg.d_causal:
             o.attn_causal_bwd(L.qkv, keymask, L.lse, t.datt, t.dqkv, t.delta, self.B, S, H, D // H, 0, D, 2 * D)
         else:
@@ -1113,7 +1154,7 @@
 
     def fwd_bwd_kernels(self, is_train=True):
         self._tick_adam = is_train
-        self.forward()
+        self.forward(with_grad=is_train)
         self.losses(with_grad=is_train, combine=not is_train)
         if is_train:
             self.backward()
@@ -1131,7 +1172,7 @@
         if is_train and split_optimizer and overlap and self.grad_cut() > 0:
             def early():
                 self._tick_adam = True
-                self.forward()
+                self.forward(with_grad=True)
                 self.losses(with_grad=True, combine=False)
                 self.backward_early(flush=True)
             self.graph = o.Graph().capture(early)
diff --git a/musicstyletransfer_amd/ops.py b/musicstyletransfer_amd/ops.py
--- a/musicstyletransfer_amd/ops.py
+++ b/musicstyletransfer_amd/ops.py
@@ -207,6 +207,14 @@
 
 
 def ffn_ln_fwd(x, W1, a_out, W2, h_out, gamma, beta, y_out, mean, rstd, eps=1e-5, ff1=None, ff2=None, proj=None, row_groups=None):
+    g0, l0, g1, g2, l = _ffn_ln_fwd_args(x, W1, a_out, W2, h_out, gamma, beta, y_out, mean, rstd, eps, ff1, ff2, proj, row_groups)
+    if proj is None:
+        call("mst_ffn_ln_fwd", C.byref(g1), C.byref(g2), C.byref(l), stream())
+    else:
+        call("mst_proj_ffn_ln_fwd", C.byref(g0), C.byref(l0), C.byref(g1), C.byref(g2), C.byref(l), stream())
+
+
+def _ffn_ln_fwd_args(x, W1, a_out, W2, h_out, gamma, beta, y_out, mean, rstd, eps=1e-5, ff1=None, ff2=None, proj=None, row_groups=None):
     ff1, ff2 = dict(ff1 or {}), dict(ff2 or {})
     if row_groups is not None:
         M, remap = _row_groups(x.shape[0], row_groups)
@@ -221,19 +229,18 @@
     l.out, l.ld_out = ptr(y_out), ld(y_out)
     l.mean, l.rstd = ptr(mean), ptr(rstd)
     if proj is None:
-        call("mst_ffn_ln_fwd", C.byref(g1), C.byref(g2), C.byref(l), stream())
-        return
+        return None, None, g1, g2, l
     kw = {k: v for k, v in proj.items() if k not in ("att", "W", "h1", "gamma", "beta", "mean", "rstd")}
     g0 = _gemm_args(proj["att"], proj["W"], proj["h1"], **kw)
     l0 = LnArgs()
     l0.mode, l0.gamma, l0.beta, l0.eps = 1, ptr(proj["gamma"]), ptr(proj["beta"]), eps
     l0.out, l0.ld_out = ptr(x), ld(x)
     l0.mean, l0.rstd = ptr(proj["mean"]), ptr(proj["rstd"])
-    call("mst_proj_ffn_ln_fwd", C.byref(g0), C.byref(l0), C.byref(g1), C.byref(g2), C.byref(l), stream())
-
-
-def ffn_ln_bwd(dff, W2t, dpre_out, gate, W1t, dx_out, x, gamma, mean, rstd, dgamma, dbeta, alpha=1.0, dx_masked=None, mask_mode=0,
-               partials=None, lead=None, row_groups=None, **kw):
+    return g0, l0, g1, g2, l
+
+
+def _ffn_ln_bwd_args(dff, W2t, dpre_out, gate, W1t, dx_out, x, gamma, mean, rstd, dgamma, dbeta, alpha=1.0, dx_masked=None, mask_mode=0,
+                     partials=None, row_groups=None, **kw):
     rg = {}
     if row_groups is not None:
         M, remap = _row_groups(dff.shape[0], row_groups)
@@ -250,6 +257,30 @@
     l.partials = ptr(partials)
     if partials is not None:
         assert partials.shape[0] >= gemm_nt_ln_parts(g1.M) and partials.shape[1] == 2 * g2.N and partials.is_contiguous()
+    return g1, g2, l
+
+
+def can_dec_tail(D, F, P, T):
+    return D == 128 and F == 512 and P == 128 and T > 0 and T % 64 == 0
+
+
+def dec_tail_pays(D, F, P, T, tiles, n_cu=256):
+    return can_dec_tail(D, F, P, T) and 0 < tiles <= n_cu
+
+
+def dec_tail_step(fwd, loss, dgrad, bwd):
+    g0, l0, g1, g2, l3 = _ffn_ln_fwd_args(**fwd)
+    go, q = _gemm_bce_args(**loss)
+    gd, l3b = _gemm_ln_bwd_args(**dgrad)
+    b1, b2, l1b = _ffn_ln_bwd_args(**bwd)
+    call("mst_dec_tail_step", C.byref(g0), C.byref(l0), C.byref(g1), C.byref(g2), C.byref(l3), C.byref(go), C.byref(q), C.byref(gd),
+         C.byref(l3b), C.byref(b1), C.byref(b2), C.byref(l1b), stream())
+
+
+def ffn_ln_bwd(dff, W2t, dpre_out, gate, W1t, dx_out, x, gamma, mean, rstd, dgamma, dbeta, alpha=1.0, dx_masked=None, mask_mode=0,
+               partials=None, lead=None, row_groups=None, **kw):
+    g1, g2, l = _ffn_ln_bwd_args(dff, W2t, dpre_out, gate, W1t, dx_out, x, gamma, mean, rstd, dgamma, dbeta, alpha, dx_masked, mask_mode,
+                                 partials, row_groups, **kw)
     if lead is None:
         call("mst_ffn_ln_bwd", C.byref(g1), C.byref(g2), C.byref(l), stream())
         return
```

Measured after the change: 26.68 million frames/s (median of 6 runs). 2.2% higher.
